# HySonLab/Protein_Redesign

Measured on AMD Instinct MI355X. Metric: denoising-steps/sec (fwd+rev) per complex, N=256 res, higher is better.
Workload: dtype f32; 1 GPU; configs[1]: synthetic 256-residue + 64-atom ligand (N=320), single_dim=512 pair_dim=64 num_blocks=4 num_steps=1000, 1 complex/GPU, sharded by sample index (no data-path collective; one all_gather of the samples at the end of the timed region); samples_per_gpu=1, hip_graph=True, outputs_finite=True, backend=single process

## Files before the change

include/prd_hip.h:

```cpp
#ifndef PRD_HIP_H
#define PRD_HIP_H

#include <stddef.h>
#include <stdint.h>

#ifdef __cplusplus
extern "C" {
#endif

#ifndef __HIP__
typedef struct ihipStream_t* hipStream_t;
#endif

#define PRD_VERSION 101
#define PRD_STEP_BOUNDARY_SYNC_INTS 2
#define PRD_ERR_ARG (-1)
#define PRD_ERR_ALIGN (-2)
#define PRD_ERR_UNSUPPORTED (-3)
#define PRD_ERR_WORKSPACE (-4)

int prd_version(void);

#define PRD_ARITH_FP32 0
#define PRD_ARITH_SPLIT16 1
// ... 163 lines not shown
int prd_tri_attn_core_v2(float* og, const float* pair, const float* mask, const float* wq, const float* wk,
                         const float* wv, const float* wg, const float* bg, int ending,
                         int b, int N, int P, int H, int c, int tune, hipStream_t stream);
int prd_tri_attn_core_v2_lse(float* og, float* lse, const float* pair, const float* mask, const float* wq, const float* wk,
                             const float* wv, const float* wg, const float* bg, int ending,
                             int b, int N, int P, int H, int c, int tune, hipStream_t stream);
int prd_tri_attn_core_fused_supported(int N, int P, int arith);
int prd_tri_attn_core_fused(float* og, float* pair_out, const float* pair, const float* og_in, const float* wo_in,
                            const float* bo_in, const float* mask, const float* wq, const float* wk, const float* wv,
                            const float* wg, const float* bg, int ending, int b, int N, int P, int H, int c,
                            hipStream_t stream);
int prd_single_attn_core(float* o, const float* qkvg, int ldq, const float* bias, const float* mask,
                         int b, int N, int H, int c, hipStream_t stream);
int prd_pair_transition(float* out, const float* pair, const float* w1, const float* b1, const float* w2,
                        const float* b2, int residual, int b, int N, int P, int* queue, int arith, hipStream_t stream);
int prd_block_tail(float* pair, const float* og, const float* wo, const float* bo, const float* w1, const float* b1,
                   const float* w2, const float* b2, const float* bias_w, const float* bias_b, float* bias_out,
                   int b, int N, int P, int H, int* queue, int arith, hipStream_t stream);
int prd_coord_head(float* eps_raw, const float* pair, const float* z, const float* mask,
                   const float* w1, const float* b1, const float* w2, int b, int N, int P, int arith, hipStream_t stream);
int prd_remove_mean(float* out, const float* x, const float* mask, int b, int N, int D, hipStream_t stream);
int prd_reverse_update(float* z, float* seq_t, int64_t* t, const float* noise_pred, const float* seq_pred,
                       const float* noise, const float* mask, const float* coef,
                       int b, int N, int n_cls, int num_steps, hipStream_t stream);

int prd_step_boundary(float* z, float* seq_t, int64_t* t, const float* eps_raw, float* seq_pred,
                      const float* noise, const float* mask, const float* coef,
                      float* single_next, const float* static_single, const float* residue_mask, const float* w_rt,
                      float* ebeta_next, const float* freqs, const float* w_beta, int* sync,
                      int b, int N, int n_cls, int num_steps, int S, int P, int time_dim,
                      const float* seq_h, int ldh, const float* w_seq, int S_h, hipStream_t stream);

int prd_spa_attn_core_supported(int N, int c, int arith);
size_t prd_spa_attn_core_workspace(int b, int N, int H, int c);
int prd_spa_attn_core(float* o, const float* qkvg, int ldq, const float* bias, const float* mask,
                      int b, int N, int H, int c, float* ws, size_t ws_bytes, int arith, hipStream_t stream);

int prd_tri_attn_heads_supported(int N, int P, int H, int c, int arith);
size_t prd_tri_attn_heads_workspace_bytes(int b, int N, int P, int H, int c);
int prd_tri_attn_core_heads(float* og, const float* pair, const float* mask, const float* wq, const float* wk,
                            const float* wv, const float* wg, const float* bg, int ending, int b, int N, int P, int H, int c,
                            float* ws, size_t ws_bytes, int arith, hipStream_t stream);
int prd_tri_attn_core_heads_lse(float* og, float* lse, const float* pair, const float* mask, const float* wq, const float* wk,
                                const float* wv, const float* wg, const float* bg, int ending, int b, int N, int P, int H, int c,
                                float* ws, size_t ws_bytes, int arith, hipStream_t stream);

int prd_tri_attn_bwd_heads_supported(int N, int P, int H, int c, int arith);
size_t prd_tri_attn_bwd_heads_workspace_bytes(int b, int N, int P, int H, int c);
int prd_tri_attn_bwd_core_heads(float* dqkvg, const float* dog, const float* og, const float* pair, const float* mask,
                                const float* wq, const float* wk, const float* wv, const float* wg, const float* bg,
                                const float* lse, float* x_out, int ending, int b, int N, int P, int H, int c,
                                float* ws, size_t ws_bytes, int arith, hipStream_t stream);

size_t prd_workspace_bytes(const char* op, int b, int N, int S, int P);

#ifdef __cplusplus
}
#endif
#endif
```

protein_redesign_amd/_lib.py:

```python
from __future__ import annotations

import ctypes as C
import os

import torch

HERE = os.path.dirname(os.path.abspath(__file__))
LIB_PATH = os.environ.get("PRD_LIB", os.path.join(HERE, "libprd_hip.so"))

vp, ci, cf, cz, cll = C.c_void_p, C.c_int, C.c_float, C.c_size_t, C.c_longlong


class PrdGemm(C.Structure):
    _fields_ = [
        ("A", vp), ("B", vp), ("C", vp),
        ("M", ci), ("N", ci), ("K", ci),
        ("lda", ci), ("ldb", ci), ("ldc", ci),
        ("G1", ci), ("G2", ci),
        ("sa1", cll), ("sa2", cll), ("sb1", cll), ("sb2", cll), ("sc1", cll), ("sc2", cll),
        ("b_kn", ci), ("alpha", cf), ("colscale", vp),
        ("bias", vp), ("act", ci), ("act_from", ci),
        ("addmat", vp), ("sad1", cll), ("sad2", cll), ("ldadd", ci),
        ("colmask", vp), ("scm1", cll), ("fill", cf),
        ("rowmask", vp), ("srm1", cll),
        ("mulmat", vp), ("smu1", cll), ("smu2", cll), ("ldmul", ci),
        ("resid", vp), ("sr1", cll), ("sr2", cll), ("ldr", ci),
        ("tile_hint", ci),
        ("a_ln", ci),
        ("ln_out", vp), ("ldlo", ci),
        ("arith", ci),
        ("C2", vp), ("ldc2", ci), ("n_split", ci),
        ("rowmask_cols", ci),
        ("rscale", vp),
        ("ws", vp), ("ws_bytes", cz),
        ("wsum", vp),
        ("out_ln", vp), ("ldol", ci),
        ("a_scale", cf),
        ("mul_pos", ci),
        ("a_amax", vp),
    ]


SIGNATURES = {
    "prd_version": [],
    "prd_tri_attn_variant": [ci, ci, ci],
    "prd_gemm": [C.POINTER(PrdGemm), vp],
    "prd_gemm_slab_workspace": [ci, ci, ci],
    "prd_gemm_slab_ok": [ci, ci, ci, ci],
    "prd_single_fc1_folded_ok": [ci] * 5,
    "prd_single_fc1_folded": [vp] * 10 + [ci] * 4 + [vp, cz, ci, vp],
    "prd_ln_rows": [vp, vp, vp, vp, ci, ci, ci, ci, vp],
    "prd_softmax_rows": [vp, ci, ci, ci, vp],
    "prd_static_pair": [vp] * 13 + [ci] * 5 + [vp],
    "prd_atom_embed": [vp] * 5 + [ci] * 4 + [vp],
    "prd_single_init": [vp] * 5 + [ci] * 3 + [vp],
    "prd_time_embed": [vp] * 4 + [ci] * 4 + [vp],
    "prd_pair_init": [vp] * 7 + [ci] * 5 + [vp],
    "prd_pair_bias": [vp] * 6 + [ci] * 4 + [vp],
    "prd_pair_bias2": [vp] * 6 + [ci] + [vp] * 5 + [ci] * 4 + [vp],
    "prd_opm_pair": [vp] * 6 + [ci] * 6 + [vp],
    "prd_pair_head_supported": [ci, ci, ci, ci],
    "prd_pair_head": [vp] * 7 + [ci] + [vp] * 3 + [ci, ci] + [vp] * 5 + [ci] + [vp] * 5 + [ci] * 5 + [vp],
    "prd_outer_linear": [vp] * 4 + [ci] + [vp] * 2 + [ci] * 5 + [vp, ci, vp],
    "prd_tri_mul": [vp] * 11 + [ci] * 5 + [vp, cz, vp, ci, vp],
    "prd_tri_mul_contract": [vp, vp, ci, ci, ci, ci, vp],
    "prd_tri_mul_contract_scaled": [vp, vp, vp, ci, ci, ci, ci, vp],
    "prd_tri_mul_chain_supported": [ci, ci, ci],
    "prd_tri_attn_core_fused_supported": [ci, ci, ci],
    "prd_tri_attn_core_fused": [vp] * 12 + [ci] * 6 + [vp],
    "prd_tri_mul_chain": [vp, vp, vp, vp, ci, ci, ci, vp, cz, ci, vp],
    "prd_tri_mul_out_bwd": [vp] * 15 + [ci] * 4 + [vp],
    "prd_tri_mul_out_bwd_amax": [vp] * 15 + [ci] * 4 + [vp, vp],
    "prd_tri_mul_bwd_operands": [vp, vp, ci, ci, ci, vp],
    "prd_tri_mul_proj_bwd": [vp] * 13 + [ci] * 5 + [vp],
    "prd_tri_attn_bwd_core": [vp] * 9 + [ci] * 6 + [vp],
    "prd_tri_attn_bwd_core_v2_supported": [ci, ci],
    "prd_tri_attn_bwd_core_v2": [vp] * 12 + [ci] * 6 + [vp],
    "prd_ln_rows_bwd": [vp, vp, vp, vp, cll, ci, vp],
    "prd_pair_bias_bwd": [vp, vp, vp, vp, vp, vp, ci, cll, ci, ci, vp],
    "prd_sym_transpose": [vp, vp, ci, ci, ci, vp],
    "prd_sym_transpose_amax": [vp, vp, ci, ci, ci, vp, vp],
    "prd_sym_rows": [vp, vp, cf, ci, ci, ci, vp],
    "prd_outer_linear_bwd_reduce": [vp, vp, ci, vp, vp, vp, cll, ci, ci, vp],
    "prd_pair_linear_supported": [ci, ci, ci],
    "prd_pair_linear": [vp, vp, vp, vp, cll, ci, ci, ci, vp, ci, vp, ci, ci, vp],
    "prd_linear_wgrad_workspace": [cll, ci, ci],
    "prd_linear_wgrad": [vp, vp, vp, vp, cll, ci, ci, ci, ci, vp, cz, ci, vp],
    "prd_embed_wgrad_workspace": [cll, ci, ci],
    "prd_embed_wgrad": [vp, vp, vp, vp, cll, ci, ci, ci, vp, cz, vp],
    "prd_rbf_rows": [vp, vp, vp, vp, ci, ci, ci, vp],
    "prd_embed_wgrad_multi": [vp, vp, vp, vp, ci, vp, cll, ci, ci, vp, cz, vp],
    "prd_tri_attn": [vp] * 10 + [ci] * 7 + [vp, cz, vp, ci, vp],
    "prd_pair_transition": [vp] * 6 + [ci] * 4 + [vp, ci, vp],
    "prd_block_tail": [vp] * 11 + [ci] * 4 + [vp, ci, vp],
    "prd_single_attn_core": [vp, vp, ci, vp, vp] + [ci] * 4 + [vp],
    "prd_coord_head": [vp] * 7 + [ci] * 4 + [vp],
    "prd_remove_mean": [vp] * 3 + [ci] * 3 + [vp],
    "prd_reverse_update": [vp] * 8 + [ci] * 4 + [vp],
    "prd_step_boundary": [vp] * 16 + [ci] * 7 + [vp, ci, vp, ci] + [vp],
    "prd_tri_attn_core": [vp] * 8 + [ci] * 7 + [vp],
    "prd_tri_attn_core_v2": [vp] * 8 + [ci] * 7 + [vp],
    "prd_tri_attn_core_v2_lse": [vp] * 9 + [ci] * 7 + [vp],
    "prd_tri_attn_v2_form": [ci, ci, ci],
    "prd_tri_attn_core_chunked": [vp] * 8 + [ci] * 6 + [vp, cz, vp],
    "prd_tri_attn_stats_bytes": [ci] * 5,
    "prd_tri_attn_v2_supported": [ci, ci, ci],
    "prd_tri_attn_out": [vp] * 5 + [ci] * 4 + [vp, ci, vp],
    "prd_spa_attn_core_supported": [ci, ci, ci],
    "prd_spa_attn_core_workspace": [ci, ci, ci, ci],
    "prd_spa_attn_core": [vp, vp, ci, vp, vp, ci, ci, ci, ci, vp, cz, ci, vp],
    "prd_workspace_bytes": [C.c_char_p, ci, ci, ci, ci],
    "prd_tri_attn_pair_supported": [ci, ci, ci],
    "prd_tri_attn_pair": [vp, vp, vp, vp, vp, ci, ci, ci, ci, ci, vp, ci, vp],
    "prd_tri_attn_heads_supported": [ci] * 5,
    "prd_tri_attn_heads_workspace_bytes": [ci] * 5,
    "prd_tri_attn_core_heads": [vp] * 8 + [ci] * 6 + [vp, cz, ci, vp],
    "prd_tri_attn_core_heads_lse": [vp] * 9 + [ci] * 6 + [vp, cz, ci, vp],
    "prd_tri_attn_bwd_heads_supported": [ci] * 5,
    "prd_tri_attn_bwd_heads_workspace_bytes": [ci] * 5,
    "prd_tri_attn_bwd_core_heads": [vp] * 12 + [ci] * 6 + [vp, cz, ci, vp],
}

GEMM_MODES = {"fp32": 0, "split16": 1, "bf16x3": 1}
DEFAULT_GEMM_MODE = "split16"

_ARITH_BEFORE_STREAM = ("prd_coord_head", "prd_pair_head", "prd_pair_init", "prd_opm_pair", "prd_outer_linear", "prd_tri_mul", "prd_tri_mul_contract", "prd_tri_mul_contract_scaled", "prd_tri_mul_proj_bwd",
                        "prd_tri_attn", "prd_tri_attn_core", "prd_tri_attn_out", "prd_pair_transition", "prd_block_tail", "prd_tri_mul_chain",
                        "prd_linear_wgrad", "prd_pair_linear", "prd_spa_attn_core", "prd_tri_attn_pair",
                        "prd_tri_attn_core_heads", "prd_tri_attn_core_heads_lse", "prd_tri_attn_bwd_core_heads", "prd_single_fc1_folded")
_ARITH_LAST = ("prd_tri_attn_variant", "prd_tri_mul_chain_supported", "prd_tri_attn_core_fused_supported", "prd_tri_attn_stats_bytes",
               "prd_gemm_slab_ok", "prd_pair_head_supported", "prd_pair_linear_supported", "prd_spa_attn_core_supported",
               "prd_tri_attn_pair_supported", "prd_tri_attn_heads_supported",
               "prd_tri_attn_bwd_heads_supported", "prd_single_fc1_folded_ok")
_TUNE_BEFORE_STREAM = ("prd_tri_attn_core_v2", "prd_tri_attn_core_v2_lse")
_TUNE_LAST = ("prd_tri_attn_v2_supported", "prd_tri_attn_v2_form")


def tune_from_env(env=None) -> int:
    env = os.environ if env is None else env

    def geti(name, default):
        v = env.get(name)
        return default if v is None or v == "" else int(v)

    t = geti("PRD_TA_VARIANT", 0) & 15
    if geti("PRD_TA2_V3", 1) == 0:
        t |= 1 << 4
    if geti("PRD_TA2_LONG", 1) == 0:
        t |= 1 << 5
    f = geti("PRD_TA2_FLAGS", -1)
    if f >= 0:
        t |= (1 << 6) | ((f & 31) << 7)
    if geti("PRD_OL_VARIANT", 0) == 1:
        t |= 1 << 12
    nw = geti("PRD_TMS_NW", 8)
    t |= (1 << 13) if nw == 12 else (2 << 13) if nw == 16 else 0
    if geti("PRD_GEMM_KG", 1) == 0:
        t |= 1 << 15
    if geti("PRD_GEMM_SLAB", 1) == 0:
        t |= 1 << 16
    if geti("PRD_GEMM_BRING", 1) == 0:
        t |= 1 << 17
    if geti("PRD_GEMM_XCDCOLS", 0) == 1:
        t |= 1 << 18
    if geti("PRD_TA2_TAIL", 1) == 0:
        t |= 1 << 19
    if geti("PRD_TA2_XCD8", 1) == 0:
        t |= 1 << 20
    if geti("PRD_TA2_GV", 1) == 0:
        t |= 1 << 21
    if geti("PRD_TMP_NW", 12) == 16:
        t |= 1 << 22
    if geti("PRD_TMS_DEPTH", 2) == 3 and nw == 8:
        t |= 3 << 13
    return t


ABI_VERSION = 101


class _Library:

    def __init__(self, cdll, mode: int, tune: int = 0):
        self._cdll = cdll
        self._mode = mode
        self._tune = tune
        self._wrapped = {}
# ... 137 lines not shown
```

protein_redesign_amd/csrc/prd_common.h:

```cpp
#pragma once
#include <hip/hip_runtime.h>
#include <stdint.h>

typedef float f32x16 __attribute__((ext_vector_type(16)));
typedef float f32x4 __attribute__((ext_vector_type(4)));
typedef float f32x2 __attribute__((ext_vector_type(2)));

#define PRD_DEV __device__ __forceinline__

PRD_DEV f32x16 mfma32(float a, float b, f32x16 c) { return __builtin_amdgcn_mfma_f32_32x32x2f32(a, b, c, 0, 0, 0); }
PRD_DEV f32x4 mfma16(float a, float b, f32x4 c) { return __builtin_amdgcn_mfma_f32_16x16x4f32(a, b, c, 0, 0, 0); }

PRD_DEV float sigmoidf_(float x) { return 1.0f / (1.0f + expf(-x)); }
PRD_DEV float relu_nan(float v) { return v < 0.f ? 0.f : v; }
PRD_DEV float sigmoid_fast(float x) { return __builtin_amdgcn_rcpf(1.0f + __builtin_amdgcn_exp2f(-1.4426950408889634f * x)); }

constexpr float NEG_LOG2E = -1.4426950408889634f;
PRD_DEV float gate_from_scaled(float y) { return __builtin_amdgcn_rcpf(1.0f + __builtin_amdgcn_exp2f(y)); }

typedef __amdgpu_buffer_rsrc_t prd_rsrc;
PRD_DEV prd_rsrc make_rsrc(const void* p) {
    const unsigned long long a = reinterpret_cast<unsigned long long>(p);
    const unsigned lo = __builtin_amdgcn_readfirstlane((unsigned)a), hi = __builtin_amdgcn_readfirstlane((unsigned)(a >> 32));
    return __builtin_amdgcn_make_buffer_rsrc(reinterpret_cast<void*>(((unsigned long long)hi << 32) | lo), 0, 0x7fffffff, 0x00020000);
}
PRD_DEV void buf_store(float v, prd_rsrc rs, unsigned lane_bytes, unsigned uniform_bytes) {
    __builtin_amdgcn_raw_buffer_store_b32(__float_as_uint(v), rs, lane_bytes, uniform_bytes, 0);
}
PRD_DEV float buf_load(prd_rsrc rs, unsigned lane_bytes, unsigned uniform_bytes) {
    return __uint_as_float(__builtin_amdgcn_raw_buffer_load_b32(rs, lane_bytes, uniform_bytes, 0));
}
constexpr unsigned BUF_OOB = 0x80000000u;

PRD_DEV int drow32(int q, int hi) { return (q & 3) + 8 * (q >> 2) + 4 * hi; }
PRD_DEV int cll_ch(int s, int hi) { return 8 * (s >> 2) + 4 * hi + (s & 3); }

PRD_DEV float xhalf_sum(float v) { return v + __shfl_xor(v, 32); }
PRD_DEV float row16_sum(float v) {
    v += __builtin_bit_cast(float, __builtin_amdgcn_update_dpp(0, __builtin_bit_cast(int, v), 0x128, 0xf, 0xf, false));
    v += __builtin_bit_cast(float, __builtin_amdgcn_update_dpp(0, __builtin_bit_cast(int, v), 0x124, 0xf, 0xf, false));
    v += __builtin_bit_cast(float, __builtin_amdgcn_update_dpp(0, __builtin_bit_cast(int, v), 0x122, 0xf, 0xf, false));
    v += __builtin_bit_cast(float, __builtin_amdgcn_update_dpp(0, __builtin_bit_cast(int, v), 0x121, 0xf, 0xf, false));
    return v;
}

template <int C>
PRD_DEV void load_row_cll(const float* __restrict__ row, int hi, bool valid, float (&x)[C / 2]) {
#pragma unroll
    for (int m = 0; m < C / 8; ++m) {
        float4 v = make_float4(0.f, 0.f, 0.f, 0.f);
        if (valid) v = *reinterpret_cast<const float4*>(row + 8 * m + 4 * hi);
        x[4 * m + 0] = v.x; x[4 * m + 1] = v.y; x[4 * m + 2] = v.z; x[4 * m + 3] = v.w;
    }
}

// ... 440 lines not shown
}

template <int NB>
PRD_DEV void zero_acc(f32x16 (&acc)[NB]) {
#pragma unroll
    for (int nb = 0; nb < NB; ++nb)
#pragma unroll
        for (int q = 0; q < 16; ++q) acc[nb][q] = 0.f;
}

PRD_DEV float max3f(float a, float b, float c) {
    float d;
    asm("v_max3_f32 %0, %1, %2, %3" : "=v"(d) : "v"(a), "v"(b), "v"(c));
    return d;
}
PRD_DEV float max2f(float a, float b) {
    float d;
    asm("v_max_f32 %0, %1, %2" : "=v"(d) : "v"(a), "v"(b));
    return d;
}

PRD_DEV float rows4_max(float v) {
    auto a = __builtin_amdgcn_permlane32_swap(__float_as_uint(v), __float_as_uint(v), false, false);
    v = max2f(__uint_as_float(a[0]), __uint_as_float(a[1]));
    auto b = __builtin_amdgcn_permlane16_swap(__float_as_uint(v), __float_as_uint(v), false, false);
    return max2f(__uint_as_float(b[0]), __uint_as_float(b[1]));
}
PRD_DEV float rows4_sum(float v) {
    auto a = __builtin_amdgcn_permlane32_swap(__float_as_uint(v), __float_as_uint(v), false, false);
    v = __uint_as_float(a[0]) + __uint_as_float(a[1]);
    auto b = __builtin_amdgcn_permlane16_swap(__float_as_uint(v), __float_as_uint(v), false, false);
    return __uint_as_float(b[0]) + __uint_as_float(b[1]);
}

PRD_DEV void wave_lds_fence() {
    __builtin_amdgcn_fence(__ATOMIC_RELEASE, "wavefront");
    __builtin_amdgcn_wave_barrier();
    __builtin_amdgcn_fence(__ATOMIC_ACQUIRE, "wavefront");
}

struct WaveTasks {
    int* q;
    long ntask, cur, stride;
    int shard, nshard, count, last;
    PRD_DEV WaveTasks(int* queue, long ntask_, int waves_per_wg) : q(queue), ntask(ntask_) {
        stride = (long)gridDim.x * waves_per_wg;
        cur = (long)(threadIdx.x >> 6) * gridDim.x + blockIdx.x;
        nshard = gridDim.x < 8 ? (int)gridDim.x : 8;
        shard = (int)(blockIdx.x % nshard);
        count = (int)((ntask - shard + nshard - 1) / nshard);
        const int wgs = (int)((gridDim.x - shard + nshard - 1) / nshard);
        last = count + wgs * waves_per_wg - 1;
    }
    PRD_DEV long next() {
        if (!q) {
            const long t = (long)__builtin_amdgcn_readfirstlane((int)cur);
            cur += stride;
            return t < ntask ? t : -1;
        }
        int t = 0;
        if ((threadIdx.x & 63) == 0) {
            t = atomicAdd(q + 32 * shard, 1);
            if (t == last) atomicExch(q + 32 * shard, 0);
        }
        t = __builtin_amdgcn_readfirstlane(t);
        return t < count ? (long)t * nshard + shard : -1;
    }
};

#define PRD_SPLIT_ARITH(a)                                                                       \
    const int arith_full = (a);                                                                  \
    const int tune = (a) >> 8;                                                                   \
    (void)tune; (void)arith_full;                                                                \
    if ((a) < 0 || ((a) & 0xff) > 1) return -1;                                                  \
    (a) &= 0xff
#define PRD_TGET_TA_VARIANT(t) ((t) & 15)
#define PRD_TGET_TA2_NO_V3(t) (((t) >> 4) & 1)
#define PRD_TGET_TA2_NO_LONG(t) (((t) >> 5) & 1)
#define PRD_TGET_TA2_FLAGS(t) ((((t) >> 6) & 1) ? (((t) >> 7) & 31) : -1)
#define PRD_TGET_TA2_NO_TAIL_SPLIT(t) (((t) >> 19) & 1)
#define PRD_TGET_TA2_NO_GV(t) (((t) >> 21) & 1)
#define PRD_TGET_TMP_NW16(t) (((t) >> 22) & 1)
#define PRD_TGET_TMS_D3(t) ((((t) >> 13) & 3) == 3)
#define PRD_TGET_OL_GEN2(t) (((t) >> 12) & 1)
#define PRD_TGET_TMS_NW(t) ((((t) >> 13) & 3) == 1 ? 12 : (((t) >> 13) & 3) == 2 ? 16 : 8)

static inline int prd_ceil_div(int a, int b) { return (a + b - 1) / b; }
static inline int prd_round_up(int a, int b) { return prd_ceil_div(a, b) * b; }
```

protein_redesign_amd/csrc/prd_pair.hip:

```cpp
#include "prd_common.h"
#include <cstdlib>
#include "../../include/prd_hip.h"
#include <mutex>

#ifdef PRD_TIMING
__device__ unsigned long long prd_dbg_pair[256 * 16 * 8];
extern "C" int prd_debug_read_pair(void* dst) { return (int)hipMemcpyFromSymbol(dst, HIP_SYMBOL(prd_dbg_pair), sizeof(prd_dbg_pair)); }
struct PairPhaseTimer {
    unsigned long long t, acc[8];
    __device__ PairPhaseTimer() { for (int k = 0; k < 8; ++k) acc[k] = 0; t = __builtin_readcyclecounter(); }
    __device__ void mark(int k) {
        __builtin_amdgcn_sched_barrier(0);
        const unsigned long long n = __builtin_readcyclecounter();
        __builtin_amdgcn_sched_barrier(0);
        acc[k] += n - t;
        t = n;
    }
    __device__ void flush() {
        if ((threadIdx.x & 63) == 0) for (int k = 0; k < 8; ++k) prd_dbg_pair[(blockIdx.x * 16 + (threadIdx.x >> 6)) * 8 + k] = acc[k];
    }
};
#else
struct PairPhaseTimer {
    __device__ void mark(int) {}
// ... 1453 lines not shown
    constexpr int NWH = 8;
    const size_t lds = (size_t)4 * P * dist_dim + (size_t)4 * P * C + ((size_t)dist_dim + P + 16 * P + 4 * P) * 4;
    const long ntask = (long)b * N * prd_ceil_div(N, 32);
    const int grid = grid_for(ntask, NWH, 256);
    if (P == 64) {
        PRD_SET_LDS((pair_head_h2_kernel<64, NWH>), lds);
        hipLaunchKernelGGL((pair_head_h2_kernel<64, NWH>), dim3(grid), dim3(NWH * 64), lds, stream, pair, static_pair, z, mask, centers, w_dist,
                           ebeta, dist_dim, ab, w_out, b_out, C, apply_mask, bias_a, gamma_a, beta_a, w_a, bvec_a, Ha, bias_b, gamma_b, beta_b,
                           w_b, bvec_b, Hb, b, N);
    } else {
        PRD_SET_LDS((pair_head_h2_kernel<32, NWH>), lds);
        hipLaunchKernelGGL((pair_head_h2_kernel<32, NWH>), dim3(grid), dim3(NWH * 64), lds, stream, pair, static_pair, z, mask, centers, w_dist,
                           ebeta, dist_dim, ab, w_out, b_out, C, apply_mask, bias_a, gamma_a, beta_a, w_a, bvec_a, Ha, bias_b, gamma_b, beta_b,
                           w_b, bvec_b, Hb, b, N);
    }
    return (int)hipGetLastError();
}

extern "C" int prd_opm_pair(float* out, const float* pair, const float* ab, const float* mask, const float* w_out,
                            const float* b_out, int flags, int b, int N, int P, int C, int arith, hipStream_t stream) {
    PRD_SPLIT_ARITH(arith);
    if (!out || !pair || !ab || !mask || !w_out || !b_out || b <= 0 || N <= 0) return PRD_ERR_ARG;
    PRD_CHECK_P(P);
    if (C <= 0 || (C & 7)) return PRD_ERR_UNSUPPORTED;
    const size_t lds = ((size_t)P * (C + 4) + P) * sizeof(float);
    if (lds > 160 * 1024) return PRD_ERR_UNSUPPORTED;
    const long ntask = (long)b * N * prd_ceil_div(N, 32);
    const int grid = grid_for(ntask, 4, 1024);
    if (arith == PRD_ARITH_SPLIT16 && (C % 128) == 0) {
        const size_t lds2 = (size_t)4 * P * C + (size_t)P * 4;
        if (P == 64) {
            PRD_SET_LDS(opm_pair_h2_kernel<64>, lds2);
            hipLaunchKernelGGL(opm_pair_h2_kernel<64>, dim3(grid), dim3(WG), lds2, stream, out, pair, ab, mask, w_out, b_out, b, N, C, flags);
        } else {
            PRD_SET_LDS(opm_pair_h2_kernel<32>, lds2);
            hipLaunchKernelGGL(opm_pair_h2_kernel<32>, dim3(grid), dim3(WG), lds2, stream, out, pair, ab, mask, w_out, b_out, b, N, C, flags);
        }
        return (int)hipGetLastError();
    }
    if (P == 64) {
        PRD_SET_LDS(opm_pair_kernel<64>, lds);
        hipLaunchKernelGGL(opm_pair_kernel<64>, dim3(grid), dim3(WG), lds, stream, out, pair, ab, mask, w_out, b_out, b, N, C, flags);
    } else {
        PRD_SET_LDS(opm_pair_kernel<32>, lds);
        hipLaunchKernelGGL(opm_pair_kernel<32>, dim3(grid), dim3(WG), lds, stream, out, pair, ab, mask, w_out, b_out, b, N, C, flags);
    }
    return (int)hipGetLastError();
}

namespace {
template <int P, int KS>
__global__ __launch_bounds__(512) void outer_linear_ks_kernel(float* out, const float* pair, const float* __restrict__ x,
                                                              const float* __restrict__ u, const float* __restrict__ w,
                                                              const float* __restrict__ bias, int b, int N, int residual, int ldu) {
    constexpr int NB = P / 32, NW = 8, S = 128 * KS, NG = NB * 4;
    constexpr int CW = 16 * KS;
    constexpr int XP = CW * 4 + 16;
    constexpr int LR = CW / 4;
    constexpr int RPI = 64 / LR;
    constexpr int NLD = 32 / RPI;
    extern __shared__ __attribute__((aligned(16))) unsigned char smem_ks[];
    float4* part = reinterpret_cast<float4*>(smem_ks);
    float4* stage = part;
    constexpr int PSZ = NW * NG * 64;
    const int lane = threadIdx.x & 63, r = lane & 31, hi = lane >> 5;
    const int wave = __builtin_amdgcn_readfirstlane(threadIdx.x >> 6);
    PairPhaseTimer pt;
    const int k0 = wave * CW;
    float4* mystage = stage + (size_t)wave * 32 * (XP / 16);
    u32x4 wh[NB][KS], wl[NB][KS];
#pragma unroll
    for (int nb = 0; nb < NB; ++nb)
#pragma unroll
        for (int st = 0; st < KS; ++st) {
            const float* wp = w + (size_t)(32 * nb + r) * (2 * S) + k0 + 16 * st + 8 * hi;
            const float4 g0 = *reinterpret_cast<const float4*>(wp), g1 = *reinterpret_cast<const float4*>(wp + 4);
            const float v[8] = {g0.x, g0.y, g0.z, g0.w, g1.x, g1.y, g1.z, g1.w};
#pragma unroll
            for (int q = 0; q < 4; ++q) {
                unsigned a_, b_;
                split2h(H2_WSCALE * v[2 * q], H2_WSCALE * v[2 * q + 1], a_, b_);
                wh[nb][st][q] = a_;
                wl[nb][st][q] = b_;
            }
        }
    const int nvb = (N + 31) / 32;
    const int npairs = nvb * (nvb + 1) / 2;
    constexpr int RG = 8;
    const int ntask = b * npairs * (32 / RG);
    struct Task { int bb, i0, jb; };
    auto decode = [&](int t) {
        Task T;
        const int grp = t % (32 / RG), t2 = t / (32 / RG);
        T.bb = t2 / npairs;
        int pidx = t2 - T.bb * npairs, ib = 0;
        while (pidx >= nvb - ib) { pidx -= nvb - ib; ++ib; }
        T.jb = ib + pidx;
        T.i0 = ib * 32 + grp * RG;
        return T;
    };
    const int lane_w = lane;
    struct Epi { float4 ui, pu, pm; };
    pt.mark(6);
    for (int t = blockIdx.x; t < ntask; t += gridDim.x) {
        const Task T = decode(t);
        int lane = lane_w;
        asm volatile("" : "+v"(lane));
// ... 52 lines not shown
        fetch_x(T.i0, xa);
        __syncthreads();
        pt.mark(4);
        auto finish = [&](int i, const float4* pb, const Epi& e) {
            if (!row_ok(i)) return;
            float4 sum = make_float4(0.f, 0.f, 0.f, 0.f);
#pragma unroll
            for (int w2 = 0; w2 < NW; ++w2) {
                const float4 v = pb[(size_t)w2 * NG * 64 + eoff];
                sum.x += v.x; sum.y += v.y; sum.z += v.z; sum.w += v.w;
            }
            const bool upper = jvalid && je >= i, mirror = jvalid && je > i;
            const float4 ui = e.ui, pu = e.pu, pm = e.pm;
            if (upper)
                *reinterpret_cast<float4*>(out + (((size_t)T.bb * N + i) * N + je) * P + ech) =
                    make_float4(pu.x + (((sum.x * H2_INV_WSCALE + ui.x) - uj.x) + bs.x), pu.y + (((sum.y * H2_INV_WSCALE + ui.y) - uj.y) + bs.y),
                                pu.z + (((sum.z * H2_INV_WSCALE + ui.z) - uj.z) + bs.z), pu.w + (((sum.w * H2_INV_WSCALE + ui.w) - uj.w) + bs.w));
            if (mirror)
                *reinterpret_cast<float4*>(out + (((size_t)T.bb * N + je) * N + i) * P + ech) =
                    make_float4(pm.x + (((sum.x * H2_INV_WSCALE + uj.x) - ui.x) + bs.x), pm.y + (((sum.y * H2_INV_WSCALE + uj.y) - ui.y) + bs.y),
                                pm.z + (((sum.z * H2_INV_WSCALE + uj.z) - ui.z) + bs.z), pm.w + (((sum.w * H2_INV_WSCALE + uj.w) - ui.w) + bs.w));
        };
        for (int ii = 0; ii < RG; ++ii) {
            const int i = T.i0 + ii;
            fetch_epi(i, enext);
            f32x16 acc[NB];
            zero_acc(acc);
            if (row_ok(i)) {
#pragma unroll
                for (int st = 0; st < KS; ++st) {
                    const float f[8] = {xa[st][0].x * xb[st][0].x, xa[st][0].y * xb[st][0].y, xa[st][0].z * xb[st][0].z, xa[st][0].w * xb[st][0].w,
                                        xa[st][1].x * xb[st][1].x, xa[st][1].y * xb[st][1].y, xa[st][1].z * xb[st][1].z, xa[st][1].w * xb[st][1].w};
                    u32x4 ph, pl;
#pragma unroll
                    for (int q = 0; q < 4; ++q) {
                        unsigned a_, b_;
                        split2h(f[2 * q], f[2 * q + 1], a_, b_);
                        ph[q] = a_;
                        pl[q] = b_;
                    }
#pragma unroll
                    for (int nb = 0; nb < NB; ++nb)
                        acc[nb] = __builtin_amdgcn_mfma_f32_32x32x16_f16(__builtin_bit_cast(f16x8_t, wh[nb][st]), __builtin_bit_cast(f16x8_t, ph), acc[nb], 0, 0, 0);
#pragma unroll
                    for (int nb = 0; nb < NB; ++nb)
                        acc[nb] = __builtin_amdgcn_mfma_f32_32x32x16_f16(__builtin_bit_cast(f16x8_t, wh[nb][st]), __builtin_bit_cast(f16x8_t, pl), acc[nb], 0, 0, 0);
#pragma unroll
                    for (int nb = 0; nb < NB; ++nb)
                        acc[nb] = __builtin_amdgcn_mfma_f32_32x32x16_f16(__builtin_bit_cast(f16x8_t, wl[nb][st]), __builtin_bit_cast(f16x8_t, ph), acc[nb], 0, 0, 0);
                }
            }
            if (ii + 1 < RG) fetch_x(i + 1, xa);
            pt.mark(0);
            if (ii > 0) finish(i - 1, part + (size_t)((ii - 1) & 1) * PSZ, ecur);
            ecur = enext;
            pt.mark(3);
            {
                float4* pw = part + (size_t)(ii & 1) * PSZ + ((size_t)wave * NG) * 64;
#pragma unroll
                for (int g = 0; g < NG; ++g)
                    pw[g * 64 + ((lane & 48) | ((lane & 15) ^ ((2 * g + hi) & 15)))] = make_float4(acc[g >> 2][4 * (g & 3)], acc[g >> 2][4 * (g & 3) + 1], acc[g >> 2][4 * (g & 3) + 2],
                                                     acc[g >> 2][4 * (g & 3) + 3]);
            }
            pt.mark(1);
            asm volatile("s_waitcnt lgkmcnt(0)\n\ts_barrier" ::: "memory");
            pt.mark(2);
        }
        finish(T.i0 + RG - 1, part + (size_t)((RG - 1) & 1) * PSZ, ecur);
        __syncthreads();
    }
    pt.mark(7);
    pt.flush();
}
}

extern "C" int prd_outer_linear(float* out, const float* pair, const float* x, const float* u, int ldu, const float* w,
                                const float* bias, int residual, int b, int N, int P, int S, int* queue, int arith, hipStream_t stream) {
    PRD_SPLIT_ARITH(arith);
    if (!out || !pair || !x || !u || !w || !bias || b <= 0 || N <= 0) return PRD_ERR_ARG;
    if (ldu < P || (ldu & 3)) return PRD_ERR_ALIGN;
    PRD_CHECK_P(P);
    if (S <= 0 || (S & 7)) return PRD_ERR_UNSUPPORTED;
    const long ntask = (long)b * N * prd_ceil_div(N, 32);
    const size_t lds = ((size_t)P * (S + 4) + P) * sizeof(float);
    const bool ol_v1 = PRD_TGET_OL_GEN2(tune);
    if (arith == PRD_ARITH_SPLIT16 && !ol_v1 && (S == 128 || S == 256 || S == 512) && (long)b * N * N < (1L << 30)) {
        const int nvb = prd_ceil_div(N, 32);
        const long ntile = (long)b * (nvb * (nvb + 1) / 2) * 4;
        const int grid = (int)(ntile < 256 ? ntile : 256);
        const size_t ldsp = (size_t)2 * 8 * (P / 32 * 4) * 64 * 16, ldss = (size_t)8 * 32 * ((S / 8) * 4 + 16);
        const size_t ldsk = ldsp > ldss ? ldsp : ldss;
#define PRD_OLKS(PP, KK)                                                                                               \
        do {                                                                                                           \
            PRD_SET_LDS((outer_linear_ks_kernel<PP, KK>), ldsk);                                                       \
            hipLaunchKernelGGL((outer_linear_ks_kernel<PP, KK>), dim3(grid), dim3(512), ldsk, stream, out, pair, x, u, w, bias, b, N, residual, ldu); \
        } while (0)
        if (P == 64) { if (S == 512) PRD_OLKS(64, 4); else if (S == 256) PRD_OLKS(64, 2); else PRD_OLKS(64, 1); }
        else { if (S == 512) PRD_OLKS(32, 4); else if (S == 256) PRD_OLKS(32, 2); else PRD_OLKS(32, 1); }
#undef PRD_OLKS
        return (int)hipGetLastError();
    }
    if (arith == PRD_ARITH_SPLIT16 && (S % 128) == 0 && (size_t)4 * P * S + 4 * P <= 160 * 1024) {
        constexpr int NWL = 8;
        const int nvb = prd_ceil_div(N, 32);
        const long nsym = (long)b * (nvb * (nvb + 1) / 2) * 32;
        const int grid = grid_for(nsym, 4, 256);
        const size_t lds2 = (size_t)4 * P * S + 4 * P;
        if (P == 64) {
            PRD_SET_LDS((outer_linear_res_h2_kernel<64, NWL>), lds2);
            hipLaunchKernelGGL((outer_linear_res_h2_kernel<64, NWL>), dim3(grid), dim3(NWL * 64), lds2, stream, out, pair, x, u, w, bias, b, N, S, residual, ldu);
        } else {
            PRD_SET_LDS((outer_linear_res_h2_kernel<32, NWL>), lds2);
            hipLaunchKernelGGL((outer_linear_res_h2_kernel<32, NWL>), dim3(grid), dim3(NWL * 64), lds2, stream, out, pair, x, u, w, bias, b, N, S, residual, ldu);
        }
        return (int)hipGetLastError();
    }
    if (lds <= 150 * 1024 && (S % 64) == 0) {
        constexpr int NWL = 8;
        const int nvb = prd_ceil_div(N, 32);
        const long nsym = (long)b * (nvb * (nvb + 1) / 2) * 32;
        const int grid = grid_for(nsym, 4, 256);
        int* oq = (nsym > (long)grid * NWL) ? queue : nullptr;
        if (P == 64) {
            PRD_SET_LDS((outer_linear_res_kernel<64, NWL>), lds);
            hipLaunchKernelGGL((outer_linear_res_kernel<64, NWL>), dim3(grid), dim3(NWL * 64), lds, stream, oq, out, pair, x, u, w, bias, b, N, S, residual, ldu);
        } else {
            PRD_SET_LDS((outer_linear_res_kernel<32, NWL>), lds);
            hipLaunchKernelGGL((outer_linear_res_kernel<32, NWL>), dim3(grid), dim3(NWL * 64), lds, stream, oq, out, pair, x, u, w, bias, b, N, S, residual, ldu);
        }
        return (int)hipGetLastError();
    }
    const int grid = grid_for(ntask, 4, 1024);
    if (P == 64) hipLaunchKernelGGL(outer_linear_kernel<64>, dim3(grid), dim3(WG), 0, stream, out, pair, x, u, w, bias, b, N, S, residual, ldu);
    else hipLaunchKernelGGL(outer_linear_kernel<32>, dim3(grid), dim3(WG), 0, stream, out, pair, x, u, w, bias, b, N, S, residual, ldu);
    return (int)hipGetLastError();
}

namespace {
template <int P>
int launch_pair_tail_h2(float* out, const float* pair, const float* og, const float* wo, const float* bo, const float* w1,
                        const float* b1, const float* w2, const float* b2, const float* bias_w, const float* bias_b,
                        float* bias_out, int H, long rows, long nn, int residual, hipStream_t stream) {
    constexpr int NWH = 12;
    const size_t lds = ((size_t)2 * 4 * P * (P / 8) + (size_t)2 * P * (4 * P / 8) + (size_t)2 * P * 8) * 16 + (size_t)(4 * P + 2 * P + 8 * P) * 4;
    if (lds > 160 * 1024) return PRD_ERR_UNSUPPORTED;
    const int grid = grid_for((rows + 31) / 32, 4, 256);
    PRD_SET_LDS((pair_tail_h2_kernel<P, NWH>), lds);
    hipLaunchKernelGGL((pair_tail_h2_kernel<P, NWH>), dim3(grid), dim3(NWH * 64), lds, stream, out, pair, og, wo, bo, w1, b1, w2, b2,
// ... 103 lines not shown
```

protein_redesign_amd/csrc/prd_tri.hip:

```cpp
#include "prd_common.h"
#include "../../include/prd_hip.h"
#include <atomic>
#include <cstdlib>
#include <mutex>

#ifdef PRD_TIMING
__device__ unsigned long long prd_dbg[256 * 16 * 8 * 4];
__device__ int prd_dbg_sel;
extern "C" int prd_debug_read(void* dst) { return (int)hipMemcpyFromSymbol(dst, HIP_SYMBOL(prd_dbg), sizeof(prd_dbg)); }
extern "C" int prd_debug_select(int id) { return (int)hipMemcpyToSymbol(HIP_SYMBOL(prd_dbg_sel), &id, sizeof(int)); }
#define PRD_STAMP(k) do { if (lane == 0 && it < 8) prd_dbg[((blockIdx.x * 12 + wave) * 8 + it) * 4 + (k)] = __builtin_readcyclecounter(); } while (0)
struct PhaseTimer {
    unsigned long long t, acc[8];
    __device__ PhaseTimer() { for (int k = 0; k < 8; ++k) acc[k] = 0; t = __builtin_readcyclecounter(); }
    __device__ void mark(int k) {
        __builtin_amdgcn_sched_barrier(0);
        const unsigned long long n = __builtin_readcyclecounter();
        __builtin_amdgcn_sched_barrier(0);
        acc[k] += n - t;
        t = n;
    }
    __device__ void flush(int id = 0) {
        if (prd_dbg_sel != 0 && prd_dbg_sel != id) return;
        if ((threadIdx.x & 63) == 0) for (int k = 0; k < 8; ++k) prd_dbg[(blockIdx.x * 16 + (threadIdx.x >> 6)) * 8 + k] = acc[k];
// ... 285 lines not shown
    *reinterpret_cast<float4*>(&As[BUF][srow * LDP + 4 * sf]) = R##a0;            \
    *reinterpret_cast<float4*>(&As[BUF][(srow + 32) * LDP + 4 * sf]) = R##a1;     \
    *reinterpret_cast<float4*>(&Bs[BUF][srow * LDP + 4 * sf]) = R##b0;            \
    *reinterpret_cast<float4*>(&Bs[BUF][(srow + 32) * LDP + 4 * sf]) = R##b1;
#define PRD_TMC_CHUNK(C, CUR, R, N)                                               \
    {                                                                             \
        const int c2 = (C) + 2 < nchunk ? (C) + 2 : nchunk - 1;                   \
        PRD_TMC_LOAD(N, c2 * KCH)                                                 \
        const float* as = &As[CUR][(wm0 + r) * LDP + hi * 16];                    \
        const float* bs = &Bs[CUR][(wn0 + r) * LDP + hi * 16];                    \
        _Pragma("unroll") for (int t = 0; t < 4; ++t) {                           \
            const float4 a = *reinterpret_cast<const float4*>(as + 4 * t);        \
            const float4 bq = *reinterpret_cast<const float4*>(bs + 4 * t);       \
            acc = mfma32(a.x, bq.x, acc);                                         \
            acc = mfma32(a.y, bq.y, acc);                                         \
            acc = mfma32(a.z, bq.z, acc);                                         \
            acc = mfma32(a.w, bq.w, acc);                                         \
        }                                                                         \
        if ((C) + 1 < nchunk) { PRD_TMC_STAGE(R, (CUR) ^ 1) }                     \
        __syncthreads();                                                          \
    }
    float4 ua0, ua1, ub0, ub1, va0, va1, vb0, vb1;
    PRD_TMC_LOAD(u, 0)
    PRD_TMC_STAGE(u, 0)
    {
        const int c1 = 1 < nchunk ? 1 : 0;
        PRD_TMC_LOAD(u, c1 * KCH)
    }
    __syncthreads();
    for (int c = 0; c < nchunk; c += 2) {
        PRD_TMC_CHUNK(c, 0, u, v)
        if (c + 1 < nchunk) PRD_TMC_CHUNK(c + 1, 1, v, u)
    }
#undef PRD_TMC_LOAD
#undef PRD_TMC_LD1
#undef PRD_TMC_STAGE
#undef PRD_TMC_CHUNK
    float* __restrict__ Oc = O + (size_t)ch * N * ldn;
    const int n = n0 + wn0 + r;
    if (n < N) {
#pragma unroll
        for (int q = 0; q < 16; ++q) {
            const int m = m0 + wm0 + drow32(q, hi);
            if (m < N) Oc[(size_t)m * ldn + n] = acc[q];
        }
    }
    }
}

constexpr int TMS_T = 160, TMS_PLANE = TMS_T * 64, TMS_OPER = 2 * TMS_PLANE;
template <int NWV, int DEPTH = 2, bool ASC = false>
__global__ __launch_bounds__(NWV * 64) void tri_mul_contract_split_kernel(float* __restrict__ O, const float* __restrict__ AB,
                                                                          int N, int ldn, int P, int nbatch, int tiles, int swap,
                                                                          const unsigned* __restrict__ a_amax) {
    constexpr int NT = NWV * 64, NPT = (2560 + NT - 1) / NT, NSUB = (25 + NWV - 1) / NWV;
    extern __shared__ __attribute__((aligned(16))) unsigned char tms[];
    PhaseTimer pt;
    const int tid = threadIdx.x, lane = tid & 63, wave = tid >> 6;
    const int r = lane & 31, hi = lane >> 5;
    const int nch = nbatch * P;
    const int t2 = tiles * tiles;
    unsigned srow[NPT], sdst[NPT], ssrc[NPT];
    bool sisb[NPT], sok[NPT];
    const int wbase = __builtin_amdgcn_readfirstlane(tid & ~63);
#pragma unroll
    for (int i = 0; i < NPT; ++i) {
        const int pw = wbase + NT * i;
        sok[i] = pw < 2560;
        const int oper = (sok[i] && pw >= 1280) ? 1 : 0;
        const int pc = sok[i] ? tid + NT * i : 0;
        const int q = pc - 1280 * oper;
        const int row = q >> 3, f = q & 7;
        sisb[i] = oper == 1;
        srow[i] = row;
        sdst[i] = oper * TMS_OPER + row * 64 + (((f >> 1) ^ ((row >> 2) & 3)) << 4) + (f & 1) * 8;
        ssrc[i] = ((unsigned)row * ldn + 4 * f) * 4u;
    }
    const unsigned swz = (unsigned)((r >> 2) & 3);
    for (int vblk = blockIdx.x; vblk < nch * t2; vblk += gridDim.x) {
        int ch, tile;
        if ((nch & 7) == 0 && (gridDim.x & 7) == 0) {
            const int xcd = vblk & 7, k = vblk >> 3;
            ch = xcd + 8 * (k / t2);
            tile = k % t2;
        } else {
            ch = vblk / t2;
            tile = vblk % t2;
        }
        const int bb = ch / P, d = ch - bb * P;
        const int m0 = (tile / tiles) * TMS_T, n0 = (tile % tiles) * TMS_T;
        float asc = 1.0f, iasc = 1.0f;
        if constexpr (ASC) {
            asc = split_scale(a_amax[bb]);
            iasc = __uint_as_float((254u << 23) - __float_as_uint(asc));
        }
        const float* __restrict__ A = AB + ((size_t)bb * 2 * P + (swap ? P : 0) + d) * N * ldn;
        const float* __restrict__ B = AB + ((size_t)bb * 2 * P + (swap ? 0 : P) + d) * N * ldn;
        const prd_rsrc ra = make_rsrc(A + (size_t)m0 * ldn), rb = make_rsrc(B + (size_t)n0 * ldn);
        unsigned off[NPT];
#pragma unroll
        for (int i = 0; i < NPT; ++i)
            off[i] = (sok[i] && (sisb[i] ? n0 : m0) + (int)srow[i] < N) ? ssrc[i] : BUF_OOB;
        int si[NSUB], sj[NSUB];
        bool sv[NSUB];
#pragma unroll
        for (int k = 0; k < NSUB; ++k) {
            const int s_ = wave + NWV * k;
// ... 61 lines not shown
        _Pragma("unroll") for (int st = 0; st < 2; ++st) {                                                          \
            const unsigned col = (((unsigned)(2 * st + hi)) ^ swz) << 4;                                            \
            _Pragma("unroll") for (int k = 0; k < NSUB; ++k) {                                                      \
                if (sv[k]) {                                                                                        \
                    const unsigned char* ap = base + (32 * si[k] + r) * 64 + col;                                   \
                    const unsigned char* bp = base + TMS_OPER + (32 * sj[k] + r) * 64 + col;                        \
                    u32x4 a[2], bq[2];                                                                              \
                    _Pragma("unroll") for (int pl = 0; pl < 2; ++pl) {                                              \
                        a[pl] = *reinterpret_cast<const u32x4*>(ap + pl * TMS_PLANE);                               \
                        bq[pl] = *reinterpret_cast<const u32x4*>(bp + pl * TMS_PLANE);                              \
                    }                                                                                               \
                    const int pa[3] = {0, 0, 1}, pb[3] = {0, 1, 0};                                                 \
                    _Pragma("unroll") for (int t = 0; t < 3; ++t)                                                   \
                        acc[k] = __builtin_amdgcn_mfma_f32_32x32x16_f16(__builtin_bit_cast(f16x8_t, a[pa[t]]),      \
                                                                        __builtin_bit_cast(f16x8_t, bq[pb[t]]), acc[k], 0, 0, 0); \
                }                                                                                                   \
            }                                                                                                       \
        }                                                                                                           \
        pt.mark(0);                                                                                                 \
        if ((C) + 1 < nchunk) { PRD_TMS_STAGE(R, cur_ ^ 1) }                                                        \
        pt.mark(1);                                                                                                 \
        __syncthreads();                                                                                            \
        pt.mark(2);                                                                                                 \
    }
            PRD_TMS_LOAD(u, 0)
            PRD_TMS_STAGE(u, 0)
            PRD_TMS_LOAD(u, (1 < nchunk ? 1 : 0))
            PRD_TMS_LOAD(v, (2 < nchunk ? 2 : nchunk - 1))
            __syncthreads();
            pt.mark(3);
            for (int c = 0; c < nchunk; c += 3) {
                PRD_TMS_CHUNK3(c, u, w)
                if (c + 1 < nchunk) PRD_TMS_CHUNK3(c + 1, v, u)
                if (c + 2 < nchunk) PRD_TMS_CHUNK3(c + 2, w, v)
            }
#undef PRD_TMS_CHUNK3
        } else {
        PRD_TMS_LOAD(u, 0)
        PRD_TMS_STAGE(u, 0)
        {
            const int c1 = 1 < nchunk ? 1 : 0;
            PRD_TMS_LOAD(u, c1)
        }
        __syncthreads();
        pt.mark(3);
        for (int c = 0; c < nchunk; c += 2) {
            PRD_TMS_CHUNK(c, 0, u, v)
            if (c + 1 < nchunk) PRD_TMS_CHUNK(c + 1, 1, v, u)
        }
        }
#undef PRD_TMS_LOAD
#undef PRD_TMS_STAGE
#undef PRD_TMS_CHUNK
        float* __restrict__ Oc = O + (size_t)ch * N * ldn;
#pragma unroll
        for (int k = 0; k < NSUB; ++k) {
            if (!sv[k]) continue;
            const int n = n0 + 32 * sj[k] + r;
            if (n < N) {
#pragma unroll
                for (int q = 0; q < 16; ++q) {
                    const int m = m0 + 32 * si[k] + drow32(q, hi);
                    if (m < N) Oc[(size_t)m * ldn + n] = ASC ? acc[k][q] * iasc : acc[k][q];
                }
            }
        }
        pt.mark(4);
    }
    pt.flush(3);
}

template <int P, int NW, bool B3>
__global__ __launch_bounds__(NW * 64) void tri_mul_out_kernel(int* queue, float* out, const float* pair, const float* __restrict__ O,
                                                              const float* __restrict__ wo, const float* __restrict__ bo,
                                                              const float* __restrict__ wog, const float* __restrict__ bog,
                                                              int b, int N, int ldn, int residual) {
    constexpr int KH = P / 2, NB = P / 32;
    constexpr int WSZ = B3 ? P * P : P * (P + 4);
    __shared__ __attribute__((aligned(16))) float Wol[WSZ];
    __shared__ __attribute__((aligned(16))) float Wgl[WSZ];
    __shared__ __attribute__((aligned(16))) float bol[P];
    __shared__ __attribute__((aligned(16))) float bgl[P];
    constexpr float ASC = B3 ? H2_INV_WSCALE : 1.0f;
    PhaseTimer pt;
    if (B3) {
        stage_weight_h2<P>(reinterpret_cast<u32x4*>(Wol), wo, P, P, threadIdx.x, NW * 64, H2_WSCALE);
        stage_weight_h2<P>(reinterpret_cast<u32x4*>(Wgl), wog, P, P, threadIdx.x, NW * 64, H2_WSCALE);
    } else {
        stage_weight_cll<P>(Wol, wo, P, P, threadIdx.x, NW * 64);
        stage_weight_cll<P>(Wgl, wog, P, P, threadIdx.x, NW * 64);
    }
    stage_vec_cll(bol, bo, P, threadIdx.x, NW * 64);
    stage_vec_cll(bgl, bog, P, threadIdx.x, NW * 64);
    __syncthreads();
    pt.mark(6);
    const int lane = threadIdx.x & 63, r = lane & 31, hi = lane >> 5, wave = threadIdx.x >> 6;
    const int nvb = (N + 31) / 32;
    const long ntask = (long)b * N * nvb;
    const long slots = (long)gridDim.x * 4;
    const long left = ntask % slots;
    const bool coop = !B3 && queue == nullptr && NB == 2 && NW >= 4 && left > 0 && left <= 2 * (long)gridDim.x;
    const long nwhole = coop ? ntask - left : ntask;
    WaveTasks tasks(queue, nwhole, NW);
    for (long task = tasks.next(); task >= 0; task = tasks.next()) {
        const int vb = (int)(task % nvb);
        const long bi = task / nvb;
        const int bb = (int)(bi / N), i = (int)(bi - (long)bb * N);
        const int j = vb * 32 + r;
        const bool valid = j < N;
        const int jj = valid ? j : 0;
        const long off = (bi * N + jj) * P;
        float x[KH], xr[KH];
        {
            const prd_rsrc ro = make_rsrc(O + (((long)bb * P) * N + i) * ldn + vb * 32);
            const unsigned cbytes = (unsigned)N * (unsigned)ldn * 4u;
            const unsigned lo = valid ? (unsigned)r * 4u + (unsigned)(4 * hi) * cbytes : BUF_OOB;
#pragma unroll
            for (int s = 0; s < KH; ++s) x[s] = buf_load(ro, lo, (unsigned)(8 * (s >> 2) + (s & 3)) * cbytes);
            const prd_rsrc rp = make_rsrc(pair + (bi * N + vb * 32) * P);
            load_row_cll_buf<P>(rp, valid ? ((unsigned)r * P + 4 * hi) * 4u : BUF_OOB, xr);
        }
        pt.mark(0);
        float gate[KH];
        {
            float xn[KH];
#pragma unroll
            for (int s = 0; s < KH; ++s) xn[s] = xr[s];
            ln_cll<KH>(xn);
            pt.mark(1);
            f32x16 ag[NB];
            zero_acc(ag);
            if (B3) {
                u32x4 xs[2][P / 16];
                split2h_cll<KH>(xn, xs);
                rowgemm_h2<P, NB>(reinterpret_cast<const u32x4*>(Wgl), P, 0, xs, ag, r, hi);
            } else {
                rowgemm<P, NB>(Wgl, xn, ag, r, hi);
            }
#pragma unroll
            for (int s = 0; s < KH; ++s) gate[s] = sigmoid_fast(ag[s >> 4][s & 15] * ASC + bgl[hi * KH + s]);
        }
        pt.mark(2);
        ln_cll<KH>(x);
        pt.mark(3);
        f32x16 ao[NB];
        zero_acc(ao);
        if (B3) {
            u32x4 xs[2][P / 16];
            split2h_cll<KH>(x, xs);
            rowgemm_h2<P, NB>(reinterpret_cast<const u32x4*>(Wol), P, 0, xs, ao, r, hi);
        } else {
            rowgemm<P, NB>(Wol, x, ao, r, hi);
        }
        pt.mark(4);
#pragma unroll
        for (int s = 0; s < KH; ++s) x[s] = (residual ? xr[s] : 0.f) + gate[s] * (ao[s >> 4][s & 15] * ASC + bol[hi * KH + s]);
        store_row_cll<P>(out + off, hi, valid, x);
        pt.mark(5);
    }
    pt.mark(7);
    pt.flush(2);
    if (coop) {
        __shared__ float part[2][64][17];
        for (long task = nwhole + blockIdx.x; task < ntask; task += gridDim.x) {
            const int vb = (int)(task % nvb);
            const long bi = task / nvb;
            const int bb = (int)(bi / N), i = (int)(bi - (long)bb * N);
            const int j = vb * 32 + r;
            const bool valid = j < N;
            const int jj = valid ? j : 0;
            const long off = (bi * N + jj) * P;
            const int nb = wave & 1;
            f32x16 acc[1];
            zero_acc(acc);
            float x[KH];
            if (wave < 2) {
                load_row_cll<P>(pair + off, hi, valid, x);
                ln_cll<KH>(x);
                if (B3) {
                    u32x4 xs[2][P / 16];
                    split2h_cll<KH>(x, xs);
                    rowgemm_h2<P, 1>(reinterpret_cast<const u32x4*>(Wgl), P, nb * 32, xs, acc, r, hi);
                } else {
                    rowgemm<P, 1>(Wgl + nb * 32 * (P + 4), x, acc, r, hi);
                }
            } else if (wave < 4) {
#pragma unroll
                for (int s = 0; s < KH; ++s)
                    x[s] = valid ? O[(((long)bb * P + cll_ch(s, hi)) * N + i) * ldn + jj] : 0.f;
                ln_cll<KH>(x);
                if (B3) {
                    u32x4 xs[2][P / 16];
                    split2h_cll<KH>(x, xs);
                    rowgemm_h2<P, 1>(reinterpret_cast<const u32x4*>(Wol), P, nb * 32, xs, acc, r, hi);
                } else {
                    rowgemm<P, 1>(Wol + nb * 32 * (P + 4), x, acc, r, hi);
                }
#pragma unroll
                for (int q = 0; q < 16; ++q) part[nb][lane][q] = acc[0][q] * ASC;
            }
            __syncthreads();
            if (wave < 2) {
                float* orow = out + off + 32 * nb + 4 * hi;
                const float* prow = pair + off + 32 * nb + 4 * hi;
#pragma unroll
                for (int gq = 0; gq < 4; ++gq) {
                    float4 pv = make_float4(0.f, 0.f, 0.f, 0.f);
                    if (valid && residual) pv = *reinterpret_cast<const float4*>(prow + 8 * gq);
                    float o4[4] = {pv.x, pv.y, pv.z, pv.w};
#pragma unroll
                    for (int e = 0; e < 4; ++e) {
                        const int q = 4 * gq + e, sidx = 16 * nb + q;
// ... 1211 lines not shown
                }
            }
            float4 qf[2], gf[2];
#pragma unroll
            for (int t = 0; t < 2; ++t) {
                const int src = 16 * t + ql + 32 * (g4 & 1);
                float lo[4], up[4], glo[4], gup[4];
#pragma unroll
                for (int e = 0; e < 4; ++e) {
                    lo[e] = __shfl(qg[e], src);
                    up[e] = __shfl(qg[4 + e], src);
                    glo[e] = __shfl(qg[8 + e], src);
                    gup[e] = __shfl(qg[12 + e], src);
                }
                const bool hiq = (g4 >> 1) != 0;
                qf[t] = make_float4(sc * (hiq ? up[0] : lo[0]), sc * (hiq ? up[1] : lo[1]), sc * (hiq ? up[2] : lo[2]), sc * (hiq ? up[3] : lo[3]));
                gf[t] = make_float4(sigmoid_fast(hiq ? gup[0] : glo[0]), sigmoid_fast(hiq ? gup[1] : glo[1]),
                                    sigmoid_fast(hiq ? gup[2] : glo[2]), sigmoid_fast(hiq ? gup[3] : glo[3]));
            }
            f32x4 o[2];
            float l_tot[2], m_ref[2];
            ta_keyloop<2, true>(Kl, Vt, kadd, qf, npad, ql, g4, o, l_tot, m_ref);
#pragma unroll
            for (int t = 0; t < 2; ++t) {
                const int v = qb * 32 + 16 * t + ql;
                if (v < N) {
                    const long pos = ending ? (((long)bb * N + v) * N + u) : (bu * N + v);
                    float4* dst = reinterpret_cast<float4*>(og + pos * HC + h * C + 4 * g4);
                    float* st = stats + (pos * H + h) * 2;
                    const float il = 1.0f / l_tot[t];
                    float4 mine = make_float4(gf[t].x * (o[t][0] * il), gf[t].y * (o[t][1] * il), gf[t].z * (o[t][2] * il), gf[t].w * (o[t][3] * il));
                    float m_new = m_ref[t], l_new = l_tot[t];
                    if (!first) {
                        const float m0 = st[0], l0 = st[1];
                        const float4 prev = *dst;
                        const float M = fmaxf(m0, m_ref[t]);
                        const float w0 = l0 * exp2f(m0 - M), w1 = l_tot[t] * exp2f(m_ref[t] - M);
                        const float iw = 1.0f / (w0 + w1);
                        const float a0 = w0 * iw, a1 = w1 * iw;
                        mine = make_float4(a0 * prev.x + a1 * mine.x, a0 * prev.y + a1 * mine.y, a0 * prev.z + a1 * mine.z, a0 * prev.w + a1 * mine.w);
                        m_new = M;
                        l_new = w0 + w1;
                    }
                    *dst = mine;
                    if (g4 == 0) { st[0] = m_new; st[1] = l_new; }
                }
            }
        }
    }
}

template <int P, int NW, bool B3>
__global__ __launch_bounds__(NW * 64) void tri_attn_out_kernel(int* queue, float* out, const float* pair, const float* __restrict__ og,
                                                               const float* __restrict__ wo, const float* __restrict__ bo, long rows, int residual) {
    constexpr int KH = P / 2, NB = P / 32, HC = 64;
    __shared__ __attribute__((aligned(16))) float Wl[B3 ? P * HC : P * (HC + 4)];
    __shared__ __attribute__((aligned(16))) float bl[P];
    if (B3) stage_weight_h2<HC>(reinterpret_cast<u32x4*>(Wl), wo, P, HC, threadIdx.x, NW * 64, H2_WSCALE);
    else stage_weight_cll<HC>(Wl, wo, P, HC, threadIdx.x, NW * 64);
    stage_vec_cll(bl, bo, P, threadIdx.x, NW * 64);
    __syncthreads();
    const int lane = threadIdx.x & 63, r = lane & 31, hi = lane >> 5;
    const long ntask = (rows + 31) / 32;
    WaveTasks tasks(queue, ntask, NW);
    for (long task = tasks.next(); task >= 0; task = tasks.next()) {
        const long pos = task * 32 + r;
        const bool valid = pos < rows;
        float x[HC / 2];
        load_row_cll<HC>(og + pos * HC, hi, valid, x);
        f32x16 acc[NB];
        zero_acc(acc);
        if (B3) {
            u32x4 xs[2][HC / 16];
            split2h_cll<HC / 2>(x, xs);
            rowgemm_h2<HC, NB>(reinterpret_cast<const u32x4*>(Wl), P, 0, xs, acc, r, hi);
        } else {
            rowgemm<HC, NB>(Wl, x, acc, r, hi);
        }
        float pr[KH];
        load_row_cll<P>(pair + pos * P, hi, valid && residual, pr);
#pragma unroll
        for (int s = 0; s < KH; ++s) pr[s] = pr[s] + (acc[s >> 4][s & 15] * (B3 ? H2_INV_WSCALE : 1.0f) + bl[hi * KH + s]);
        store_row_cll<P>(out + pos * P, hi, valid, pr);
    }
}

int grid_for(long tasks, int per_wg, int cap) {
    long g = (tasks + per_wg - 1) / per_wg;
    if (g > cap) g = cap;
    if (g < 1) g = 1;
    return (int)g;
}

}

#define PRD_SET_LDS(kernel, bytes)                                                                              \
    do {                                                                                                        \
        static std::once_flag prd_lds_once;                                                                     \
        std::call_once(prd_lds_once, [] {                                                                       \
            (void)hipFuncSetAttribute((const void*)kernel, hipFuncAttributeMaxDynamicSharedMemorySize, 160 * 1024); \
        });                                                                                                     \
        (void)(bytes);                                                                                          \
    } while (0)

static void launch_contract_split(int tune, int grid, size_t lds3, hipStream_t stream, float* O, const float* AB, int N, int ldn, int P, int nbatch,
                                  int tiles, int swap, const unsigned* a_amax = nullptr) {
    if (a_amax) {
        PRD_SET_LDS((tri_mul_contract_split_kernel<8, 2, true>), lds3);
        hipLaunchKernelGGL((tri_mul_contract_split_kernel<8, 2, true>), dim3(grid), dim3(512), lds3, stream, O, AB, N, ldn, P, nbatch, tiles, swap, a_amax);
        return;
    }
    const int nw = PRD_TGET_TMS_NW(tune);
#ifdef PRD_AB
    if (nw == 8 && PRD_TGET_TMS_D3(tune)) {
        PRD_SET_LDS((tri_mul_contract_split_kernel<8, 3>), lds3);
        hipLaunchKernelGGL((tri_mul_contract_split_kernel<8, 3>), dim3(grid), dim3(512), lds3, stream, O, AB, N, ldn, P, nbatch, tiles, swap, nullptr);
        return;
    }
    if (nw == 16) {
        PRD_SET_LDS((tri_mul_contract_split_kernel<16>), lds3);
        hipLaunchKernelGGL((tri_mul_contract_split_kernel<16>), dim3(grid), dim3(1024), lds3, stream, O, AB, N, ldn, P, nbatch, tiles, swap, nullptr);
        return;
    }
#endif
    if (nw == 12) {
        PRD_SET_LDS((tri_mul_contract_split_kernel<12>), lds3);
        hipLaunchKernelGGL((tri_mul_contract_split_kernel<12>), dim3(grid), dim3(768), lds3, stream, O, AB, N, ldn, P, nbatch, tiles, swap, nullptr);
    } else {
        PRD_SET_LDS((tri_mul_contract_split_kernel<8>), lds3);
        hipLaunchKernelGGL((tri_mul_contract_split_kernel<8>), dim3(grid), dim3(512), lds3, stream, O, AB, N, ldn, P, nbatch, tiles, swap, nullptr);
    }
}


#ifdef PRD_AB
constexpr bool PRD_FIRST_GEN = true;
#else
constexpr bool PRD_FIRST_GEN = false;
#endif
namespace {
size_t tri_attn_lds(int N, int P, bool b3, bool* long_row) {
    const int npad = prd_round_up(N, 64);
    const size_t wsz = b3 ? (size_t)3 * 64 * (2 * (P / 16) + 1) * 4 : (size_t)64 * (P + 4);
    size_t lds = (wsz + (size_t)3 * npad * KP + 16 * (npad + 4) + npad + 32) * sizeof(float);
    if (b3) lds = (size_t)64 * P * 4 + (size_t)npad * (192 + KP * 4 + 4) + (size_t)64 * (npad + 8) + 128;
    *long_row = lds > 160 * 1024;
    if (*long_row) {
        const size_t lds_sl = (size_t)64 * P * 4 + (size_t)npad * 68 + (size_t)64 * (npad + 8) + 128 + 8 * 4096;
        if (b3 && lds_sl <= 160 * 1024) return lds_sl;
        lds = ((size_t)64 * (P + 4) + (size_t)npad * KP + 16 * (npad + 4) + npad) * sizeof(float);
    }
    return lds;
}
}

extern "C" int prd_tri_attn_variant(int N, int P, int arith) {
    PRD_SPLIT_ARITH(arith);
    if (N <= 0) return PRD_ERR_ARG;
    if (P != 32 && P != 64) return PRD_ERR_UNSUPPORTED;
    bool long_row;
    const bool split = arith == PRD_ARITH_SPLIT16;
    const bool v2 = split && PRD_TGET_TA_VARIANT(tune) == 0 && prd_tri_attn_v2_supported(N, P, tune);
    const bool b3 = split && (PRD_FIRST_GEN || v2);
    const size_t lds = tri_attn_lds(N, P, b3, &long_row);
    if (lds > 160 * 1024)
        return v2 ? 2 : 3;
    if (!long_row) return 0;
    if (v2) return 2;
    const int npad = prd_round_up(N, 64);
    return (b3 && lds == (size_t)64 * P * 4 + (size_t)npad * 68 + (size_t)64 * (npad + 8) + 128 + 8 * 4096) ? 2 : 1;
}

namespace {
constexpr int TA_CHUNK_MAX = 960;
int ta_chunks(int N) { return prd_ceil_div(N, TA_CHUNK_MAX); }
}

extern "C" size_t prd_tri_attn_stats_bytes(int b, int N, int P, int H, int arith) {
    if (b <= 0 || N <= 0 || H <= 0) return 0;
    return prd_tri_attn_variant(N, P, arith) == 3 ? (size_t)b * N * N * H * 2 * sizeof(float) : 0;
}

extern "C" int prd_tri_attn_core_chunked(float* og, const float* pair, const float* mask, const float* wq, const float* wk,
// ... 44 lines not shown
extern "C" int prd_tri_mul(float* out, const float* pair, const float* mask, const float* w_proj, const float* b_proj,
                           const float* w_gate, const float* b_gate, const float* w_out, const float* b_out,
                           const float* w_ogate, const float* b_ogate, int incoming, int residual,
                           int b, int N, int P, float* ws, size_t ws_bytes, int* queue, int arith, hipStream_t stream) {
    PRD_SPLIT_ARITH(arith);
    if (!out || !pair || !mask || !w_proj || !b_proj || !w_gate || !b_gate || !w_out || !b_out || !w_ogate || !b_ogate || !ws ||
        b <= 0 || N <= 0) return PRD_ERR_ARG;
    if (P != 32 && P != 64) return PRD_ERR_UNSUPPORTED;
    if (ws_bytes < prd_workspace_bytes("tri_mul", b, N, 0, P)) return PRD_ERR_WORKSPACE;
    const int ldn = prd_round_up(N, 32);
    float* AB = ws;
    float* O = ws + (size_t)2 * b * P * N * ldn;
    const bool b3m = arith == PRD_ARITH_SPLIT16;
    {
        constexpr int NWP = 16;
        const bool b3 = b3m;
        const size_t wsz = b3 ? (size_t)2 * P * P : (size_t)2 * P * (P + 4);
        const size_t lds = (2 * wsz + 4 * P) * sizeof(float);
        const long ntask = ((long)b * N * (ldn / 32) + 7) / 8 * 8 * (2 * P / 32);
        const int grid = grid_for(ntask, 4, 256);
#define PRD_PROJ_LAUNCH(PP, BB, NWV)                                                                                 \
        do {                                                                                                         \
            PRD_SET_LDS((tri_mul_proj_kernel<PP, NWV, BB>), lds);                                                    \
            hipLaunchKernelGGL((tri_mul_proj_kernel<PP, NWV, BB>), dim3(grid), dim3(NWV * 64), lds, stream, queue, AB, pair, mask, \
                               w_proj, b_proj, w_gate, b_gate, b, N, ldn, incoming);                                 \
        } while (0)
        if (P == 64) { if (b3) { if (PRD_TGET_TMP_NW16(tune)) PRD_PROJ_LAUNCH(64, true, 16); else PRD_PROJ_LAUNCH(64, true, 12); } else PRD_PROJ_LAUNCH(64, false, NWP); }
        else { if (b3) PRD_PROJ_LAUNCH(32, true, 12); else PRD_PROJ_LAUNCH(32, false, NWP); }
#undef PRD_PROJ_LAUNCH
        int e = (int)hipGetLastError();
        if (e) return e;
    }
    {
        const int tiles = prd_ceil_div(N, 64);
        const int vblocks = b * P * tiles * tiles;
        if (b3m) {
            const int tl = prd_ceil_div(N, TMS_T);
            const int vb3 = b * P * tl * tl;
            const size_t lds3 = (size_t)4 * TMS_OPER;
        launch_contract_split(tune, vb3 < 256 ? vb3 : 256, lds3, stream, O, AB, N, ldn, P, b, tl, 0);
        }
        else
            hipLaunchKernelGGL(tri_mul_contract_kernel, dim3(vblocks < 1024 ? vblocks : 1024), dim3(256), 0, stream, O, AB, N, ldn, P, b, tiles);
        int e = (int)hipGetLastError();
        if (e) return e;
    }
    {
        constexpr int NWO = 8;
        const bool b3o = b3m;
        const long ntask = (long)b * N * prd_ceil_div(N, 32);
        const int grid = grid_for(ntask, 4, 256);
#define PRD_OUT_LAUNCH(PP, BB)                                                                                         \
        hipLaunchKernelGGL((tri_mul_out_kernel<PP, NWO, BB>), dim3(grid), dim3(NWO * 64), 0, stream, queue, out, pair, O, w_out, \
                           b_out, w_ogate, b_ogate, b, N, ldn, residual)
        if (P == 64) { if (b3o) PRD_OUT_LAUNCH(64, true); else PRD_OUT_LAUNCH(64, false); }
        else { if (b3o) PRD_OUT_LAUNCH(32, true); else PRD_OUT_LAUNCH(32, false); }
#undef PRD_OUT_LAUNCH
    }
    return (int)hipGetLastError();
}

extern "C" int prd_tri_mul_contract(float* O, const float* AB, int b, int N, int P, int arith, hipStream_t stream) {
    PRD_SPLIT_ARITH(arith);
    if (!O || !AB || b <= 0 || N <= 0) return PRD_ERR_ARG;
    if (P != 32 && P != 64 && P != 128) return PRD_ERR_UNSUPPORTED;
    const int ldn = prd_round_up(N, 32);
    if (arith == PRD_ARITH_SPLIT16) {
        const int tl = prd_ceil_div(N, TMS_T);
        const int vb3 = b * P * tl * tl;
        const size_t lds3 = (size_t)4 * TMS_OPER;
        launch_contract_split(tune, vb3 < 256 ? vb3 : 256, lds3, stream, O, AB, N, ldn, P, b, tl, 0);
    } else {
        const int tiles = prd_ceil_div(N, 64);
        const int vblocks = b * P * tiles * tiles;
        hipLaunchKernelGGL(tri_mul_contract_kernel, dim3(vblocks < 1024 ? vblocks : 1024), dim3(256), 0, stream, O, AB, N, ldn, P, b, tiles);
    }
    return (int)hipGetLastError();
}

extern "C" int prd_tri_mul_contract_scaled(float* O, const float* AB, const unsigned* a_amax, int b, int N, int P, int arith, hipStream_t stream) {
    if (!a_amax) return PRD_ERR_ARG;
    if ((arith & 0xff) != PRD_ARITH_SPLIT16) return prd_tri_mul_contract(O, AB, b, N, P, arith, stream);
    PRD_SPLIT_ARITH(arith);
    if (!O || !AB || b <= 0 || N <= 0) return PRD_ERR_ARG;
    if (P != 32 && P != 64 && P != 128) return PRD_ERR_UNSUPPORTED;
    const int ldn = prd_round_up(N, 32);
    const int tl = prd_ceil_div(N, TMS_T);
    const int vb3 = b * P * tl * tl;
    launch_contract_split(tune, vb3 < 256 ? vb3 : 256, (size_t)4 * TMS_OPER, stream, O, AB, N, ldn, P, b, tl, 0, a_amax);
    return (int)hipGetLastError();
}

extern "C" int prd_tri_mul_chain_supported(int N, int P, int arith) {
    return (N > 0 && (P == 32 || P == 64) && arith >= 0 && (arith & 0xff) == PRD_ARITH_SPLIT16) ? 1 : 0;
}

extern "C" int prd_tri_mul_chain(float* pair, const float* mask, const float* const* w_outgoing, const float* const* w_incoming,
                                 int b, int N, int P, float* ws, size_t ws_bytes, int arith, hipStream_t stream) {
    PRD_SPLIT_ARITH(arith);
    if (!pair || !mask || !w_outgoing || !w_incoming || !ws || b <= 0 || N <= 0) return PRD_ERR_ARG;
    for (int k = 0; k < 8; ++k)
        if (!w_outgoing[k] || !w_incoming[k]) return PRD_ERR_ARG;
    if (!prd_tri_mul_chain_supported(N, P, arith)) return PRD_ERR_UNSUPPORTED;
    if (ws_bytes < prd_workspace_bytes("tri_mul", b, N, 0, P)) return PRD_ERR_WORKSPACE;
    const int ldn = prd_round_up(N, 32);
    float* AB = ws;
    float* O = ws + (size_t)2 * b * P * N * ldn;
    const float* const* wa = w_outgoing;
    const float* const* wb = w_incoming;
    const size_t ldsp = ((size_t)2 * 2 * P * P + 4 * P) * sizeof(float);
    const long ptask = ((long)b * N * (ldn / 32) + 7) / 8 * 8 * (2 * P / 32);
    const int pgrid = grid_for(ptask, 4, 256);
    const int tl = prd_ceil_div(N, TMS_T);
    const int vb3 = b * P * tl * tl;
    const size_t lds3 = (size_t)4 * TMS_OPER;
    const long rtask = (long)b * N * (ldn / 32);
    const int rgrid = grid_for(rtask, 4, 256);
    const size_t ldsf = ((size_t)2 * P * P + (size_t)2 * 2 * P * P + 6 * P) * sizeof(float);
#define PRD_CHAIN_STAGE_OK() do { const hipError_t e_ = hipGetLastError(); if (e_ != hipSuccess) return (int)e_; } while (0)
    if (P == 64 && PRD_TGET_TMP_NW16(tune)) {
        PRD_SET_LDS((tri_mul_proj_kernel<64, 16, true>), ldsp);
        hipLaunchKernelGGL((tri_mul_proj_kernel<64, 16, true>), dim3(pgrid), dim3(16 * 64), ldsp, stream, (int*)nullptr, AB, pair, mask,
                           wa[0], wa[1], wa[2], wa[3], b, N, ldn, 0);
    } else if (P == 64) {
        PRD_SET_LDS((tri_mul_proj_kernel<64, 12, true>), ldsp);
        hipLaunchKernelGGL((tri_mul_proj_kernel<64, 12, true>), dim3(pgrid), dim3(12 * 64), ldsp, stream, (int*)nullptr, AB, pair, mask,
                           wa[0], wa[1], wa[2], wa[3], b, N, ldn, 0);
    } else {
        PRD_SET_LDS((tri_mul_proj_kernel<32, 12, true>), ldsp);
        hipLaunchKernelGGL((tri_mul_proj_kernel<32, 12, true>), dim3(pgrid), dim3(12 * 64), ldsp, stream, (int*)nullptr, AB, pair, mask,
                           wa[0], wa[1], wa[2], wa[3], b, N, ldn, 0);
    }
    PRD_CHAIN_STAGE_OK();
        launch_contract_split(tune, vb3 < 256 ? vb3 : 256, lds3, stream, O, AB, N, ldn, P, b, tl, 1);
    PRD_CHAIN_STAGE_OK();
    if (P == 64) {
        PRD_SET_LDS((tri_mul_out_proj_kernel<64, 12>), ldsf);
        hipLaunchKernelGGL((tri_mul_out_proj_kernel<64, 12>), dim3(rgrid), dim3(12 * 64), ldsf, stream, pair, O, mask, wa[4], wa[5], wa[6], wa[7],
                           wb[0], wb[1], wb[2], wb[3], AB, b, N, ldn);
    } else {
        PRD_SET_LDS((tri_mul_out_proj_kernel<32, 8>), ldsf);
        hipLaunchKernelGGL((tri_mul_out_proj_kernel<32, 8>), dim3(rgrid), dim3(8 * 64), ldsf, stream, pair, O, mask, wa[4], wa[5], wa[6], wa[7],
                           wb[0], wb[1], wb[2], wb[3], AB, b, N, ldn);
    }
    PRD_CHAIN_STAGE_OK();
        launch_contract_split(tune, vb3 < 256 ? vb3 : 256, lds3, stream, O, AB, N, ldn, P, b, tl, 0);
    PRD_CHAIN_STAGE_OK();
    {
        const long ntask = (long)b * N * prd_ceil_div(N, 32);
        const int grid = grid_for(ntask, 4, 256);
        if (P == 64) hipLaunchKernelGGL((tri_mul_out_kernel<64, 8, true>), dim3(grid), dim3(8 * 64), 0, stream, (int*)nullptr, pair, pair, O,
                                        wb[4], wb[5], wb[6], wb[7], b, N, ldn, 1);
        else hipLaunchKernelGGL((tri_mul_out_kernel<32, 8, true>), dim3(grid), dim3(8 * 64), 0, stream, (int*)nullptr, pair, pair, O,
                                wb[4], wb[5], wb[6], wb[7], b, N, ldn, 1);
    }
#undef PRD_CHAIN_STAGE_OK
    return (int)hipGetLastError();
}

extern "C" int prd_tri_attn_core(float* og, const float* pair, const float* mask, const float* wq, const float* wk,
                                 const float* wv, const float* wg, const float* bg, int ending,
                                 int b, int N, int P, int H, int c, int arith, hipStream_t stream) {
    PRD_SPLIT_ARITH(arith);
    if (!og || !pair || !mask || !wq || !wk || !wv || !wg || !bg || b <= 0 || N <= 0) return PRD_ERR_ARG;
    if ((P != 32 && P != 64) || c != 16 || H * c != 64) return PRD_ERR_UNSUPPORTED;
    const int npad = prd_round_up(N, 64);
    const int nqb = prd_ceil_div(N, 32);
    const bool split = arith == PRD_ARITH_SPLIT16;
    const int variant = PRD_FIRST_GEN ? PRD_TGET_TA_VARIANT(tune) : 0;
    if (split && variant == 0 && prd_tri_attn_v2_supported(N, P, tune) && (long)b * N * N <= 0x7fffffffL / 2)
        return prd_tri_attn_core_v2(og, pair, mask, wq, wk, wv, wg, bg, ending, b, N, P, H, c, tune, stream);
    const bool b3 = split && PRD_FIRST_GEN;
    bool long_row;
    const size_t lds = tri_attn_lds(N, P, b3, &long_row);
    if (lds > 160 * 1024) return PRD_ERR_UNSUPPORTED;
    const int nw = 8;
    const long rows_total = (long)b * N;
    const long cap = 256 / H;
    long per_head = cap < rows_total ? cap : rows_total;
    if (per_head < 1) per_head = 1;
    const long rounds = (rows_total + per_head - 1) / per_head;
    per_head = (rows_total + rounds - 1) / rounds;
    const int grid = (int)(per_head * H);
#define PRD_TA_LAUNCH(KERNEL, NWV, ...)                                                                                \
    do {                                                                                                               \
        PRD_SET_LDS((KERNEL<__VA_ARGS__>), lds);                                                                       \
        hipLaunchKernelGGL((KERNEL<__VA_ARGS__>), dim3(grid), dim3(NWV * 64), lds, stream, og, pair, mask, wq, wk, wv, wg, bg, b, N, npad, H, ending); \
    } while (0)
    (void)nqb; (void)nw;
    const bool split_long = long_row && b3 &&
        lds == (size_t)64 * P * 4 + (size_t)npad * 68 + (size_t)64 * (npad + 8) + 128 + 8 * 4096;
#ifdef PRD_AB
    if (split_long) { if (P == 64) PRD_TA_LAUNCH(tri_attn_core_split_long_kernel, 8, 64, 8); else PRD_TA_LAUNCH(tri_attn_core_split_long_kernel, 8, 32, 8); }
    else if (!long_row && b3) {
        if (P == 64) {
            if (variant == 1) PRD_TA_LAUNCH(tri_attn_core_split_kernel, 16, 64, 16, 1, false);
            else if (variant == 2) PRD_TA_LAUNCH(tri_attn_core_split_kernel, 12, 64, 12, 1, false);
            else if (variant == 3) PRD_TA_LAUNCH(tri_attn_core_split_kernel, 8, 64, 8, 1, true);
            else PRD_TA_LAUNCH(tri_attn_core_split_kernel, 8, 64, 8, 2, true);
        } else {
            PRD_TA_LAUNCH(tri_attn_core_split_kernel, 8, 32, 8, 2, true);
        }
    } else
#else
    (void)split_long; (void)variant;
#endif
    if (long_row) { if (P == 64) PRD_TA_LAUNCH(tri_attn_core_long_kernel, 8, 64, 8); else PRD_TA_LAUNCH(tri_attn_core_long_kernel, 8, 32, 8); }
    else { if (P == 64) PRD_TA_LAUNCH(tri_attn_core_kernel, 12, 64, 12, true, false); else PRD_TA_LAUNCH(tri_attn_core_kernel, 12, 32, 12, true, false); }
#undef PRD_TA_LAUNCH
    return (int)hipGetLastError();
}

extern "C" int prd_single_attn_core(float* o, const float* qkvg, int ldq, const float* bias, const float* mask,
                                    int b, int N, int H, int c, hipStream_t stream) {
    if (!o || !qkvg || !bias || b <= 0 || N <= 0) return PRD_ERR_ARG;
    if (c != 16 || H * c != 64) return PRD_ERR_UNSUPPORTED;
    if (ldq < 4 * H * c || (ldq & 3)) return PRD_ERR_ALIGN;
    hipLaunchKernelGGL(single_attn_core_kernel, dim3(b * H * prd_ceil_div(N, 16)), dim3(256), 0, stream, o, qkvg, bias, mask, b, N, H, ldq);
    return (int)hipGetLastError();
}

static size_t tri_attn_fused_lds(int N, int P) {
    bool long_row;
    const size_t lds = tri_attn_lds(N, P, true, &long_row);
    if (long_row) return (size_t)1 << 30;
    return lds + (size_t)P * 4 + (size_t)P * 256;
}

extern "C" int prd_tri_attn_core_fused_supported(int N, int P, int arith) {
    return (PRD_FIRST_GEN && N > 0 && (P == 32 || P == 64) && arith >= 0 && (arith & 0xff) == PRD_ARITH_SPLIT16 &&
            tri_attn_fused_lds(N, P) <= 160 * 1024) ? 1 : 0;
}

extern "C" int prd_tri_attn_core_fused(float* og, float* pair_out, const float* pair, const float* og_in, const float* wo_in,
                                       const float* bo_in, const float* mask, const float* wq, const float* wk, const float* wv,
                                       const float* wg, const float* bg, int ending, int b, int N, int P, int H, int c,
                                       hipStream_t stream) {
    if (!og || !pair_out || !pair || !og_in || !wo_in || !bo_in || !mask || !wq || !wk || !wv || !wg || !bg || b <= 0 || N <= 0 ||
        pair_out == pair) return PRD_ERR_ARG;
    if ((P != 32 && P != 64) || c != 16 || H * c != 64) return PRD_ERR_UNSUPPORTED;
    if (!prd_tri_attn_core_fused_supported(N, P, PRD_ARITH_SPLIT16)) return PRD_ERR_UNSUPPORTED;
    const int npad = prd_round_up(N, 64);
    const size_t lds = tri_attn_fused_lds(N, P);
    const long rows_total = (long)b * N;
    const long cap = 256 / H;
    long per_head = cap < rows_total ? cap : rows_total;
    if (per_head < 1) per_head = 1;
    const long rounds = (rows_total + per_head - 1) / per_head;
    per_head = (rows_total + rounds - 1) / rounds;
    const int grid = (int)(per_head * H);
#ifndef PRD_AB
    (void)grid; (void)lds; (void)npad;
    return PRD_ERR_UNSUPPORTED;
#else
    if (P == 64) {
        PRD_SET_LDS((tri_attn_core_split_kernel<64, 8, 2, true, true>), lds);
        hipLaunchKernelGGL((tri_attn_core_split_kernel<64, 8, 2, true, true>), dim3(grid), dim3(512), lds, stream, og, pair, mask, wq, wk, wv, wg,
                           bg, b, N, npad, H, ending, og_in, wo_in, bo_in, pair_out);
    } else {
        PRD_SET_LDS((tri_attn_core_split_kernel<32, 8, 2, true, true>), lds);
        hipLaunchKernelGGL((tri_attn_core_split_kernel<32, 8, 2, true, true>), dim3(grid), dim3(512), lds, stream, og, pair, mask, wq, wk, wv, wg,
                           bg, b, N, npad, H, ending, og_in, wo_in, bo_in, pair_out);
    }
    return (int)hipGetLastError();
#endif
}

extern "C" int prd_tri_attn_out(float* out, const float* pair, const float* og, const float* wo, const float* bo,
                                int residual, int b, int N, int P, int* queue, int arith, hipStream_t stream) {
    PRD_SPLIT_ARITH(arith);
    if (!out || !pair || !og || !wo || !bo || b <= 0 || N <= 0) return PRD_ERR_ARG;
    if (P != 32 && P != 64) return PRD_ERR_UNSUPPORTED;
    constexpr int NWA = 12;
    const long rows = (long)b * N * N;
    const int grid2 = grid_for((rows + 31) / 32, 4, 256);
    const bool b3 = arith == PRD_ARITH_SPLIT16;
#define PRD_TAO(PP, BB) hipLaunchKernelGGL((tri_attn_out_kernel<PP, NWA, BB>), dim3(grid2), dim3(NWA * 64), 0, stream, queue, out, pair, og, wo, bo, rows, residual)
    if (P == 64) { if (b3) PRD_TAO(64, true); else PRD_TAO(64, false); }
    else { if (b3) PRD_TAO(32, true); else PRD_TAO(32, false); }
#undef PRD_TAO
    return (int)hipGetLastError();
}

extern "C" int prd_tri_attn(float* out, const float* pair, const float* mask, const float* wq, const float* wk, const float* wv,
                            const float* wg, const float* bg, const float* wo, const float* bo, int ending, int residual,
                            int b, int N, int P, int H, int c, float* ws, size_t ws_bytes, int* queue, int arith, hipStream_t stream) {
    PRD_SPLIT_ARITH(arith);
    if (!ws) return PRD_ERR_ARG;
    if (ws_bytes < prd_workspace_bytes("tri_attn", b, N, 0, P)) return PRD_ERR_WORKSPACE;
    int e;
    if (prd_tri_attn_variant(N, P, arith_full) == 3) {
        const size_t nog = (size_t)b * N * N * 64;
        e = prd_tri_attn_core_chunked(ws, pair, mask, wq, wk, wv, wg, bg, ending, b, N, P, H, c, ws + nog, ws_bytes - nog * sizeof(float), stream);
    } else {
        e = prd_tri_attn_core(ws, pair, mask, wq, wk, wv, wg, bg, ending, b, N, P, H, c, arith_full, stream);
    }
    if (e) return e;
    return prd_tri_attn_out(out, pair, ws, wo, bo, residual, b, N, P, queue, arith_full, stream);
}
```

protein_redesign_amd/csrc/prd_tri2.hip:

```cpp
#include "prd_common.h"
#include "../../include/prd_hip.h"
#include <cstdlib>
#include <mutex>

#ifdef PRD_TIMING
__device__ unsigned long long prd_dbg2[256 * 12 * 8 * 16];
extern "C" int prd_debug_read2(void* dst) { return (int)hipMemcpyFromSymbol(dst, HIP_SYMBOL(prd_dbg2), sizeof(prd_dbg2)); }
#define PRD2_STAMP(k) do { if (lane == 0 && it < 8) prd_dbg2[((blockIdx.x * 12 + wave) * 8 + it) * 16 + (k)] = __builtin_readcyclecounter(); } while (0)
#else
#define PRD2_STAMP(k)
#endif

namespace {

constexpr float LOG2E_2 = 1.4426950408889634f;
constexpr float P_SHIFT = 4.0f;
constexpr int V2_MAXN = 384;
constexpr int PRD_V3_DEFAULT_KL = 0;

PRD_DEV f32x16 mfma_h(u32x4 a, u32x4 b, f32x16 c) {
    return __builtin_amdgcn_mfma_f32_32x32x16_f16(__builtin_bit_cast(f16x8_t, a), __builtin_bit_cast(f16x8_t, b), c, 0, 0, 0);
}

typedef _Float16 h16x2 __attribute__((ext_vector_type(2)));
// ... 507 lines not shown
#pragma unroll
                for (int k = 4; k >= 0; --k) {
                    has[k] = k == 0 ? own_t1 > 0 : (k - 1 < nhelp && qtile(m4 + k) > qtile(m4 + k - 1));
                    if (has[k]) kv = k;
                }
#pragma unroll
                for (int k = 0; k < 5; ++k) {
                    const float v_ = part[(size_t)(s0 + (has[k] ? k : kv)) * 640 + 9 * 64 + lane];
                    mm[k] = has[k] ? v_ : -INFINITY;
                }
                float M = mm[0];
#pragma unroll
                for (int k = 1; k < 5; ++k) M = max2f(M, mm[k]);
                float o[8], l = 0.f;
#pragma unroll
                for (int jj = 0; jj < 8; ++jj) o[jj] = 0.f;
#pragma unroll
                for (int k = 0; k < 5; ++k) {
                    const float* pp = part + (size_t)(s0 + (has[k] ? k : kv)) * 640 + lane;
                    const float scl = has[k] ? __builtin_amdgcn_exp2f(mm[k] - M) : 0.f;
                    l += scl * pp[8 * 64];
#pragma unroll
                    for (int jj = 0; jj < 8; ++jj) o[jj] += scl * pp[jj * 64];
                }
                finish(wave, o, l, M);
            }
        }
        PRD2_STAMP(5);
    }
}

struct V3Lds { unsigned buf0, bufsize, plane, bias, qs, gs, part; int nslot; };

PRD_DEV V3Lds v3_layout(int P, int NP) {
    V3Lds L;
    const int nqb = NP / 32, m4 = nqb & 3, nhelp = m4 ? 4 - m4 : 0;
    unsigned off = 64u * P * 4u;
    L.plane = (unsigned)NP * 16u;
    L.bufsize = 8u * L.plane + (unsigned)NP * 4u + 64u;
    L.buf0 = off; off += 2u * L.bufsize;
    L.bias = off; off += 64u;
    L.qs = off; off += 2u * (unsigned)m4 * 2048u;
    L.gs = off; off += 3u * (unsigned)m4 * 2048u;
    L.nslot = (nhelp + 1) * m4;
    L.part = off;
    return L;
}

template <int P, int NW, int KL, bool GV>
__global__ __launch_bounds__(NW * 64) void tri_attn_core_v3_kernel(
    float* __restrict__ og, const float* __restrict__ pair, const float* __restrict__ mask,
    const float* __restrict__ wq, const float* __restrict__ wk, const float* __restrict__ wv,
    const float* __restrict__ wg, const float* __restrict__ bg, int b, int N, int NP, int H, int ending, int flags,
    float* __restrict__ lse_out) {
    constexpr int C = 16, HC = 64, NT = NW * 64, KH = P / 2;
    constexpr float VSCALE = H2_WSCALE;
    extern __shared__ __attribute__((aligned(16))) unsigned char lds[];
#include "prd_tri2_v3_body.inc"
}

template <int P, int NW, int KL, bool GV>
PRD_DEV void tri_attn_core_v3_body(
    float* __restrict__ og, const float* __restrict__ pair, const float* __restrict__ mask,
    const float* __restrict__ wq, const float* __restrict__ wk, const float* __restrict__ wv,
    const float* __restrict__ wg, const float* __restrict__ bg, int b, int N, int NP, int H, int ending, int flags,
    float* __restrict__ lse_out, unsigned char* lds) {
    constexpr int C = 16, HC = 64, NT = NW * 64, KH = P / 2;
    constexpr float VSCALE = H2_WSCALE;
#include "prd_tri2_v3_body.inc"
}

constexpr unsigned PRD_SPIN_LIMIT = 1u << 22;

PRD_DEV bool spin_until_ge(unsigned* word, unsigned target, unsigned* tmo) {
    unsigned spins = 0;
    while (__hip_atomic_load(word, __ATOMIC_RELAXED, __HIP_MEMORY_SCOPE_AGENT) < target) {
        __builtin_amdgcn_s_sleep(2);
        if (++spins > PRD_SPIN_LIMIT) {
            __hip_atomic_store(tmo, 1u, __ATOMIC_RELAXED, __HIP_MEMORY_SCOPE_AGENT);
            return false;
        }
    }
    return true;
}

PRD_DEV void grid_barrier_counter(unsigned* bar, unsigned epoch) {
    asm volatile("s_waitcnt vmcnt(0)" ::: "memory");
    __syncthreads();
    if (threadIdx.x == 0) {
        __builtin_amdgcn_fence(__ATOMIC_RELEASE, "agent");
        asm volatile("s_waitcnt vmcnt(0)" ::: "memory");
        __hip_atomic_fetch_add(bar, 1u, __ATOMIC_RELAXED, __HIP_MEMORY_SCOPE_AGENT);
        spin_until_ge(bar, epoch * gridDim.x, bar + 1);
        __builtin_amdgcn_fence(__ATOMIC_ACQUIRE, "agent");
    }
    __syncthreads();
}

PRD_DEV unsigned xcc_id() {
    unsigned x;
    asm volatile("s_getreg_b32 %0, hwreg(HW_REG_XCC_ID)" : "=s"(x));
    return x & 7u;
}

PRD_DEV void grid_barrier_register(unsigned* bar, unsigned xcc) {
    if (threadIdx.x == 0) {
        __hip_atomic_fetch_add(bar + 8 + xcc, 1u, __ATOMIC_RELAXED, __HIP_MEMORY_SCOPE_AGENT);
        asm volatile("s_waitcnt vmcnt(0)" ::: "memory");
        __hip_atomic_fetch_add(bar + 2, 1u, __ATOMIC_RELAXED, __HIP_MEMORY_SCOPE_AGENT);
    }
}

PRD_DEV void grid_barrier_xcd(unsigned* bar, unsigned epoch, unsigned xcc) {
    asm volatile("s_waitcnt vmcnt(0)" ::: "memory");
    __syncthreads();
    if (threadIdx.x == 0) {
        unsigned* tmo = bar + 1;
        bool ok = spin_until_ge(bar + 2, gridDim.x, tmo);
        const unsigned mine = __hip_atomic_load(bar + 8 + xcc, __ATOMIC_RELAXED, __HIP_MEMORY_SCOPE_AGENT);
// ... 1004 lines not shown
            }
            __builtin_amdgcn_s_setprio(0);
            if (valid) {
                const float fv = __builtin_ldexpf(1.0f, -E - (int)B2_PSHIFT);
                const float fk = kover ? 0.f : fv * 0.6931471805599453f;
                float* dst = dqkvg + row_pos(v) * (4 * HC) + HC + h * C + 4 * hi;
                *reinterpret_cast<float4*>(dst) = make_float4(fk * (ok[0] + ok[8]), fk * (ok[1] + ok[9]), fk * (ok[2] + ok[10]), fk * (ok[3] + ok[11]));
                *reinterpret_cast<float4*>(dst + 8) = make_float4(fk * (ok[4] + ok[12]), fk * (ok[5] + ok[13]), fk * (ok[6] + ok[14]), fk * (ok[7] + ok[15]));
                *reinterpret_cast<float4*>(dst + HC) = make_float4(fv * (ov[0] + ov[8]), fv * (ov[1] + ov[9]), fv * (ov[2] + ov[10]), fv * (ov[3] + ov[11]));
                *reinterpret_cast<float4*>(dst + HC + 8) = make_float4(fv * (ov[4] + ov[12]), fv * (ov[5] + ov[13]), fv * (ov[6] + ov[14]), fv * (ov[7] + ov[15]));
            }
        }
    }
}

size_t v2l_lds_bytes(int N, int P, bool* share_out = nullptr) {
    const int NP = prd_round_up(N, 32), nqb = NP / 32, rem = nqb % 12, G = rem ? 12 / rem : 0;
    const size_t base = (size_t)64 * P * 4 + (size_t)NP * (2 * 32 + 64 + 4) + 128 + 64 + (size_t)V2L_TAIL_MAX * 128;
    const size_t extra = G >= 2 ? (size_t)rem * 2048 + 12 * 2560 : 0;
    const bool share = G >= 2 && base + extra <= 160 * 1024;
    if (share_out) *share_out = share;
    return base + (share ? extra : 0);
}

size_t v2_lds_bytes(int N, int P) {
    const int NP = prd_round_up(N, 32), nqb = NP / 32, m4 = nqb & 3;
    const size_t base = (size_t)64 * P * 4 + (size_t)NP * (4 * 32 + 64 + 64 + 4) + 128;
    return base + (size_t)(m4 ? m4 * (5 - m4) : 0) * 2560;
}

}

#define PRD2_SET_LDS(kernel)                                                                                    \
    do {                                                                                                        \
        static std::once_flag once;                                                                             \
        std::call_once(once, [] {                                                                               \
            (void)hipFuncSetAttribute((const void*)kernel, hipFuncAttributeMaxDynamicSharedMemorySize, 160 * 1024); \
        });                                                                                                     \
    } while (0)

extern "C" int prd_tri_attn_v2_supported(int N, int P, int tune) {
    if (N <= 0 || (P != 32 && P != 64)) return 0;
    if (N <= V2_MAXN) return v2_lds_bytes(N, P) <= 160 * 1024 ? 1 : 0;
    if (PRD_TGET_TA2_NO_LONG(tune)) return 0;
    return (prd_round_up(N, 32) <= 1024 && v2l_lds_bytes(N, P) <= 160 * 1024) ? 1 : 0;
}

extern "C" int prd_tri_attn_v2_form(int N, int P, int tune) {
    if (!prd_tri_attn_v2_supported(N, P, tune)) return 0;
    if (N > V2_MAXN) return 3;
    return (!PRD_TGET_TA2_NO_V3(tune) && v3_lds_bytes(N, P) <= 160 * 1024) ? 2 : 1;
}

extern "C" int prd_tri_attn_core_v2_lse(float* og, float* lse, const float* pair, const float* mask, const float* wq, const float* wk,
                                        const float* wv, const float* wg, const float* bg, int ending,
                                        int b, int N, int P, int H, int c, int tune, hipStream_t stream) {
    if (!og || !pair || !mask || !wq || !wk || !wv || !wg || !bg || b <= 0 || N <= 0 || tune < 0) return PRD_ERR_ARG;
    if ((P != 32 && P != 64) || c != 16 || H * c != 64) return PRD_ERR_UNSUPPORTED;
    if (!prd_tri_attn_v2_supported(N, P, tune)) return PRD_ERR_UNSUPPORTED;
    if (lse && N > V2_MAXN) return PRD_ERR_UNSUPPORTED;
    if ((long)b * N * N > 0x7fffffffL / 2) return PRD_ERR_UNSUPPORTED;
    const int NP = prd_round_up(N, 32);
    const bool long_rows = N > V2_MAXN;
    bool share = false;
    const size_t lds = long_rows ? v2l_lds_bytes(N, P, &share) : v2_lds_bytes(N, P);
    const long rows_total = (long)b * N;
    const long cap = 256 / H;
    long per_head = cap < rows_total ? cap : rows_total;
    if (per_head < 1) per_head = 1;
    const long rounds = (rows_total + per_head - 1) / per_head;
    per_head = (rows_total + rounds - 1) / rounds;
    if (per_head >= 8 && !((tune >> 20) & 1)) per_head = (per_head + 7) / 8 * 8;
    if (per_head > cap) per_head = cap;
    const int grid = (int)(per_head * H);
    constexpr int NWV = 12;
    const int flags_env = PRD_TGET_TA2_FLAGS(tune);
    const int use_v3 = !PRD_TGET_TA2_NO_V3(tune);
    const bool v3 = !long_rows && use_v3 && v3_lds_bytes(N, P) <= 160 * 1024;
    const int flags0 = flags_env >= 0 ? flags_env : (v3 ? 0 : 1);
    const int nqb_ = NP / 32, rem_ = nqb_ % 12;
    const int ntail_ = N - 32 * (nqb_ - 1);
    const bool tail1 = long_rows && nqb_ >= 2 && ntail_ >= 1 && ntail_ <= V2L_TAIL_MAX && !PRD_TGET_TA2_NO_GV(tune) && !(flags0 & 2);
    const int flags = flags0 | ((long_rows && rem_ && 12 / rem_ >= 2 && !share) ? 16 : 0) | (PRD_TGET_TA2_NO_TAIL_SPLIT(tune) ? 32 : 0)
                      | (tail1 ? 64 : 0) | ((long_rows && (flags0 & 4)) ? 128 : 0);
    if (long_rows) {
#define PRD_V2L_LAUNCH(PP, PF, GVF)                                                                                               \
        do {                                                                                                                      \
            PRD2_SET_LDS((tri_attn_core_v2l_kernel<PP, NWV, PF, GVF>));                                                           \
            hipLaunchKernelGGL((tri_attn_core_v2l_kernel<PP, NWV, PF, GVF>), dim3(grid), dim3(NWV * 64), lds, stream, og, pair, mask, wq, wk, \
                               wv, wg, bg, b, N, NP, H, ending, flags);                                                           \
        } while (0)
        const bool pf = (flags & 8) != 0;
        const bool gvl = !PRD_TGET_TA2_NO_GV(tune);
#ifdef PRD_AB
        if (P == 64) {
            if (gvl) { if (pf) PRD_V2L_LAUNCH(64, true, true); else PRD_V2L_LAUNCH(64, false, true); }
            else { if (pf) PRD_V2L_LAUNCH(64, true, false); else PRD_V2L_LAUNCH(64, false, false); }
        } else {
            if (gvl) { if (pf) PRD_V2L_LAUNCH(32, true, true); else PRD_V2L_LAUNCH(32, false, true); }
            else { if (pf) PRD_V2L_LAUNCH(32, true, false); else PRD_V2L_LAUNCH(32, false, false); }
        }
#else
        (void)pf; (void)gvl;
        if (P == 64) PRD_V2L_LAUNCH(64, false, true); else PRD_V2L_LAUNCH(32, false, true);
#endif
#undef PRD_V2L_LAUNCH
        return (int)hipGetLastError();
    }
    if (v3) {
        const size_t lds3 = v3_lds_bytes(N, P);
#define PRD_V3_LAUNCH(PP, KLF, GVF)                                                                                                 \
        do {                                                                                                                      \
            PRD2_SET_LDS((tri_attn_core_v3_kernel<PP, NWV, KLF, GVF>));                                                           \
            hipLaunchKernelGGL((tri_attn_core_v3_kernel<PP, NWV, KLF, GVF>), dim3(grid), dim3(NWV * 64), lds3, stream, og, pair, mask, wq, wk, wv, wg, \
                               bg, b, N, NP, H, ending, flags & ~6, lse);                                                         \
        } while (0)
        const int kl = flags_env >= 0 ? (flags >> 1) & 3 : PRD_V3_DEFAULT_KL;
        const bool gvf = !PRD_TGET_TA2_NO_GV(tune) && kl == 0;
#ifdef PRD_AB
        if (P == 64) {
            if (gvf) PRD_V3_LAUNCH(64, 0, true);
            else if (kl == 0) PRD_V3_LAUNCH(64, 0, false); else if (kl == 1) PRD_V3_LAUNCH(64, 1, false); else if (kl == 2) PRD_V3_LAUNCH(64, 2, false); else PRD_V3_LAUNCH(64, 3, false);
        } else {
            if (gvf) PRD_V3_LAUNCH(32, 0, true);
            else if (kl == 0) PRD_V3_LAUNCH(32, 0, false); else if (kl == 1) PRD_V3_LAUNCH(32, 1, false); else if (kl == 2) PRD_V3_LAUNCH(32, 2, false); else PRD_V3_LAUNCH(32, 3, false);
        }
#else
        (void)gvf;
        if (P == 64) PRD_V3_LAUNCH(64, 0, true); else PRD_V3_LAUNCH(32, 0, true);
#endif
#undef PRD_V3_LAUNCH
        return (int)hipGetLastError();
    }
    if (P == 64) {
        PRD2_SET_LDS((tri_attn_core_v2_kernel<64, NWV>));
        hipLaunchKernelGGL((tri_attn_core_v2_kernel<64, NWV>), dim3(grid), dim3(NWV * 64), lds, stream, og, pair, mask, wq, wk, wv, wg, bg, b, N,
                           NP, H, ending, flags, lse);
    } else {
        PRD2_SET_LDS((tri_attn_core_v2_kernel<32, NWV>));
        hipLaunchKernelGGL((tri_attn_core_v2_kernel<32, NWV>), dim3(grid), dim3(NWV * 64), lds, stream, og, pair, mask, wq, wk, wv, wg, bg, b, N,
                           NP, H, ending, flags, lse);
    }
    return (int)hipGetLastError();
}

extern "C" int prd_tri_attn_core_v2(float* og, const float* pair, const float* mask, const float* wq, const float* wk,
                                    const float* wv, const float* wg, const float* bg, int ending,
                                    int b, int N, int P, int H, int c, int tune, hipStream_t stream) {
    return prd_tri_attn_core_v2_lse(og, nullptr, pair, mask, wq, wk, wv, wg, bg, ending, b, N, P, H, c, tune, stream);
}

static int prd_cu_count() {
    static int cus = 0;
    static std::once_flag once;
    std::call_once(once, [] {
        int dev = 0, n = 0;
        if (hipGetDevice(&dev) == hipSuccess && hipDeviceGetAttribute(&n, hipDeviceAttributeMultiprocessorCount, dev) == hipSuccess) cus = n;
    });
    return cus;
}

extern "C" int prd_tri_attn_pair_supported(int N, int P, int arith) {
    PRD_SPLIT_ARITH(arith);
    if (N <= 0 || (P != 32 && P != 64) || arith != PRD_ARITH_SPLIT16) return 0;
    if (N > V2_MAXN || PRD_TGET_TA2_NO_V3(tune) || PRD_TGET_TA2_NO_GV(tune) || PRD_TGET_TA2_FLAGS(tune) >= 0) return 0;
    return v3_lds_bytes(N, P) <= 160 * 1024 ? 1 : 0;
}

extern "C" int prd_tri_attn_pair(float* og, float* pair, const float* mask, const float* const* w_start, const float* const* w_end,
                                 int b, int N, int P, int H, int c, unsigned* bar, int arith, hipStream_t stream) {
    if (!og || !pair || !mask || !w_start || !w_end || !bar || b <= 0 || N <= 0 || arith < 0) return PRD_ERR_ARG;
    const int tune = arith >> 8;
    for (int k = 0; k < 7; ++k) if (!w_start[k]) return PRD_ERR_ARG;
    for (int k = 0; k < 5; ++k) if (!w_end[k]) return PRD_ERR_ARG;
    if (c != 16 || H * c != 64) return PRD_ERR_UNSUPPORTED;
    if (!prd_tri_attn_pair_supported(N, P, arith)) return PRD_ERR_UNSUPPORTED;
    if ((long)b * N * N > 0x7fffffffL / 2) return PRD_ERR_UNSUPPORTED;
    const int NP = prd_round_up(N, 32);
    const long rows_total = (long)b * N, cap = 256 / H;
    long per_head = cap < rows_total ? cap : rows_total;
    if (per_head < 1) per_head = 1;
    const long rounds = (rows_total + per_head - 1) / per_head;
    per_head = (rows_total + rounds - 1) / rounds;
    if (per_head >= 8) per_head = (per_head + 7) / 8 * 8;
    if (per_head > cap) per_head = cap;
    const int grid = (int)(per_head * H);
    const int cus = prd_cu_count();
    if (cus <= 0 || grid > cus) return PRD_ERR_UNSUPPORTED;
    const size_t lds3 = v3_lds_bytes(N, P);
    const size_t ldso = (size_t)P * 64 * 4 + (size_t)P * 4;
    const size_t lds = lds3 > ldso ? lds3 : ldso;
    hipError_t e = hipMemsetAsync(bar, 0, 32 * sizeof(unsigned), stream);
    const int plain = PRD_TGET_TA2_NO_TAIL_SPLIT(tune) ? 1 : 0;
    if (e != hipSuccess) return (int)e;
    constexpr int NWV = 12;
    if (P == 64) {
        PRD2_SET_LDS((tri_attn_pair_kernel<64, NWV>));
        hipLaunchKernelGGL((tri_attn_pair_kernel<64, NWV>), dim3(grid), dim3(NWV * 64), lds, stream, og, pair, mask, w_start[0], w_start[1], w_start[2],
                           w_start[3], w_start[4], w_start[5], w_start[6], w_end[0], w_end[1], w_end[2], w_end[3], w_end[4], b, N, NP, H, bar, plain);
    } else {
        PRD2_SET_LDS((tri_attn_pair_kernel<32, NWV>));
        hipLaunchKernelGGL((tri_attn_pair_kernel<32, NWV>), dim3(grid), dim3(NWV * 64), lds, stream, og, pair, mask, w_start[0], w_start[1], w_start[2],
// ... 37 lines not shown
```

protein_redesign_amd/csrc/prd_tri2_v3_body.inc:

```
    const V3Lds L = v3_layout(P, NP);
    u32x4* Wb = reinterpret_cast<u32x4*>(lds);
    float* biasl = reinterpret_cast<float*>(lds + L.bias);
    const int tid = threadIdx.x, lane = tid & 63;
    const int wave = __builtin_amdgcn_readfirstlane(tid >> 6);
    const int r = lane & 31, hi = lane >> 5;
    const int nqb = NP / 32;
    const int rstride = gridDim.x / H;
    int h, slot;
    if ((rstride & 7) == 0) {
        const int xcd = blockIdx.x & 7, idx = blockIdx.x >> 3;
        h = idx % H;
        slot = (idx / H) * 8 + xcd;
    } else {
        h = blockIdx.x % H;
        slot = blockIdx.x / H;
    }
    const float sc = 0.25f * LOG2E_2;
    stage_weight_h2_rows<P>(Wb, 64, 0, wk + (long)h * C * P, C, P, tid, NT, H2_WSCALE);
    stage_weight_h2_rows<P>(Wb, 64, C, wq + (long)h * C * P, C, P, tid, NT, sc * H2_WSCALE);
    stage_weight_h2_rows<P>(Wb, 64, 2 * C, wg + (long)h * C * P, C, P, tid, NT, NEG_LOG2E * H2_WSCALE);
    stage_weight_h2_rows<P>(Wb, 64, 3 * C, wv + (long)h * C * P, C, P, tid, NT, H2_WSCALE);
    if (tid < 16) {
        const int hh = tid >> 3, e = tid & 7;
        biasl[tid] = H2_WSCALE * NEG_LOG2E * bg[h * C + 4 * hh + (e & 3) + 8 * (e >> 2)];
// ... 338 lines not shown
                    const float alpha = __builtin_amdgcn_exp2f(m_run - m_new);
                    m_run = m_new;
                    mref = m_new - P_SHIFT;
                    lsum *= alpha;
#pragma unroll
                    for (int e = 0; e < 16; ++e) { o0[e] *= alpha; s[e] -= mref; }
                    bool dummy = false;
                    PBuf p;
                    ldv(t, p);
                    exp_split(s, lsum, dummy, p);
                    pv_tile(p, o0);
                }
            }
#pragma unroll
            for (int jj = 0; jj < 8; ++jj) o8[jj] = o0[jj] + o0[jj + 8];
            work_rem -= T1 - T0;
        };
        auto put_partial = [&](int pslot, const float (&o8)[8], float lsum, float mref) {
            float* pp = reinterpret_cast<float*>(lds + L.part) + ((size_t)par * L.nslot + pslot) * 640 + lane;
#pragma unroll
            for (int jj = 0; jj < 8; ++jj) pp[jj * 64] = o8[jj];
            pp[8 * 64] = lsum;
            pp[9 * 64] = mref;
        };
        if (owner) {
            float o8[8], lsum = 0.f, mref = 0.f;
            if (remap && group_owner) {
                const unsigned qo = L.qs + (unsigned)(par * m4 + gi) * 2048u + (unsigned)hi * 512u + (unsigned)r * 16u;
                qh4 = *reinterpret_cast<const u32x4*>(lds + qo);
                ql4 = *reinterpret_cast<const u32x4*>(lds + qo + 1024u);
            }
            if (own_t1 > 0) run_piece(qh4, ql4, 0, own_t1, o8, lsum, mref);
            if (!group_owner) finish(rcur, wave, o8, lsum, gate, mref);
            else if (own_t1 > 0) put_partial((nhelp + 1) * gi, o8, lsum, mref);
        } else if (helper) {
            for (int i = 0; i < m4; ++i) {
                const int pc = (flags & 32) ? hj : (hj + i) % nhelp;
                const int T0 = qtile(m4 + pc), T1 = qtile(m4 + pc + 1);
                if (T1 <= T0) continue;
                const unsigned qo = L.qs + (unsigned)(par * m4 + i) * 2048u + (unsigned)hi * 512u + (unsigned)r * 16u;
                const u32x4 qh = *reinterpret_cast<const u32x4*>(lds + qo), ql = *reinterpret_cast<const u32x4*>(lds + qo + 1024u);
                float o8[8], lsum, mref;
                run_piece(qh, ql, T0, T1, o8, lsum, mref);
                put_partial((nhelp + 1) * i + 1 + pc, o8, lsum, mref);
            }
        }
        set_sprio();
        PRD2_STAMP(2);
        rprev = rcur;
        const int bun = bu + rstride;
        if (bun < nrows) {
            rcur = make_row(bun);
            phase1(rcur, par ^ 1, gpar == 2 ? 0 : gpar + 1);
        }
        PRD2_STAMP(4);
        gpar = gpar == 2 ? 0 : gpar + 1;
    }
    if (it > 0 && m4 > 0) {
        __syncthreads();
        if (group_owner) merge(rprev, (it - 1) & 1, gpar == 0 ? 2 : gpar - 1);
    }
```

protein_redesign_amd/ops.py:

```python
from __future__ import annotations

import math
import os
from typing import Mapping, Optional, Tuple

import torch

from ._lib import PrdGemm, arithmetic, check, dptr, lib, stream

F32 = torch.float32


_QUEUES = {}


def task_queue(device) -> int:
    import os
    if not os.environ.get("PRD_TASK_QUEUE"):
        return 0
    key = torch.device(device).index if torch.device(device).index is not None else torch.cuda.current_device()
    q = _QUEUES.get(key)
    if q is None:
        q = _QUEUES[key] = torch.zeros(256, dtype=torch.int32, device=f"cuda:{key}")
    return q.data_ptr()


class SideStream:

    def __init__(self, device):
        import os
        self.enabled = os.environ.get("PRD_SIDE_STREAM", "0") == "1"
        self.stream = torch.cuda.Stream(device=device) if self.enabled else None

    def fork(self):
        import contextlib
        if not self.enabled:
            return contextlib.nullcontext()
        self.stream.wait_stream(torch.cuda.current_stream())
        return torch.cuda.stream(self.stream)

    def join(self):
        if self.enabled:
            torch.cuda.current_stream().wait_stream(self.stream)


def _off(t, elem_offset: int = 0) -> int:
    return (t if isinstance(t, int) else dptr(t)) + 4 * elem_offset


def round_up(a: int, b: int) -> int:
    return (a + b - 1) // b * b


def gemm(A, B, Cout, M, N, K, lda, ldb, ldc, *, a_off=0, b_off=0, c_off=0, G1=1, G2=1,
         sa=(0, 0), sb=(0, 0), sc=(0, 0), b_kn=False, alpha=1.0, bias=None, act=0, act_from=0,
         addmat=None, sad=(0, 0), ldadd=0, colmask=None, scm1=0, fill=0.0, rowmask=None, srm1=0,
         mulmat=None, mul_off=0, smu=(0, 0), ldmul=0, resid=None, res_off=0, sr=(0, 0), ldr=0,
         colscale=None, tile_hint=0, a_ln=False, ln_out=None, c2=None, n_split=0, rowmask_cols=0, rscale=None,
         slab=False, wsum=None, out_ln=None, a_scale=0.0, mul_pos=False, a_amax=None, unsupported_ok=False):
    g = PrdGemm()
# ... 155 lines not shown
                              stream()), "prd_pair_bias")
    return out


def pair_bias2(pair, set_a, set_b):
    b, N, _, P = pair.shape
    (wa, ba, ga, bea), (wb, bb, gb, beb) = set_a, set_b
    Ha, Hb = wa.shape[0], wb.shape[0]
    oa = torch.empty(b, Ha, N, N, device=pair.device, dtype=F32)
    ob = torch.empty(b, Hb, N, N, device=pair.device, dtype=F32)
    check(lib().prd_pair_bias2(dptr(oa), dptr(pair), dptr(ga), dptr(bea), dptr(wa), dptr(ba), Ha,
                               dptr(ob), dptr(gb), dptr(beb), dptr(wb), dptr(bb), Hb, b, N, P, stream()), "prd_pair_bias2")
    return oa, ob


def opm_pair(pair, ab, mask, w_out, b_out, *, residual: bool, apply_mask: bool, out=None) -> torch.Tensor:
    b, N, _, P = pair.shape
    Cc = ab.shape[-1] // 2
    if out is None:
        out = torch.empty_like(pair)
    flags = (1 if residual else 0) | (2 if apply_mask else 0)
    check(lib().prd_opm_pair(dptr(out), dptr(pair), dptr(ab), dptr(mask), dptr(w_out), dptr(b_out), flags,
                             b, N, P, Cc, stream()), "prd_opm_pair")
    return out


def row_block(t: torch.Tensor):
    if t.dim() != 3 or t.stride(-1) != 1 or t.stride(0) != t.shape[1] * t.stride(1) or not t.is_cuda or t.dtype != F32:
        raise RuntimeError("expected a CUDA fp32 [b, N, C] tensor or a column block of one")
    if (t.storage_offset() | t.stride(1)) & 3:
        raise RuntimeError("column block must start on a 16-byte boundary and have a row pitch that is a multiple of 4 floats")
    return t.data_ptr(), t.stride(1)


def pair_head_supported(P: int, dist_dim: int, C: int) -> bool:
    return lib().prd_pair_head_supported(P, dist_dim, C) == 1


def pair_head(static_pair_t, z, mask, centers, w_dist, ebeta, ab, w_out, b_out, *, apply_mask: bool, set_a, set_b, out=None):
    b, N, _, P = static_pair_t.shape
    (wa, ba, ga, bea), (wb, bb_, gb, beb) = set_a, set_b
    Ha, Hb = wa.shape[0], wb.shape[0]
    if out is None:
        out = torch.empty_like(static_pair_t)
    oa = torch.empty(b, Ha, N, N, device=out.device, dtype=F32)
    ob = torch.empty(b, Hb, N, N, device=out.device, dtype=F32)
    check(lib().prd_pair_head(dptr(out), dptr(static_pair_t), dptr(z), dptr(mask), dptr(centers), dptr(w_dist), dptr(ebeta),
                              w_dist.shape[1], dptr(ab), dptr(w_out), dptr(b_out), ab.shape[-1] // 2, int(apply_mask),
                              dptr(oa), dptr(ga), dptr(bea), dptr(wa), dptr(ba), Ha, dptr(ob), dptr(gb), dptr(beb), dptr(wb), dptr(bb_), Hb,
                              b, N, P, stream()), "prd_pair_head")
    return out, oa, ob


def outer_linear_pair(pair, x, u, w, bias, *, residual: bool, out=None) -> torch.Tensor:
    b, N, _, P = pair.shape
    if out is None:
        out = torch.empty_like(pair)
    up, ldu = row_block(u)
    check(lib().prd_outer_linear(dptr(out), dptr(pair), dptr(x), up, ldu, dptr(w), dptr(bias), int(residual),
                                 b, N, P, x.shape[-1], task_queue(pair.device), stream()), "prd_outer_linear")
    return out


def workspace_bytes(op: str, b: int, N: int, S: int, P: int) -> int:
    return int(lib().prd_workspace_bytes(op.encode(), b, N, S, P))


def tri_mul(pair, mask, wts, *, incoming: bool, residual: bool, out=None, ws=None) -> torch.Tensor:
    b, N, _, P = pair.shape
    if out is None:
        out = torch.empty_like(pair)
    nbytes = workspace_bytes("tri_mul", b, N, 0, P)
    if ws is None:
        ws = torch.empty(nbytes // 4, device=pair.device, dtype=F32)
    check(lib().prd_tri_mul(dptr(out), dptr(pair), dptr(mask), *[dptr(w) for w in wts], int(incoming), int(residual),
                            b, N, P, dptr(ws), ws.numel() * 4, task_queue(pair.device), stream()), "prd_tri_mul")
    return out


def tri_mul_chain_supported(N: int, P: int) -> bool:
    return lib().prd_tri_mul_chain_supported(N, P) == 1


def tri_mul_chain_(pair, mask, wts_outgoing, wts_incoming, ws=None) -> torch.Tensor:
    import ctypes
    b, N, _, P = pair.shape
    nbytes = workspace_bytes("tri_mul", b, N, 0, P)
    if ws is None:
        ws = torch.empty(nbytes // 4, device=pair.device, dtype=F32)
    arr = ctypes.c_void_p * 8
    wa = arr(*[dptr(w) for w in wts_outgoing])
    wb = arr(*[dptr(w) for w in wts_incoming])
    check(lib().prd_tri_mul_chain(dptr(pair), dptr(mask), ctypes.cast(wa, ctypes.c_void_p), ctypes.cast(wb, ctypes.c_void_p),
                                  b, N, P, dptr(ws), ws.numel() * 4, stream()), "prd_tri_mul_chain")
    return pair


PERSISTENT_ATTN = os.environ.get("PRD_PERSISTENT_ATTN", "0") == "1"
_PAIR_BARS = {}


def tri_attn_pair_supported(N: int, P: int) -> bool:
    return lib().prd_tri_attn_pair_supported(N, P) == 1


def tri_attn_pair_bar(device) -> torch.Tensor:
    key = torch.device(device).index if torch.device(device).index is not None else torch.cuda.current_device()
    bar = _PAIR_BARS.get(key)
    if bar is None:
        bar = _PAIR_BARS[key] = torch.zeros(32, dtype=torch.int32, device=f"cuda:{key}")
    return bar


def tri_attn_pair_(pair, mask, wts_start, wts_end, H: int, c: int, og=None) -> torch.Tensor:
    import ctypes
    b, N, _, P = pair.shape
    if og is None:
        og = torch.empty(b, N, N, 64, device=pair.device, dtype=F32)
    wa = (ctypes.c_void_p * 7)(*[dptr(w) for w in wts_start])
    wb = (ctypes.c_void_p * 5)(*[dptr(w) for w in wts_end])
    bar = tri_attn_pair_bar(pair.device)
    check(lib().prd_tri_attn_pair(dptr(og), dptr(pair), dptr(mask), ctypes.cast(wa, ctypes.c_void_p), ctypes.cast(wb, ctypes.c_void_p),
                                  b, N, P, H, c, bar.data_ptr(), stream()), "prd_tri_attn_pair")
    return og


def tri_attn_pair_timed_out(device) -> bool:
    return int(tri_attn_pair_bar(device)[1].item()) != 0


def tri_mul_backward(dy, pair, mask, wts, *, incoming: bool, ws=None):
    wp, bp, wg, bg, wo, bo, wog, bog = wts
    b, N, _, P = pair.shape
    ldn = round_up(N, 32)
    dev = pair.device
    unit = b * P * N * ldn
    if ws is None:
        ws = torch.empty(3 * unit, device=dev, dtype=F32)
        scratch = torch.empty_like(pair)
        check(lib().prd_tri_mul(dptr(scratch), dptr(pair), dptr(mask), *[dptr(w) for w in wts], int(incoming), 0, b, N, P,
                                dptr(ws), ws.numel() * 4, 0, stream()), "prd_tri_mul (recompute)")
    AB = ws[:2 * unit].view(b, 2 * P, N, ldn)
    O = ws[2 * unit:].view(b, P, N, ldn)
    dy = dy.contiguous()
    dz, dgp, dx1 = torch.empty_like(pair), torch.empty_like(pair), torch.empty_like(pair)
    x, lo = torch.empty_like(pair), torch.empty_like(pair)
    ops4 = torch.empty(b, 4 * P, N, ldn, device=dev, dtype=F32)
# ... 245 lines not shown
    if bad:
        raise ValueError(f"model widths {', '.join(bad)} do not run on the GPU; supported: {MODEL_WIDTHS}")


def step_boundary_fusable(time_dim: int) -> bool:
    return 0 < time_dim <= 512 and time_dim % 2 == 0


def tri_attn_heads_supported(N: int, P: int, H: int, c: int) -> bool:
    return lib().prd_tri_attn_heads_supported(N, P, H, c) == 1


def tri_attn_heads_ws_floats(b: int, N: int, P: int, H: int, c: int) -> int:
    return int(lib().prd_tri_attn_heads_workspace_bytes(b, N, P, H, c)) // 4


def tri_attn_core_heads(pair, mask, wts, H: int, c: int, *, ending: bool, ws=None, lse=None) -> torch.Tensor:
    b, N, _, P = pair.shape
    check_head_layout(H, c, P)
    need = tri_attn_heads_ws_floats(b, N, P, H, c)
    if ws is None or ws.numel() < need:
        ws = torch.empty(need, device=pair.device, dtype=F32)
    og = ws[:b * N * N * H * c].view(b, N, N, H * c)
    if lse is not None:
        if lse.numel() != b * N * H * N * 2:
            raise ValueError("tri_attn_core_heads: lse must be [b*N, H, N, 2]")
        check(lib().prd_tri_attn_core_heads_lse(dptr(og), dptr(lse), dptr(pair), dptr(mask), *[dptr(w) for w in wts], int(ending), b, N, P,
                                                H, c, dptr(ws), ws.numel() * 4, stream()), "prd_tri_attn_core_heads_lse")
        return og
    check(lib().prd_tri_attn_core_heads(dptr(og), dptr(pair), dptr(mask), *[dptr(w) for w in wts], int(ending), b, N, P, H, c,
                                        dptr(ws), ws.numel() * 4, stream()), "prd_tri_attn_core_heads")
    return og


def tri_attn_bwd_heads_supported(N: int, P: int, H: int, c: int) -> bool:
    return lib().prd_tri_attn_bwd_heads_supported(N, P, H, c) == 1


def tri_attn_bwd_core_heads(dog, og, pair, mask, wts, H: int, c: int, *, ending: bool, lse=None, x_out=None, dqkvg=None, ws=None):
    b, N, _, P = pair.shape
    HC = H * c
    check_head_layout(H, c, P)
    if dqkvg is None:
        dqkvg = torch.empty(b, N, N, 4, HC, device=pair.device, dtype=F32)
    need = int(lib().prd_tri_attn_bwd_heads_workspace_bytes(b, N, P, H, c)) // 4
    if ws is None or ws.numel() < need:
        ws = torch.empty(need, device=pair.device, dtype=F32)
    check(lib().prd_tri_attn_bwd_core_heads(dptr(dqkvg), dptr(dog), dptr(og), dptr(pair), dptr(mask), *[dptr(w) for w in wts], dptr(lse),
                                            dptr(x_out), int(ending), b, N, P, H, c, dptr(ws), ws.numel() * 4, stream()),
          "prd_tri_attn_bwd_core_heads")
    return dqkvg


def tri_attn(pair, mask, wts, H: int, c: int, *, ending: bool, residual: bool, out=None, ws=None) -> torch.Tensor:
    b, N, _, P = pair.shape
    if not default_head_layout(H, c):
        og = tri_attn_core_heads(pair, mask, wts[:5], H, c, ending=ending, ws=ws)
        return linear(og, wts[5], wts[6], resid=pair if residual else None, out=out)
    if out is None:
        out = torch.empty_like(pair)
    nbytes = workspace_bytes("tri_attn", b, N, 0, P)
    if ws is None:
        ws = torch.empty(nbytes // 4, device=pair.device, dtype=F32)
    check(lib().prd_tri_attn(dptr(out), dptr(pair), dptr(mask), *[dptr(w) for w in wts], int(ending), int(residual),
                             b, N, P, H, c, dptr(ws), ws.numel() * 4, task_queue(pair.device), stream()), "prd_tri_attn")
    return out


def pair_transition(pair, w1, b1, w2, b2, *, residual: bool, out=None) -> torch.Tensor:
    b, N, _, P = pair.shape
    if out is None:
        out = torch.empty_like(pair)
    check(lib().prd_pair_transition(dptr(out), dptr(pair), dptr(w1), dptr(b1), dptr(w2), dptr(b2), int(residual),
                                    b, N, P, task_queue(pair.device), stream()), "prd_pair_transition")
    return out


def block_tail_(pair, og, wo, bo, w1, b1, w2, b2, bias_w=None, bias_b=None) -> Optional[torch.Tensor]:
    b, N, _, P = pair.shape
    bias_out = None
    H = 0
    if bias_w is not None:
        H = bias_w.shape[0]
        bias_out = torch.empty(b, H, N, N, device=pair.device, dtype=F32)
    check(lib().prd_block_tail(dptr(pair), dptr(og), dptr(wo), dptr(bo), dptr(w1), dptr(b1), dptr(w2), dptr(b2),
                               dptr(bias_w), dptr(bias_b), dptr(bias_out), b, N, P, H, task_queue(pair.device), stream()),
          "prd_block_tail")
    return bias_out


def coord_head(pair, z, mask, w1, b1, w2) -> torch.Tensor:
    b, N, _, P = pair.shape
    out = torch.empty(b, N, 3, device=pair.device, dtype=F32)
    check(lib().prd_coord_head(dptr(out), dptr(pair), dptr(z), dptr(mask), dptr(w1), dptr(b1), dptr(w2), b, N, P,
                               stream()), "prd_coord_head")
    return out


def remove_mean(x, mask) -> torch.Tensor:
    b, N, D = x.shape
    out = torch.empty_like(x)
    check(lib().prd_remove_mean(dptr(out), dptr(x), dptr(mask), b, N, D, stream()), "prd_remove_mean")
    return out


def reverse_update_(z, seq_t, t, noise_pred, seq_pred, noise, mask, coef, num_steps: int):
    b, N, _ = z.shape
    check(lib().prd_reverse_update(dptr(z), dptr(seq_t), dptr(t, torch.int64), dptr(noise_pred), dptr(seq_pred),
                                   dptr(noise), dptr(mask), dptr(coef), b, N, seq_pred.shape[-1], num_steps, stream()),
          "prd_reverse_update")


def step_boundary_(z, seq_t, t, eps_raw, seq_pred, noise, mask, coef, num_steps: int, single_next, static_single, residue_mask,
                   w_rt, ebeta_next, freqs, w_beta, sync, seq_h=None, w_seq=None):
    b, N, _ = z.shape
    P, TD = w_beta.shape
    hp, ldh = row_block(seq_h) if seq_h is not None else (None, 0)
    check(lib().prd_step_boundary(dptr(z), dptr(seq_t), dptr(t, torch.int64), dptr(eps_raw), dptr(seq_pred), dptr(noise), dptr(mask),
                                  dptr(coef), dptr(single_next), dptr(static_single), dptr(residue_mask), dptr(w_rt),
                                  dptr(ebeta_next), dptr(freqs), dptr(w_beta), dptr(sync, torch.int32), b, N, seq_pred.shape[-1],
                                  num_steps, static_single.shape[-1], P, TD, hp, ldh, dptr(w_seq),
                                  (seq_h.shape[-1] if seq_h is not None else 0), stream()), "prd_step_boundary")


def tri_attn_stats_floats(b: int, N: int, P: int, H: int = 4) -> int:
    return lib().prd_tri_attn_stats_bytes(b, N, P, H) // 4


def tri_attn_lse_supported(N: int, P: int) -> bool:
    return (lib().prd_get_gemm_mode() == 1 and lib().prd_tri_attn_v2_form(N, P) in (1, 2)
            and lib().prd_tri_attn_bwd_core_v2_supported(N, P) == 1 and TRI_ATTN_BWD_V2)


def tri_attn_core(pair, mask, wts, H: int, c: int, *, ending: bool, og=None, stats=None, lse=None) -> torch.Tensor:
    b, N, _, P = pair.shape
    if og is None:
        og = torch.empty(b, N, N, 64, device=pair.device, dtype=F32)
    if lse is not None:
        if not tri_attn_lse_supported(N, P) or lse.numel() != b * N * H * N * 2:
            raise ValueError("tri_attn_core: lse is kept by the split-16 short-row kernels only, as [b*N, H, N, 2]")
        check(lib().prd_tri_attn_core_v2_lse(dptr(og), dptr(lse), dptr(pair), dptr(mask), *[dptr(w) for w in wts], int(ending),
                                             b, N, P, H, c, stream()), "prd_tri_attn_core_v2_lse")
        return og
    nst = tri_attn_stats_floats(b, N, P, H)
    if nst:
        if stats is None:
            stats = torch.empty(nst, device=pair.device, dtype=F32)
        if stats.numel() < nst:
            raise ValueError("tri_attn_core: stats buffer too small")
        check(lib().prd_tri_attn_core_chunked(dptr(og), dptr(pair), dptr(mask), *[dptr(w) for w in wts], int(ending),
                                              b, N, P, H, c, dptr(stats), stats.numel() * 4, stream()), "prd_tri_attn_core_chunked")
        return og
    check(lib().prd_tri_attn_core(dptr(og), dptr(pair), dptr(mask), *[dptr(w) for w in wts], int(ending),
                                  b, N, P, H, c, stream()), "prd_tri_attn_core")
    return og


def tri_attn_v2_supported(N: int, P: int) -> bool:
    return lib().prd_tri_attn_v2_supported(N, P) == 1


def tri_attn_core_v2(pair, mask, wts, H: int, c: int, *, ending: bool, og=None) -> torch.Tensor:
    b, N, _, P = pair.shape
    if og is None:
        og = torch.empty(b, N, N, 64, device=pair.device, dtype=F32)
    check(lib().prd_tri_attn_core_v2(dptr(og), dptr(pair), dptr(mask), *[dptr(w) for w in wts], int(ending),
                                     b, N, P, H, c, stream()), "prd_tri_attn_core_v2")
    return og


def tri_attn_core_v2_lse(pair, mask, wts, H: int, c: int, *, ending: bool, lse, og=None) -> torch.Tensor:
    b, N, _, P = pair.shape
    if og is None:
        og = torch.empty(b, N, N, 64, device=pair.device, dtype=F32)
    check(lib().prd_tri_attn_core_v2_lse(dptr(og), dptr(lse), dptr(pair), dptr(mask), *[dptr(w) for w in wts], int(ending),
                                         b, N, P, H, c, stream()), "prd_tri_attn_core_v2_lse")
    return og


def tri_attn_core_fused_supported(N: int, P: int) -> bool:
    return lib().prd_tri_attn_core_fused_supported(N, P) == 1


def tri_attn_core_fused(pair, og_in, wo_in, bo_in, mask, wts, H: int, c: int, *, ending: bool, pair_out, og=None) -> torch.Tensor:
    b, N, _, P = pair.shape
    if og is None:
        og = torch.empty(b, N, N, 64, device=pair.device, dtype=F32)
    check(lib().prd_tri_attn_core_fused(dptr(og), dptr(pair_out), dptr(pair), dptr(og_in), dptr(wo_in), dptr(bo_in), dptr(mask),
                                        *[dptr(w) for w in wts], int(ending), b, N, P, H, c, stream()), "prd_tri_attn_core_fused")
    return og


def tri_attn_out(pair, og, wo, bo, *, residual: bool, out=None) -> torch.Tensor:
    b, N, _, P = pair.shape
    if out is None:
        out = torch.empty_like(pair)
    check(lib().prd_tri_attn_out(dptr(out), dptr(pair), dptr(og), dptr(wo), dptr(bo), int(residual), b, N, P,
                                 task_queue(pair.device), stream()), "prd_tri_attn_out")
    return out



def cached_pack(module, name: str, params, build):
    key = tuple((p.data_ptr(), p._version) for p in params)
    cache = module.__dict__.setdefault("_prd_pack_cache", {})
    hit = cache.get(name)
    if hit is None or hit[0] != key:
# ... 126 lines not shown
```

protein_redesign_amd/trunk.py:

```python
from __future__ import annotations

import os

import math
from argparse import Namespace
from typing import Mapping, Optional, Tuple

import torch
from torch import nn

from . import ops
from .af2_blocks import OuterProductUpdate, SPAttention

_VARIANCE_INITS = {
    "default": (1.0, "fan_in", "truncated_normal"),
    "relu": (2.0, "fan_in", "truncated_normal"),
    "glorot": (1.0, "fan_avg", "uniform"),
    "normal": (1.0, "fan_in", "normal"),
}
_TRUNC_STD_CORRECTION = 0.87962566103423978


def _variance_scaling_(weight: torch.Tensor, scale: float, mode: str, distribution: str) -> None:
    fan_out, fan_in = weight.shape
# ... 28 lines not shown

    def forward(self, x: torch.Tensor) -> torch.Tensor:
        return ops.linear(x.contiguous(), self.weight, self.bias)


def _node_mask(mask_2d: torch.Tensor) -> torch.Tensor:
    return torch.diagonal(mask_2d, dim1=-2, dim2=-1).contiguous()


class Attention(nn.Module):

    def __init__(self, embed_dim: int, head_dim: int, num_heads: int):
        super().__init__()
        self.embed_dim, self.head_dim, self.num_heads = embed_dim, head_dim, num_heads
        self.scale = 1.0 / math.sqrt(head_dim)
        self.inf = 2.0 ** 15
        self.norm = nn.LayerNorm(embed_dim, elementwise_affine=False)
        self.q_proj = Linear(embed_dim, num_heads * head_dim, bias=False, init="glorot")
        self.k_proj = Linear(embed_dim, num_heads * head_dim, bias=False, init="glorot")
        self.v_proj = Linear(embed_dim, num_heads * head_dim, bias=False, init="glorot")
        self.gate_proj = Linear(embed_dim, num_heads * head_dim, init="gating")
        self.out_proj = Linear(num_heads * head_dim, embed_dim, init="final")

    def weights(self):
        return (self.q_proj.weight, self.k_proj.weight, self.v_proj.weight, self.gate_proj.weight,
                self.gate_proj.bias, self.out_proj.weight, self.out_proj.bias)

    def packed(self):
        ws = self.weights()[:5]
        return ops.cached_pack(self, "qkvg", ws, lambda: ops.pack_attention(*ws, self.scale))

    def run_single(self, x, mask, attn_bias, resid, ln_a=False, qkvg=None):
        return ops.gated_attention_single(x, mask, attn_bias, self.packed(), self.out_proj.weight, self.out_proj.bias,
                                          self.num_heads, self.head_dim, key_mask=True, resid=resid, ln_a=ln_a, qkvg=qkvg)

    def forward(self, x: torch.Tensor, mask: torch.Tensor, attn_bias: Optional[torch.Tensor] = None) -> torch.Tensor:
        if x.dim() != 3:
            raise RuntimeError("Attention.forward expects [b, N, E]; use TriangleAttention for pair rows")
        b, N, _ = x.shape
        if attn_bias is None:
            attn_bias = torch.zeros(b, self.num_heads, N, N, device=x.device, dtype=torch.float32)
        return self.run_single(x.contiguous(), mask.contiguous(), attn_bias.contiguous(), None, ln_a=True)


class TriangleAttention(nn.Module):

    def __init__(self, pair_dim: int, head_dim: int, num_heads: int, mode: str):
        super().__init__()
        if mode not in ("starting", "ending"):
            raise ValueError(f"Invalid mode: {mode}")
        self.attn = Attention(pair_dim, head_dim, num_heads)
        self.mode = mode

    def run(self, pair, mask, *, residual: bool, out=None, ws=None):
        a = self.attn
        return ops.tri_attn(pair, mask, a.weights(), a.num_heads, a.head_dim, ending=self.mode == "ending",
                            residual=residual, out=out, ws=ws)

    def forward(self, pair: torch.Tensor, mask_2d: torch.Tensor) -> torch.Tensor:
        return self.run(pair.contiguous(), _node_mask(mask_2d), residual=False)


class TriangleMultiplication(nn.Module):

    def __init__(self, pair_dim: int, mode: str):
        super().__init__()
        if mode not in ("outgoing", "incoming"):
            raise ValueError(f"Invalid mode: {mode}")
        self.mode = mode
        self.norm = nn.LayerNorm(pair_dim, elementwise_affine=False)
        self.ab_proj = Linear(pair_dim, pair_dim * 2, init="default")
        self.ab_gate = Linear(pair_dim, pair_dim * 2, init="gating")
        self.ab_norm = nn.LayerNorm(pair_dim, elementwise_affine=False)
        self.out_proj = Linear(pair_dim, pair_dim, init="final")
        self.out_gate = Linear(pair_dim, pair_dim, init="gating")

    def weights(self):
        return (self.ab_proj.weight, self.ab_proj.bias, self.ab_gate.weight, self.ab_gate.bias,
                self.out_proj.weight, self.out_proj.bias, self.out_gate.weight, self.out_gate.bias)

    def run(self, pair, mask, *, residual: bool, out=None, ws=None):
        return ops.tri_mul(pair, mask, self.weights(), incoming=self.mode == "incoming", residual=residual, out=out, ws=ws)

    def forward(self, pair: torch.Tensor, mask_2d: torch.Tensor) -> torch.Tensor:
        return self.run(pair.contiguous(), _node_mask(mask_2d), residual=False)


_TRI_MUL_CHAIN = os.environ.get("PRD_TRI_MUL_CHAIN", "1") != "0"
_TRI_ATTN_FUSE = os.environ.get("PRD_TRI_ATTN_FUSE", "0") == "1"
_PAIR_HEAD = os.environ.get("PRD_PAIR_HEAD", "1") != "0"
_MERGE_HEAD = os.environ.get("PRD_MERGE_HEAD", "1") != "0"
_HEAD_SLAB = os.environ.get("PRD_HEAD_SLAB", "0") == "1"
_MERGE_PROJ = os.environ.get("PRD_MERGE_PROJ", "1") != "0"
_FOLD_OUT_PROJ = os.environ.get("PRD_FOLD_OUT_PROJ", "1") != "0"


class OuterLinear(nn.Module):

    def __init__(self, single_dim: int, pair_dim: int):
        super().__init__()
        self.single_dim, self.pair_dim = single_dim, pair_dim
        self.norm = nn.LayerNorm(single_dim, elementwise_affine=False)
        self.linear = Linear(single_dim * 2, pair_dim, init="final")

    def run(self, single, pair, *, residual: bool, out=None):
        b, N, S = single.shape
        w = self.linear.weight
        u = torch.empty(b, N, self.pair_dim, device=single.device, dtype=torch.float32)
        if ops.ln_fusable(S):
            x = torch.empty_like(single)
# ... 54 lines not shown
                w, pb, cs = sa.packed()
                dev = w.device
                return (torch.cat([w_ol[:, S:], w]).contiguous(), torch.cat([torch.zeros(P, device=dev), pb]).contiguous(),
                        torch.cat([torch.ones(P, device=dev), cs]).contiguous())
            return ops.cached_pack(self, "after_transition_next", ws, build), 2, P + 3 * sa.num_heads * sa.head_dim
        if tail is not None:
            tw, tb = tail
            ws = (w_ol, tw, tb)

            def build():
                dev = tw.device
                return (torch.cat([w_ol[:, S:], tw]).contiguous(), torch.cat([torch.zeros(P, device=dev), tb]).contiguous(), None)
            return ops.cached_pack(self, "after_transition_tail", ws, build), 1, P
        return None, 0, 0

    def single_track_(self, single, mask, bias, next_block=None, qkvg=None, tail=None, extra=None):
        sa = self.single_attn
        b, N, S = single.shape
        fc = self.single_fc
        HC, Hd = sa.num_heads * sa.head_dim, fc[1].weight.shape[0]
        if _FOLD_OUT_PROJ and single.is_cuda and sa.head_dim == 16 and ops.fc1_fold_ok(b * N, S, HC, Hd):
            if qkvg is None:
                qkvg = ops.project_qkvg(single, sa.packed(), HC, ln_a=True)
            og = ops.single_attn_core(qkvg, mask, bias, sa.num_heads, sa.head_dim)
            wo, bo = sa.out_proj.weight, sa.out_proj.bias
            pack = ops.cached_pack(self, "fc1_fold", (wo, bo, fc[1].weight), lambda: ops.pack_fc1_fold(wo, bo, fc[1].weight))
            single, xhat = ops.transition_single_folded(single, og, pack, bo, fc[1].bias, fc[3].weight, fc[3].bias, want_ln=True)
        else:
            single = sa.run_single(single, mask, bias, single, ln_a=True, qkvg=qkvg)
            wsum1 = ops.cached_pack(self, "fc1_rowsum", (fc[1].weight,), lambda: fc[1].weight.double().sum(1).float().contiguous())
            single, xhat = ops.transition_single(single, fc[1].weight, fc[1].bias, fc[3].weight, fc[3].bias, residual=True, wsum1=wsum1,
                                                 want_ln=True)
        packed, act, act_from = self._after_transition_pack(next_block if extra is not None else None, tail if extra is not None else None)
        if packed is None or not _MERGE_PROJ:
            return single, None, None
        P = self.outer_linear.pair_dim
        x, cat = ops.project_many(single, packed, P, act=act, act_from=act_from, xhat=xhat)
        extra["qkvg" if next_block is not None else "tail"] = cat[..., P:]
        return single, x, cat[..., :P]

    def run_(self, single: torch.Tensor, pair: torch.Tensor, mask: torch.Tensor, ws=None, bias=None, next_block=None, spare_holder=None,
             qkvg=None, tail=None, extra=None):
        sa = self.single_attn
        b, N = mask.shape
        ta = self.pair_attn_ending.attn
        general = not ops.default_head_layout(ta.num_heads, ta.head_dim)
        if general and pair.is_cuda:
            ops.check_head_layout(ta.num_heads, ta.head_dim, pair.shape[-1])
        if ws is None:
            ws = torch.empty(ws_floats(b, N, pair.shape[-1], ta.num_heads, ta.head_dim), device=pair.device, dtype=torch.float32)
        if bias is None:
            bias = ops.pair_bias(pair, self.attn_bias[1].weight, self.attn_bias[1].bias)
        single, x, u = self.single_track_(single, mask, bias, next_block=next_block, qkvg=qkvg, tail=tail, extra=extra)
        if u is not None:
            ol = self.outer_linear.linear
            ops.outer_linear_pair(pair, x, u, ol.weight, ol.bias, residual=True, out=pair)
        else:
            self.outer_linear.run(single, pair, residual=True, out=pair)
        if _TRI_MUL_CHAIN and ops.tri_mul_chain_supported(N, pair.shape[-1]):
            ops.tri_mul_chain_(pair, mask, self.pair_mul_outgoing.weights(), self.pair_mul_incoming.weights(), ws=ws)
        else:
            self.pair_mul_outgoing.run(pair, mask, residual=True, out=pair, ws=ws)
            self.pair_mul_incoming.run(pair, mask, residual=True, out=pair, ws=ws)
        pf = self.pair_fc
        nb_w = next_block.attn_bias[1].weight if next_block is not None else None
        nb_b = next_block.attn_bias[1].bias if next_block is not None else None
        if general:
            self.pair_attn_starting.run(pair, mask, residual=True, out=pair, ws=ws)
            og = ops.tri_attn_core_heads(pair, mask, ta.weights()[:5], ta.num_heads, ta.head_dim, ending=True, ws=ws)
            if og.shape[-1] == 64:
                next_bias = ops.block_tail_(pair, og, ta.out_proj.weight, ta.out_proj.bias, pf[1].weight, pf[1].bias,
                                            pf[3].weight, pf[3].bias, nb_w, nb_b)
            else:
                ops.linear(og, ta.out_proj.weight, ta.out_proj.bias, resid=pair, out=pair)
                ops.pair_transition(pair, pf[1].weight, pf[1].bias, pf[3].weight, pf[3].bias, residual=True, out=pair)
                next_bias = ops.pair_bias(pair, nb_w, nb_b) if nb_w is not None else None
            return single, pair, next_bias
        nog = b * N * N * 64
        if _TRI_ATTN_FUSE and ops.tri_attn_core_fused_supported(N, pair.shape[-1]) and ws.numel() >= 2 * nog:
            ts = self.pair_attn_starting.attn
            og_s = ops.tri_attn_core(pair, mask, ts.weights()[:5], ts.num_heads, ts.head_dim, ending=False,
                                     og=ws[:nog].view(b, N, N, 64))
            spare = spare_holder[0] if spare_holder else None
            if spare is None:
                spare = torch.empty_like(pair)
            og = ops.tri_attn_core_fused(pair, og_s, ts.out_proj.weight, ts.out_proj.bias, mask, ta.weights()[:5], ta.num_heads,
                                         ta.head_dim, ending=True, pair_out=spare, og=ws[nog: 2 * nog].view(b, N, N, 64))
            pair, spare = spare, pair
            if spare_holder is not None:
                spare_holder[0] = spare
        elif ops.PERSISTENT_ATTN and ops.tri_attn_pair_supported(N, pair.shape[-1]):
            ts = self.pair_attn_starting.attn
            og = ops.tri_attn_pair_(pair, mask, ts.weights(), ta.weights()[:5], ta.num_heads, ta.head_dim, og=ws[:nog].view(b, N, N, 64))
        else:
            self.pair_attn_starting.run(pair, mask, residual=True, out=pair, ws=ws)
            og = ops.tri_attn_core(pair, mask, ta.weights()[:5], ta.num_heads, ta.head_dim, ending=True,
                                   og=ws[:nog].view(b, N, N, 64), stats=ws[nog:] if ws.numel() > nog else None)
        next_bias = ops.block_tail_(pair, og, ta.out_proj.weight, ta.out_proj.bias, pf[1].weight, pf[1].bias,
                                    pf[3].weight, pf[3].bias, nb_w, nb_b)
        return single, pair, next_bias

    def forward(self, single: torch.Tensor, pair: torch.Tensor, mask: torch.Tensor) -> Tuple[torch.Tensor, torch.Tensor]:
        single, pair, _ = self.run_(single.contiguous(), pair.contiguous().clone(), mask.contiguous())
        return single, pair


def ws_floats(b: int, N: int, P: int, H: int, c: int) -> int:
    att = ops.workspace_bytes("tri_attn", b, N, 0, P) // 4 if ops.default_head_layout(H, c) else ops.tri_attn_heads_ws_floats(b, N, P, H, c)
    return max(ops.workspace_bytes("tri_mul", b, N, 0, P) // 4, att)


class Denoiser(nn.Module):

    def __init__(self, args):
        super().__init__()
        if isinstance(args, Mapping):
            args = Namespace(**args)
        self.single_dim, self.esm_dim, self.pair_dim = args.single_dim, args.esm_dim, args.pair_dim
        self.head_dim, self.num_heads = args.head_dim, args.num_heads
        self.transition_factor, self.num_blocks = args.transition_factor, args.num_blocks
        self.n_recycles = args.n_recycles
        self.SPAAttnBlock = SPAttention(c_in=self.single_dim, c_hidden=self.single_dim, no_heads=self.num_heads,
                                        pair_bias=True, c_z=self.pair_dim)
        self.opm = OuterProductUpdate(c_m=self.single_dim, c_z=self.pair_dim, c_hidden=self.single_dim // 4)
        self.folding_blocks = nn.ModuleList(
            [FoldingBlock(self.single_dim, self.pair_dim, self.head_dim, self.num_heads, self.transition_factor)
             for _ in range(self.num_blocks)])

    def ws_floats(self, b: int, N: int) -> int:
        return ws_floats(b, N, self.pair_dim, self.num_heads, self.head_dim)

    def project_single(self, single: torch.Tensor, mask: torch.Tensor):
        if not _MERGE_HEAD or not ops.ln_fusable(single.shape[-1]):
            ab = self.opm.project(single, mask)
            mn, qkvg = self.SPAAttnBlock.project(single)
            return ab, mn, qkvg, False
        opm, spa = self.opm, self.SPAAttnBlock
        a = spa.mha
        params = (opm.layer_norm.weight, opm.layer_norm.bias, opm.linear_1.weight, opm.linear_1.bias, opm.linear_2.weight,
                  opm.linear_2.bias, spa.layer_norm_m.weight, spa.layer_norm_m.bias, a.linear_q.weight, a.linear_k.weight,
                  a.linear_v.weight, a.linear_g.weight, a.linear_g.bias)

        def build():
            go, bo, w1, b1, w2, b2, gs, bs, wq, wk, wv, wg, bg = [p.detach().double() for p in params]
            scale = 1.0 / math.sqrt(spa.c_hidden)
            w = torch.cat([w1 * go, w2 * go, wq * gs, wk * gs, wv * gs, wg * gs])
            bias = torch.cat([b1 + w1 @ bo, b2 + w2 @ bo, (wq @ bs) * scale, wk @ bs, wv @ bs, bg + wg @ bs])
            cs = torch.cat([torch.ones(2 * opm.c_hidden, dtype=torch.float64, device=w.device),
                            torch.full((wq.shape[0],), scale, dtype=torch.float64, device=w.device),
                            torch.ones(3 * wq.shape[0], dtype=torch.float64, device=w.device)])
# ... 73 lines not shown
```

Before: 588.7 denoising-steps/s.

## Prefetch next kernel's weights into cache from tail waves of current kernel

Adds a warm-hint mechanism: several pair-track kernels (outer linear, tri-mul chain, tri-attn out, tri-attn core) take a list of the next op's weight buffers and, once a wave reaches its last task or has no work, touch those buffers one cache line at a time. The aim is to hide the cold weight fetch at the start of each following kernel behind the tail of the current one. The cost is extra loads and waits in tail waves, extra kernel arguments, and wasted traffic if the lines are evicted before the next kernel runs. It is on by default through PRD_WARM_NEXT and only applies in the non-general, no-grad path.

Measured after the change: 584.7 denoising-steps/s. About the same (-0.7%).

```diff
diff --git a/include/prd_hip.h b/include/prd_hip.h
--- a/include/prd_hip.h
+++ b/include/prd_hip.h
@@ -239,6 +239,28 @@
                                 const float* lse, float* x_out, int ending, int b, int N, int P, int H, int c,
                                 float* ws, size_t ws_bytes, int arith, hipStream_t stream);
 
+#define PRD_WARM_MAX 8
+typedef struct prd_warm {
+    int n;
+    const void* ptr[PRD_WARM_MAX];
+    size_t bytes[PRD_WARM_MAX];
+} prd_warm;
+int prd_outer_linear_warm(float* out, const float* pair, const float* x, const float* u, int ldu, const float* w,
+                          const float* bias, int residual, int b, int N, int P, int S, int* queue, const prd_warm* next,
+                          int arith, hipStream_t stream);
+int prd_tri_mul_chain_warm(float* pair, const float* mask, const float* const* w_outgoing, const float* const* w_incoming,
+                           int b, int N, int P, float* ws, size_t ws_bytes, const prd_warm* next, int arith, hipStream_t stream);
+int prd_tri_attn_warm(float* out, const float* pair, const float* mask, const float* wq, const float* wk, const float* wv,
+                      const float* wg, const float* bg, const float* wo, const float* bo, int ending, int residual,
+                      int b, int N, int P, int H, int c, float* ws, size_t ws_bytes, int* queue, const prd_warm* next,
+                      int arith, hipStream_t stream);
+int prd_tri_attn_core_warm(float* og, const float* pair, const float* mask, const float* wq, const float* wk,
+                           const float* wv, const float* wg, const float* bg, int ending,
+                           int b, int N, int P, int H, int c, const prd_warm* next, int arith, hipStream_t stream);
+int prd_tri_attn_core_v2_warm(float* og, const float* pair, const float* mask, const float* wq, const float* wk,
+                              const float* wv, const float* wg, const float* bg, int ending,
+                              int b, int N, int P, int H, int c, const prd_warm* next, int tune, hipStream_t stream);
+
 size_t prd_workspace_bytes(const char* op, int b, int N, int S, int P);
 
 #ifdef __cplusplus
diff --git a/protein_redesign_amd/_lib.py b/protein_redesign_amd/_lib.py
--- a/protein_redesign_amd/_lib.py
+++ b/protein_redesign_amd/_lib.py
@@ -39,6 +39,13 @@
         ("mul_pos", ci),
         ("a_amax", vp),
     ]
+
+
+WARM_MAX = 8
+
+
+class PrdWarm(C.Structure):
+    _fields_ = [("n", ci), ("ptr", vp * WARM_MAX), ("bytes", cz * WARM_MAX)]
 
 
 SIGNATURES = {
@@ -119,6 +126,11 @@
     "prd_tri_attn_bwd_heads_supported": [ci] * 5,
     "prd_tri_attn_bwd_heads_workspace_bytes": [ci] * 5,
     "prd_tri_attn_bwd_core_heads": [vp] * 12 + [ci] * 6 + [vp, cz, ci, vp],
+    "prd_outer_linear_warm": [vp] * 4 + [ci] + [vp] * 2 + [ci] * 5 + [vp, C.POINTER(PrdWarm), ci, vp],
+    "prd_tri_mul_chain_warm": [vp, vp, vp, vp, ci, ci, ci, vp, cz, C.POINTER(PrdWarm), ci, vp],
+    "prd_tri_attn_warm": [vp] * 10 + [ci] * 7 + [vp, cz, vp, C.POINTER(PrdWarm), ci, vp],
+    "prd_tri_attn_core_warm": [vp] * 8 + [ci] * 6 + [C.POINTER(PrdWarm), ci, vp],
+    "prd_tri_attn_core_v2_warm": [vp] * 8 + [ci] * 6 + [C.POINTER(PrdWarm), ci, vp],
 }
 
 GEMM_MODES = {"fp32": 0, "split16": 1, "bf16x3": 1}
@@ -127,12 +139,13 @@
 _ARITH_BEFORE_STREAM = ("prd_coord_head", "prd_pair_head", "prd_pair_init", "prd_opm_pair", "prd_outer_linear", "prd_tri_mul", "prd_tri_mul_contract", "prd_tri_mul_contract_scaled", "prd_tri_mul_proj_bwd",
                         "prd_tri_attn", "prd_tri_attn_core", "prd_tri_attn_out", "prd_pair_transition", "prd_block_tail", "prd_tri_mul_chain",
                         "prd_linear_wgrad", "prd_pair_linear", "prd_spa_attn_core", "prd_tri_attn_pair",
-                        "prd_tri_attn_core_heads", "prd_tri_attn_core_heads_lse", "prd_tri_attn_bwd_core_heads", "prd_single_fc1_folded")
+                        "prd_tri_attn_core_heads", "prd_tri_attn_core_heads_lse", "prd_tri_attn_bwd_core_heads", "prd_single_fc1_folded",
+                        "prd_outer_linear_warm", "prd_tri_mul_chain_warm", "prd_tri_attn_warm", "prd_tri_attn_core_warm")
 _ARITH_LAST = ("prd_tri_attn_variant", "prd_tri_mul_chain_supported", "prd_tri_attn_core_fused_supported", "prd_tri_attn_stats_bytes",
                "prd_gemm_slab_ok", "prd_pair_head_supported", "prd_pair_linear_supported", "prd_spa_attn_core_supported",
                "prd_tri_attn_pair_supported", "prd_tri_attn_heads_supported",
                "prd_tri_attn_bwd_heads_supported", "prd_single_fc1_folded_ok")
-_TUNE_BEFORE_STREAM = ("prd_tri_attn_core_v2", "prd_tri_attn_core_v2_lse")
+_TUNE_BEFORE_STREAM = ("prd_tri_attn_core_v2", "prd_tri_attn_core_v2_lse", "prd_tri_attn_core_v2_warm")
 _TUNE_LAST = ("prd_tri_attn_v2_supported", "prd_tri_attn_v2_form")
 
 
diff --git a/protein_redesign_amd/csrc/prd_common.h b/protein_redesign_amd/csrc/prd_common.h
--- a/protein_redesign_amd/csrc/prd_common.h
+++ b/protein_redesign_amd/csrc/prd_common.h
@@ -1,6 +1,7 @@
 #pragma once
 #include <hip/hip_runtime.h>
 #include <stdint.h>
+#include "../../include/prd_hip.h"
 
 typedef float f32x16 __attribute__((ext_vector_type(16)));
 typedef float f32x4 __attribute__((ext_vector_type(4)));
@@ -547,6 +548,7 @@
         const int wgs = (int)((gridDim.x - shard + nshard - 1) / nshard);
         last = count + wgs * waves_per_wg - 1;
     }
+    PRD_DEV bool is_last() const { return !q && (long)__builtin_amdgcn_readfirstlane((int)cur) >= ntask; }
     PRD_DEV long next() {
         if (!q) {
             const long t = (long)__builtin_amdgcn_readfirstlane((int)cur);
@@ -562,6 +564,40 @@
         return t < count ? (long)t * nshard + shard : -1;
     }
 };
+
+constexpr int PRD_WARM_K = 8;
+struct PrdWarmK {
+    const char* p[PRD_WARM_K];
+    unsigned bytes[PRD_WARM_K];
+    int n;
+};
+PRD_DEV void warm_touch(const PrdWarmK& w) {
+    if (w.n <= 0) return;
+    const unsigned nrank = gridDim.x >= 8 ? gridDim.x >> 3 : 1u, rank = blockIdx.x >> 3;
+    if (rank >= nrank) return;
+    const unsigned lane = threadIdx.x & 63;
+    for (unsigned base = 0;; base += 64) {
+        const unsigned idx = base + lane;
+        const char* addr = nullptr;
+        unsigned acc = 0;
+        for (int k = 0; k < w.n; ++k) {
+            const unsigned bytes = w.bytes[k], lines = (bytes + 127u) >> 7;
+            const unsigned lo = (unsigned)((unsigned long long)lines * rank / nrank);
+            const unsigned hi = (unsigned)((unsigned long long)lines * (rank + 1) / nrank);
+            const unsigned cnt = hi - lo + ((rank == nrank - 1 && bytes >= 4) ? 1u : 0u);
+            if (idx >= acc && idx < acc + cnt) {
+                const unsigned l = lo + (idx - acc);
+                addr = w.p[k] + (l < hi ? (size_t)l << 7 : (size_t)bytes - 4);
+            }
+            acc += cnt;
+        }
+        if (addr) {
+            unsigned t;
+            asm volatile("global_load_dword %0, %1, off\n\ts_waitcnt vmcnt(0)" : "=&v"(t) : "v"(addr) : "memory");
+        }
+        if (base + 64 >= acc) break;
+    }
+}
 
 #define PRD_SPLIT_ARITH(a)                                                                       \
     const int arith_full = (a);                                                                  \
@@ -580,5 +616,21 @@
 #define PRD_TGET_OL_GEN2(t) (((t) >> 12) & 1)
 #define PRD_TGET_TMS_NW(t) ((((t) >> 13) & 3) == 1 ? 12 : (((t) >> 13) & 3) == 2 ? 16 : 8)
 
+static inline int prd_warm_to_k(const prd_warm* w, PrdWarmK* k) {
+    *k = PrdWarmK{};
+    if (!w) return 0;
+    if (w->n < 0 || w->n > PRD_WARM_MAX) return PRD_ERR_ARG;
+    for (int i = 0; i < w->n; ++i) {
+        if (!w->ptr[i] || w->bytes[i] == 0 || (w->bytes[i] & 3) || w->bytes[i] >= ((size_t)1 << 32)) return PRD_ERR_ARG;
+        k->p[i] = static_cast<const char*>(w->ptr[i]);
+        k->bytes[i] = (unsigned)w->bytes[i];
+    }
+    k->n = w->n;
+    return 0;
+}
+static inline void prd_warm_add(PrdWarmK* k, const void* p, size_t bytes) {
+    if (k->n < PRD_WARM_K && p && bytes) { k->p[k->n] = static_cast<const char*>(p); k->bytes[k->n] = (unsigned)bytes; ++k->n; }
+}
+
 static inline int prd_ceil_div(int a, int b) { return (a + b - 1) / b; }
 static inline int prd_round_up(int a, int b) { return prd_ceil_div(a, b) * b; }
diff --git a/protein_redesign_amd/csrc/prd_pair.hip b/protein_redesign_amd/csrc/prd_pair.hip
--- a/protein_redesign_amd/csrc/prd_pair.hip
+++ b/protein_redesign_amd/csrc/prd_pair.hip
@@ -1529,7 +1529,8 @@
 template <int P, int KS>
 __global__ __launch_bounds__(512) void outer_linear_ks_kernel(float* out, const float* pair, const float* __restrict__ x,
                                                               const float* __restrict__ u, const float* __restrict__ w,
-                                                              const float* __restrict__ bias, int b, int N, int residual, int ldu) {
+                                                              const float* __restrict__ bias, int b, int N, int residual, int ldu,
+                                                              PrdWarmK warm) {
     constexpr int NB = P / 32, NW = 8, S = 128 * KS, NG = NB * 4;
     constexpr int CW = 16 * KS;
     constexpr int XP = CW * 4 + 16;
@@ -1688,6 +1689,7 @@
             }
             if (ii + 1 < RG) fetch_x(i + 1, xa);
             pt.mark(0);
+            if (warm.n > 0 && wave == NW - 1 && ii == RG - 1 && t + (int)gridDim.x >= ntask) warm_touch(warm);
             if (ii > 0) finish(i - 1, part + (size_t)((ii - 1) & 1) * PSZ, ecur);
             ecur = enext;
             pt.mark(3);
@@ -1705,6 +1707,7 @@
         finish(T.i0 + RG - 1, part + (size_t)((RG - 1) & 1) * PSZ, ecur);
         __syncthreads();
     }
+    if (warm.n > 0 && wave == NW - 1 && (int)blockIdx.x >= ntask) warm_touch(warm);
     pt.mark(7);
     pt.flush();
 }
@@ -1712,8 +1715,16 @@
 
 extern "C" int prd_outer_linear(float* out, const float* pair, const float* x, const float* u, int ldu, const float* w,
                                 const float* bias, int residual, int b, int N, int P, int S, int* queue, int arith, hipStream_t stream) {
+    return prd_outer_linear_warm(out, pair, x, u, ldu, w, bias, residual, b, N, P, S, queue, nullptr, arith, stream);
+}
+
+extern "C" int prd_outer_linear_warm(float* out, const float* pair, const float* x, const float* u, int ldu, const float* w,
+                                     const float* bias, int residual, int b, int N, int P, int S, int* queue, const prd_warm* next,
+                                     int arith, hipStream_t stream) {
     PRD_SPLIT_ARITH(arith);
     if (!out || !pair || !x || !u || !w || !bias || b <= 0 || N <= 0) return PRD_ERR_ARG;
+    PrdWarmK warm;
+    if (prd_warm_to_k(next, &warm)) return PRD_ERR_ARG;
     if (ldu < P || (ldu & 3)) return PRD_ERR_ALIGN;
     PRD_CHECK_P(P);
     if (S <= 0 || (S & 7)) return PRD_ERR_UNSUPPORTED;
@@ -1729,7 +1740,7 @@
 #define PRD_OLKS(PP, KK)                                                                                               \
         do {                                                                                                           \
             PRD_SET_LDS((outer_linear_ks_kernel<PP, KK>), ldsk);                                                       \
-            hipLaunchKernelGGL((outer_linear_ks_kernel<PP, KK>), dim3(grid), dim3(512), ldsk, stream, out, pair, x, u, w, bias, b, N, residual, ldu); \
+            hipLaunchKernelGGL((outer_linear_ks_kernel<PP, KK>), dim3(grid), dim3(512), ldsk, stream, out, pair, x, u, w, bias, b, N, residual, ldu, warm); \
         } while (0)
         if (P == 64) { if (S == 512) PRD_OLKS(64, 4); else if (S == 256) PRD_OLKS(64, 2); else PRD_OLKS(64, 1); }
         else { if (S == 512) PRD_OLKS(32, 4); else if (S == 256) PRD_OLKS(32, 2); else PRD_OLKS(32, 1); }
diff --git a/protein_redesign_amd/csrc/prd_tri.hip b/protein_redesign_amd/csrc/prd_tri.hip
--- a/protein_redesign_amd/csrc/prd_tri.hip
+++ b/protein_redesign_amd/csrc/prd_tri.hip
@@ -361,7 +361,7 @@
 template <int NWV, int DEPTH = 2, bool ASC = false>
 __global__ __launch_bounds__(NWV * 64) void tri_mul_contract_split_kernel(float* __restrict__ O, const float* __restrict__ AB,
                                                                           int N, int ldn, int P, int nbatch, int tiles, int swap,
-                                                                          const unsigned* __restrict__ a_amax) {
+                                                                          const unsigned* __restrict__ a_amax, PrdWarmK warm) {
     constexpr int NT = NWV * 64, NPT = (2560 + NT - 1) / NT, NSUB = (25 + NWV - 1) / NWV;
     extern __shared__ __attribute__((aligned(16))) unsigned char tms[];
     PhaseTimer pt;
@@ -529,6 +529,7 @@
 #undef PRD_TMS_LOAD
 #undef PRD_TMS_STAGE
 #undef PRD_TMS_CHUNK
+        if (warm.n > 0 && wave == NWV - 1 && vblk + (int)gridDim.x >= nch * t2) warm_touch(warm);
         float* __restrict__ Oc = O + (size_t)ch * N * ldn;
 #pragma unroll
         for (int k = 0; k < NSUB; ++k) {
@@ -544,6 +545,7 @@
         }
         pt.mark(4);
     }
+    if (warm.n > 0 && (int)blockIdx.x >= nch * t2 && wave == NWV - 1) warm_touch(warm);
     pt.flush(3);
 }
 
@@ -551,7 +553,7 @@
 __global__ __launch_bounds__(NW * 64) void tri_mul_out_kernel(int* queue, float* out, const float* pair, const float* __restrict__ O,
                                                               const float* __restrict__ wo, const float* __restrict__ bo,
                                                               const float* __restrict__ wog, const float* __restrict__ bog,
-                                                              int b, int N, int ldn, int residual) {
+                                                              int b, int N, int ldn, int residual, PrdWarmK warm) {
     constexpr int KH = P / 2, NB = P / 32;
     constexpr int WSZ = B3 ? P * P : P * (P + 4);
     __shared__ __attribute__((aligned(16))) float Wol[WSZ];
@@ -579,6 +581,7 @@
     const bool coop = !B3 && queue == nullptr && NB == 2 && NW >= 4 && left > 0 && left <= 2 * (long)gridDim.x;
     const long nwhole = coop ? ntask - left : ntask;
     WaveTasks tasks(queue, nwhole, NW);
+    bool warmed = warm.n <= 0 || wave != 0;
     for (long task = tasks.next(); task >= 0; task = tasks.next()) {
         const int vb = (int)(task % nvb);
         const long bi = task / nvb;
@@ -598,6 +601,10 @@
             load_row_cll_buf<P>(rp, valid ? ((unsigned)r * P + 4 * hi) * 4u : BUF_OOB, xr);
         }
         pt.mark(0);
+        if (!warmed && tasks.is_last()) {
+            warm_touch(warm);
+            warmed = true;
+        }
         float gate[KH];
         {
             float xn[KH];
@@ -635,6 +642,7 @@
         store_row_cll<P>(out + off, hi, valid, x);
         pt.mark(5);
     }
+    if (!warmed) warm_touch(warm);
     pt.mark(7);
     pt.flush(2);
     if (coop) {
@@ -1952,7 +1960,8 @@
 
 template <int P, int NW, bool B3>
 __global__ __launch_bounds__(NW * 64) void tri_attn_out_kernel(int* queue, float* out, const float* pair, const float* __restrict__ og,
-                                                               const float* __restrict__ wo, const float* __restrict__ bo, long rows, int residual) {
+                                                               const float* __restrict__ wo, const float* __restrict__ bo, long rows, int residual,
+                                                               PrdWarmK warm) {
     constexpr int KH = P / 2, NB = P / 32, HC = 64;
     __shared__ __attribute__((aligned(16))) float Wl[B3 ? P * HC : P * (HC + 4)];
     __shared__ __attribute__((aligned(16))) float bl[P];
@@ -1963,11 +1972,16 @@
     const int lane = threadIdx.x & 63, r = lane & 31, hi = lane >> 5;
     const long ntask = (rows + 31) / 32;
     WaveTasks tasks(queue, ntask, NW);
+    bool warmed = warm.n <= 0 || threadIdx.x >= 64;
     for (long task = tasks.next(); task >= 0; task = tasks.next()) {
         const long pos = task * 32 + r;
         const bool valid = pos < rows;
         float x[HC / 2];
         load_row_cll<HC>(og + pos * HC, hi, valid, x);
+        if (!warmed && tasks.is_last()) {
+            warm_touch(warm);
+            warmed = true;
+        }
         f32x16 acc[NB];
         zero_acc(acc);
         if (B3) {
@@ -1983,6 +1997,7 @@
         for (int s = 0; s < KH; ++s) pr[s] = pr[s] + (acc[s >> 4][s & 15] * (B3 ? H2_INV_WSCALE : 1.0f) + bl[hi * KH + s]);
         store_row_cll<P>(out + pos * P, hi, valid, pr);
     }
+    if (!warmed) warm_touch(warm);
 }
 
 int grid_for(long tasks, int per_wg, int cap) {
@@ -2004,31 +2019,31 @@
     } while (0)
 
 static void launch_contract_split(int tune, int grid, size_t lds3, hipStream_t stream, float* O, const float* AB, int N, int ldn, int P, int nbatch,
-                                  int tiles, int swap, const unsigned* a_amax = nullptr) {
+                                  int tiles, int swap, const unsigned* a_amax = nullptr, const PrdWarmK& warm = PrdWarmK{}) {
     if (a_amax) {
         PRD_SET_LDS((tri_mul_contract_split_kernel<8, 2, true>), lds3);
-        hipLaunchKernelGGL((tri_mul_contract_split_kernel<8, 2, true>), dim3(grid), dim3(512), lds3, stream, O, AB, N, ldn, P, nbatch, tiles, swap, a_amax);
+        hipLaunchKernelGGL((tri_mul_contract_split_kernel<8, 2, true>), dim3(grid), dim3(512), lds3, stream, O, AB, N, ldn, P, nbatch, tiles, swap, a_amax, warm);
         return;
     }
     const int nw = PRD_TGET_TMS_NW(tune);
 #ifdef PRD_AB
     if (nw == 8 && PRD_TGET_TMS_D3(tune)) {
         PRD_SET_LDS((tri_mul_contract_split_kernel<8, 3>), lds3);
-        hipLaunchKernelGGL((tri_mul_contract_split_kernel<8, 3>), dim3(grid), dim3(512), lds3, stream, O, AB, N, ldn, P, nbatch, tiles, swap, nullptr);
+        hipLaunchKernelGGL((tri_mul_contract_split_kernel<8, 3>), dim3(grid), dim3(512), lds3, stream, O, AB, N, ldn, P, nbatch, tiles, swap, nullptr, warm);
         return;
     }
     if (nw == 16) {
         PRD_SET_LDS((tri_mul_contract_split_kernel<16>), lds3);
-        hipLaunchKernelGGL((tri_mul_contract_split_kernel<16>), dim3(grid), dim3(1024), lds3, stream, O, AB, N, ldn, P, nbatch, tiles, swap, nullptr);
+        hipLaunchKernelGGL((tri_mul_contract_split_kernel<16>), dim3(grid), dim3(1024), lds3, stream, O, AB, N, ldn, P, nbatch, tiles, swap, nullptr, warm);
         return;
     }
 #endif
     if (nw == 12) {
         PRD_SET_LDS((tri_mul_contract_split_kernel<12>), lds3);
-        hipLaunchKernelGGL((tri_mul_contract_split_kernel<12>), dim3(grid), dim3(768), lds3, stream, O, AB, N, ldn, P, nbatch, tiles, swap, nullptr);
+        hipLaunchKernelGGL((tri_mul_contract_split_kernel<12>), dim3(grid), dim3(768), lds3, stream, O, AB, N, ldn, P, nbatch, tiles, swap, nullptr, warm);
     } else {
         PRD_SET_LDS((tri_mul_contract_split_kernel<8>), lds3);
-        hipLaunchKernelGGL((tri_mul_contract_split_kernel<8>), dim3(grid), dim3(512), lds3, stream, O, AB, N, ldn, P, nbatch, tiles, swap, nullptr);
+        hipLaunchKernelGGL((tri_mul_contract_split_kernel<8>), dim3(grid), dim3(512), lds3, stream, O, AB, N, ldn, P, nbatch, tiles, swap, nullptr, warm);
     }
 }
 
@@ -2179,7 +2194,7 @@
         const int grid = grid_for(ntask, 4, 256);
 #define PRD_OUT_LAUNCH(PP, BB)                                                                                         \
         hipLaunchKernelGGL((tri_mul_out_kernel<PP, NWO, BB>), dim3(grid), dim3(NWO * 64), 0, stream, queue, out, pair, O, w_out, \
-                           b_out, w_ogate, b_ogate, b, N, ldn, residual)
+                           b_out, w_ogate, b_ogate, b, N, ldn, residual, PrdWarmK{})
         if (P == 64) { if (b3o) PRD_OUT_LAUNCH(64, true); else PRD_OUT_LAUNCH(64, false); }
         else { if (b3o) PRD_OUT_LAUNCH(32, true); else PRD_OUT_LAUNCH(32, false); }
 #undef PRD_OUT_LAUNCH
@@ -2224,7 +2239,14 @@
 
 extern "C" int prd_tri_mul_chain(float* pair, const float* mask, const float* const* w_outgoing, const float* const* w_incoming,
                                  int b, int N, int P, float* ws, size_t ws_bytes, int arith, hipStream_t stream) {
+    return prd_tri_mul_chain_warm(pair, mask, w_outgoing, w_incoming, b, N, P, ws, ws_bytes, nullptr, arith, stream);
+}
+
+extern "C" int prd_tri_mul_chain_warm(float* pair, const float* mask, const float* const* w_outgoing, const float* const* w_incoming,
+                                      int b, int N, int P, float* ws, size_t ws_bytes, const prd_warm* next, int arith, hipStream_t stream) {
     PRD_SPLIT_ARITH(arith);
+    PrdWarmK wnext;
+    if (prd_warm_to_k(next, &wnext)) return PRD_ERR_ARG;
     if (!pair || !mask || !w_outgoing || !w_incoming || !ws || b <= 0 || N <= 0) return PRD_ERR_ARG;
     for (int k = 0; k < 8; ++k)
         if (!w_outgoing[k] || !w_incoming[k]) return PRD_ERR_ARG;
@@ -2244,6 +2266,13 @@
     const long rtask = (long)b * N * (ldn / 32);
     const int rgrid = grid_for(rtask, 4, 256);
     const size_t ldsf = ((size_t)2 * P * P + (size_t)2 * 2 * P * P + 6 * P) * sizeof(float);
+    PrdWarmK wfused = PrdWarmK{}, wout = PrdWarmK{};
+    if (next) {
+        const size_t pp = (size_t)P * P * 4, pv = (size_t)P * 4;
+        for (int k = 4; k < 8; ++k) prd_warm_add(&wfused, wa[k], (k & 1) ? pv : pp);
+        for (int k = 0; k < 4; ++k) prd_warm_add(&wfused, wb[k], 2 * ((k & 1) ? pv : pp));
+        for (int k = 4; k < 8; ++k) prd_warm_add(&wout, wb[k], (k & 1) ? pv : pp);
+    }
 #define PRD_CHAIN_STAGE_OK() do { const hipError_t e_ = hipGetLastError(); if (e_ != hipSuccess) return (int)e_; } while (0)
     if (P == 64 && PRD_TGET_TMP_NW16(tune)) {
         PRD_SET_LDS((tri_mul_proj_kernel<64, 16, true>), ldsp);
@@ -2259,7 +2288,7 @@
                            wa[0], wa[1], wa[2], wa[3], b, N, ldn, 0);
     }
     PRD_CHAIN_STAGE_OK();
-        launch_contract_split(tune, vb3 < 256 ? vb3 : 256, lds3, stream, O, AB, N, ldn, P, b, tl, 1);
+        launch_contract_split(tune, vb3 < 256 ? vb3 : 256, lds3, stream, O, AB, N, ldn, P, b, tl, 1, nullptr, wfused);
     PRD_CHAIN_STAGE_OK();
     if (P == 64) {
         PRD_SET_LDS((tri_mul_out_proj_kernel<64, 12>), ldsf);
@@ -2271,15 +2300,15 @@
                            wb[0], wb[1], wb[2], wb[3], AB, b, N, ldn);
     }
     PRD_CHAIN_STAGE_OK();
-        launch_contract_split(tune, vb3 < 256 ? vb3 : 256, lds3, stream, O, AB, N, ldn, P, b, tl, 0);
+        launch_contract_split(tune, vb3 < 256 ? vb3 : 256, lds3, stream, O, AB, N, ldn, P, b, tl, 0, nullptr, wout);
     PRD_CHAIN_STAGE_OK();
     {
         const long ntask = (long)b * N * prd_ceil_div(N, 32);
         const int grid = grid_for(ntask, 4, 256);
         if (P == 64) hipLaunchKernelGGL((tri_mul_out_kernel<64, 8, true>), dim3(grid), dim3(8 * 64), 0, stream, (int*)nullptr, pair, pair, O,
-                                        wb[4], wb[5], wb[6], wb[7], b, N, ldn, 1);
+                                        wb[4], wb[5], wb[6], wb[7], b, N, ldn, 1, wnext);
         else hipLaunchKernelGGL((tri_mul_out_kernel<32, 8, true>), dim3(grid), dim3(8 * 64), 0, stream, (int*)nullptr, pair, pair, O,
-                                wb[4], wb[5], wb[6], wb[7], b, N, ldn, 1);
+                                wb[4], wb[5], wb[6], wb[7], b, N, ldn, 1, wnext);
     }
 #undef PRD_CHAIN_STAGE_OK
     return (int)hipGetLastError();
@@ -2288,7 +2317,17 @@
 extern "C" int prd_tri_attn_core(float* og, const float* pair, const float* mask, const float* wq, const float* wk,
                                  const float* wv, const float* wg, const float* bg, int ending,
                                  int b, int N, int P, int H, int c, int arith, hipStream_t stream) {
+    return prd_tri_attn_core_warm(og, pair, mask, wq, wk, wv, wg, bg, ending, b, N, P, H, c, nullptr, arith, stream);
+}
+
+extern "C" int prd_tri_attn_core_warm(float* og, const float* pair, const float* mask, const float* wq, const float* wk,
+                                      const float* wv, const float* wg, const float* bg, int ending,
+                                      int b, int N, int P, int H, int c, const prd_warm* next, int arith, hipStream_t stream) {
     PRD_SPLIT_ARITH(arith);
+    {
+        PrdWarmK chk;
+        if (prd_warm_to_k(next, &chk)) return PRD_ERR_ARG;
+    }
     if (!og || !pair || !mask || !wq || !wk || !wv || !wg || !bg || b <= 0 || N <= 0) return PRD_ERR_ARG;
     if ((P != 32 && P != 64) || c != 16 || H * c != 64) return PRD_ERR_UNSUPPORTED;
     const int npad = prd_round_up(N, 64);
@@ -2296,7 +2335,7 @@
     const bool split = arith == PRD_ARITH_SPLIT16;
     const int variant = PRD_FIRST_GEN ? PRD_TGET_TA_VARIANT(tune) : 0;
     if (split && variant == 0 && prd_tri_attn_v2_supported(N, P, tune) && (long)b * N * N <= 0x7fffffffL / 2)
-        return prd_tri_attn_core_v2(og, pair, mask, wq, wk, wv, wg, bg, ending, b, N, P, H, c, tune, stream);
+        return prd_tri_attn_core_v2_warm(og, pair, mask, wq, wk, wv, wg, bg, ending, b, N, P, H, c, next, tune, stream);
     const bool b3 = split && PRD_FIRST_GEN;
     bool long_row;
     const size_t lds = tri_attn_lds(N, P, b3, &long_row);
@@ -2393,8 +2432,8 @@
 #endif
 }
 
-extern "C" int prd_tri_attn_out(float* out, const float* pair, const float* og, const float* wo, const float* bo,
-                                int residual, int b, int N, int P, int* queue, int arith, hipStream_t stream) {
+static int tri_attn_out_impl(float* out, const float* pair, const float* og, const float* wo, const float* bo,
+                             int residual, int b, int N, int P, int* queue, const PrdWarmK& warm, int arith, hipStream_t stream) {
     PRD_SPLIT_ARITH(arith);
     if (!out || !pair || !og || !wo || !bo || b <= 0 || N <= 0) return PRD_ERR_ARG;
     if (P != 32 && P != 64) return PRD_ERR_UNSUPPORTED;
@@ -2402,26 +2441,47 @@
     const long rows = (long)b * N * N;
     const int grid2 = grid_for((rows + 31) / 32, 4, 256);
     const bool b3 = arith == PRD_ARITH_SPLIT16;
-#define PRD_TAO(PP, BB) hipLaunchKernelGGL((tri_attn_out_kernel<PP, NWA, BB>), dim3(grid2), dim3(NWA * 64), 0, stream, queue, out, pair, og, wo, bo, rows, residual)
+#define PRD_TAO(PP, BB) hipLaunchKernelGGL((tri_attn_out_kernel<PP, NWA, BB>), dim3(grid2), dim3(NWA * 64), 0, stream, queue, out, pair, og, wo, bo, rows, residual, warm)
     if (P == 64) { if (b3) PRD_TAO(64, true); else PRD_TAO(64, false); }
     else { if (b3) PRD_TAO(32, true); else PRD_TAO(32, false); }
 #undef PRD_TAO
     return (int)hipGetLastError();
 }
 
+extern "C" int prd_tri_attn_out(float* out, const float* pair, const float* og, const float* wo, const float* bo,
+                                int residual, int b, int N, int P, int* queue, int arith, hipStream_t stream) {
+    return tri_attn_out_impl(out, pair, og, wo, bo, residual, b, N, P, queue, PrdWarmK{}, arith, stream);
+}
+
 extern "C" int prd_tri_attn(float* out, const float* pair, const float* mask, const float* wq, const float* wk, const float* wv,
                             const float* wg, const float* bg, const float* wo, const float* bo, int ending, int residual,
                             int b, int N, int P, int H, int c, float* ws, size_t ws_bytes, int* queue, int arith, hipStream_t stream) {
+    return prd_tri_attn_warm(out, pair, mask, wq, wk, wv, wg, bg, wo, bo, ending, residual, b, N, P, H, c, ws, ws_bytes, queue, nullptr, arith, stream);
+}
+
+extern "C" int prd_tri_attn_warm(float* out, const float* pair, const float* mask, const float* wq, const float* wk, const float* wv,
+                                 const float* wg, const float* bg, const float* wo, const float* bo, int ending, int residual,
+                                 int b, int N, int P, int H, int c, float* ws, size_t ws_bytes, int* queue, const prd_warm* next,
+                                 int arith, hipStream_t stream) {
     PRD_SPLIT_ARITH(arith);
     if (!ws) return PRD_ERR_ARG;
+    PrdWarmK wnext;
+    if (prd_warm_to_k(next, &wnext)) return PRD_ERR_ARG;
+    prd_warm seam = {};
+    if (next && wo && bo && (P == 32 || P == 64)) {
+        seam.n = 2;
+        seam.ptr[0] = wo; seam.bytes[0] = (size_t)P * 64 * 4;
+        seam.ptr[1] = bo; seam.bytes[1] = (size_t)P * 4;
+    }
+    const prd_warm* cnext = next ? &seam : nullptr;
     if (ws_bytes < prd_workspace_bytes("tri_attn", b, N, 0, P)) return PRD_ERR_WORKSPACE;
     int e;
     if (prd_tri_attn_variant(N, P, arith_full) == 3) {
         const size_t nog = (size_t)b * N * N * 64;
         e = prd_tri_attn_core_chunked(ws, pair, mask, wq, wk, wv, wg, bg, ending, b, N, P, H, c, ws + nog, ws_bytes - nog * sizeof(float), stream);
     } else {
-        e = prd_tri_attn_core(ws, pair, mask, wq, wk, wv, wg, bg, ending, b, N, P, H, c, arith_full, stream);
+        e = prd_tri_attn_core_warm(ws, pair, mask, wq, wk, wv, wg, bg, ending, b, N, P, H, c, cnext, arith_full, stream);
     }
     if (e) return e;
-    return prd_tri_attn_out(out, pair, ws, wo, bo, residual, b, N, P, queue, arith_full, stream);
-}
+    return tri_attn_out_impl(out, pair, ws, wo, bo, residual, b, N, P, queue, wnext, arith_full, stream);
+}
diff --git a/protein_redesign_amd/csrc/prd_tri2.hip b/protein_redesign_amd/csrc/prd_tri2.hip
--- a/protein_redesign_amd/csrc/prd_tri2.hip
+++ b/protein_redesign_amd/csrc/prd_tri2.hip
@@ -583,7 +583,7 @@
     float* __restrict__ og, const float* __restrict__ pair, const float* __restrict__ mask,
     const float* __restrict__ wq, const float* __restrict__ wk, const float* __restrict__ wv,
     const float* __restrict__ wg, const float* __restrict__ bg, int b, int N, int NP, int H, int ending, int flags,
-    float* __restrict__ lse_out) {
+    float* __restrict__ lse_out, PrdWarmK warm) {
     constexpr int C = 16, HC = 64, NT = NW * 64, KH = P / 2;
     constexpr float VSCALE = H2_WSCALE;
     extern __shared__ __attribute__((aligned(16))) unsigned char lds[];
@@ -596,6 +596,7 @@
     const float* __restrict__ wq, const float* __restrict__ wk, const float* __restrict__ wv,
     const float* __restrict__ wg, const float* __restrict__ bg, int b, int N, int NP, int H, int ending, int flags,
     float* __restrict__ lse_out, unsigned char* lds) {
+    constexpr PrdWarmK warm = {};
     constexpr int C = 16, HC = 64, NT = NW * 64, KH = P / 2;
     constexpr float VSCALE = H2_WSCALE;
 #include "prd_tri2_v3_body.inc"
@@ -1706,9 +1707,9 @@
     return (!PRD_TGET_TA2_NO_V3(tune) && v3_lds_bytes(N, P) <= 160 * 1024) ? 2 : 1;
 }
 
-extern "C" int prd_tri_attn_core_v2_lse(float* og, float* lse, const float* pair, const float* mask, const float* wq, const float* wk,
-                                        const float* wv, const float* wg, const float* bg, int ending,
-                                        int b, int N, int P, int H, int c, int tune, hipStream_t stream) {
+static int tri_attn_core_v2_impl(float* og, float* lse, const float* pair, const float* mask, const float* wq, const float* wk,
+                                 const float* wv, const float* wg, const float* bg, int ending,
+                                 int b, int N, int P, int H, int c, const PrdWarmK& warm, int tune, hipStream_t stream) {
     if (!og || !pair || !mask || !wq || !wk || !wv || !wg || !bg || b <= 0 || N <= 0 || tune < 0) return PRD_ERR_ARG;
     if ((P != 32 && P != 64) || c != 16 || H * c != 64) return PRD_ERR_UNSUPPORTED;
     if (!prd_tri_attn_v2_supported(N, P, tune)) return PRD_ERR_UNSUPPORTED;
@@ -1767,7 +1768,7 @@
         do {                                                                                                                      \
             PRD2_SET_LDS((tri_attn_core_v3_kernel<PP, NWV, KLF, GVF>));                                                           \
             hipLaunchKernelGGL((tri_attn_core_v3_kernel<PP, NWV, KLF, GVF>), dim3(grid), dim3(NWV * 64), lds3, stream, og, pair, mask, wq, wk, wv, wg, \
-                               bg, b, N, NP, H, ending, flags & ~6, lse);                                                         \
+                               bg, b, N, NP, H, ending, flags & ~6, lse, warm);                                                       \
         } while (0)
         const int kl = flags_env >= 0 ? (flags >> 1) & 3 : PRD_V3_DEFAULT_KL;
         const bool gvf = !PRD_TGET_TA2_NO_GV(tune) && kl == 0;
@@ -1798,10 +1799,24 @@
     return (int)hipGetLastError();
 }
 
+extern "C" int prd_tri_attn_core_v2_lse(float* og, float* lse, const float* pair, const float* mask, const float* wq, const float* wk,
+                                        const float* wv, const float* wg, const float* bg, int ending,
+                                        int b, int N, int P, int H, int c, int tune, hipStream_t stream) {
+    return tri_attn_core_v2_impl(og, lse, pair, mask, wq, wk, wv, wg, bg, ending, b, N, P, H, c, PrdWarmK{}, tune, stream);
+}
+
 extern "C" int prd_tri_attn_core_v2(float* og, const float* pair, const float* mask, const float* wq, const float* wk,
                                     const float* wv, const float* wg, const float* bg, int ending,
                                     int b, int N, int P, int H, int c, int tune, hipStream_t stream) {
-    return prd_tri_attn_core_v2_lse(og, nullptr, pair, mask, wq, wk, wv, wg, bg, ending, b, N, P, H, c, tune, stream);
+    return prd_tri_attn_core_v2_warm(og, pair, mask, wq, wk, wv, wg, bg, ending, b, N, P, H, c, nullptr, tune, stream);
+}
+
+extern "C" int prd_tri_attn_core_v2_warm(float* og, const float* pair, const float* mask, const float* wq, const float* wk,
+                                         const float* wv, const float* wg, const float* bg, int ending,
+                                         int b, int N, int P, int H, int c, const prd_warm* next, int tune, hipStream_t stream) {
+    PrdWarmK warm;
+    if (prd_warm_to_k(next, &warm)) return PRD_ERR_ARG;
+    return tri_attn_core_v2_impl(og, nullptr, pair, mask, wq, wk, wv, wg, bg, ending, b, N, P, H, c, warm, tune, stream);
 }
 
 static int prd_cu_count() {
diff --git a/protein_redesign_amd/csrc/prd_tri2_v3_body.inc b/protein_redesign_amd/csrc/prd_tri2_v3_body.inc
--- a/protein_redesign_amd/csrc/prd_tri2_v3_body.inc
+++ b/protein_redesign_amd/csrc/prd_tri2_v3_body.inc
@@ -414,10 +414,13 @@
         if (bun < nrows) {
             rcur = make_row(bun);
             phase1(rcur, par ^ 1, gpar == 2 ? 0 : gpar + 1);
+        } else if (warm.n > 0 && wave == 0) {
+            warm_touch(warm);
         }
         PRD2_STAMP(4);
         gpar = gpar == 2 ? 0 : gpar + 1;
     }
+    if (it == 0 && warm.n > 0 && wave == 0) warm_touch(warm);
     if (it > 0 && m4 > 0) {
         __syncthreads();
         if (group_owner) merge(rprev, (it - 1) & 1, gpar == 0 ? 2 : gpar - 1);
diff --git a/protein_redesign_amd/ops.py b/protein_redesign_amd/ops.py
--- a/protein_redesign_amd/ops.py
+++ b/protein_redesign_amd/ops.py
@@ -6,6 +6,7 @@
 
 import torch
 
+from . import _lib
 from ._lib import PrdGemm, arithmetic, check, dptr, lib, stream
 
 F32 = torch.float32
@@ -267,13 +268,30 @@
     return out, oa, ob
 
 
-def outer_linear_pair(pair, x, u, w, bias, *, residual: bool, out=None) -> torch.Tensor:
+WARM_NEXT = os.environ.get("PRD_WARM_NEXT", "1") != "0"
+
+
+def warm_hint(tensors):
+    if not WARM_NEXT or tensors is None:
+        return None
+    ts = [t for t in tensors if t is not None]
+    if len(ts) > _lib.WARM_MAX:
+        raise ValueError(f"warm_hint: at most {_lib.WARM_MAX} ranges")
+    w = _lib.PrdWarm()
+    w.n = len(ts)
+    for k, t in enumerate(ts):
+        w.ptr[k] = dptr(t)
+        w.bytes[k] = t.numel() * t.element_size()
+    return w
+
+
+def outer_linear_pair(pair, x, u, w, bias, *, residual: bool, out=None, warm=None) -> torch.Tensor:
     b, N, _, P = pair.shape
     if out is None:
         out = torch.empty_like(pair)
     up, ldu = row_block(u)
-    check(lib().prd_outer_linear(dptr(out), dptr(pair), dptr(x), up, ldu, dptr(w), dptr(bias), int(residual),
-                                 b, N, P, x.shape[-1], task_queue(pair.device), stream()), "prd_outer_linear")
+    check(lib().prd_outer_linear_warm(dptr(out), dptr(pair), dptr(x), up, ldu, dptr(w), dptr(bias), int(residual),
+                                      b, N, P, x.shape[-1], task_queue(pair.device), warm, stream()), "prd_outer_linear")
     return out
 
 
@@ -297,7 +315,7 @@
     return lib().prd_tri_mul_chain_supported(N, P) == 1
 
 
-def tri_mul_chain_(pair, mask, wts_outgoing, wts_incoming, ws=None) -> torch.Tensor:
+def tri_mul_chain_(pair, mask, wts_outgoing, wts_incoming, ws=None, warm=None) -> torch.Tensor:
     import ctypes
     b, N, _, P = pair.shape
     nbytes = workspace_bytes("tri_mul", b, N, 0, P)
@@ -306,8 +324,8 @@
     arr = ctypes.c_void_p * 8
     wa = arr(*[dptr(w) for w in wts_outgoing])
     wb = arr(*[dptr(w) for w in wts_incoming])
-    check(lib().prd_tri_mul_chain(dptr(pair), dptr(mask), ctypes.cast(wa, ctypes.c_void_p), ctypes.cast(wb, ctypes.c_void_p),
-                                  b, N, P, dptr(ws), ws.numel() * 4, stream()), "prd_tri_mul_chain")
+    check(lib().prd_tri_mul_chain_warm(dptr(pair), dptr(mask), ctypes.cast(wa, ctypes.c_void_p), ctypes.cast(wb, ctypes.c_void_p),
+                                       b, N, P, dptr(ws), ws.numel() * 4, warm, stream()), "prd_tri_mul_chain")
     return pair
 
 
@@ -659,7 +677,7 @@
     return dqkvg
 
 
-def tri_attn(pair, mask, wts, H: int, c: int, *, ending: bool, residual: bool, out=None, ws=None) -> torch.Tensor:
+def tri_attn(pair, mask, wts, H: int, c: int, *, ending: bool, residual: bool, out=None, ws=None, warm=None) -> torch.Tensor:
     b, N, _, P = pair.shape
     if not default_head_layout(H, c):
         og = tri_attn_core_heads(pair, mask, wts[:5], H, c, ending=ending, ws=ws)
@@ -669,8 +687,8 @@
     nbytes = workspace_bytes("tri_attn", b, N, 0, P)
     if ws is None:
         ws = torch.empty(nbytes // 4, device=pair.device, dtype=F32)
-    check(lib().prd_tri_attn(dptr(out), dptr(pair), dptr(mask), *[dptr(w) for w in wts], int(ending), int(residual),
-                             b, N, P, H, c, dptr(ws), ws.numel() * 4, task_queue(pair.device), stream()), "prd_tri_attn")
+    check(lib().prd_tri_attn_warm(dptr(out), dptr(pair), dptr(mask), *[dptr(w) for w in wts], int(ending), int(residual),
+                                  b, N, P, H, c, dptr(ws), ws.numel() * 4, task_queue(pair.device), warm, stream()), "prd_tri_attn")
     return out
 
 
@@ -739,7 +757,7 @@
             and lib().prd_tri_attn_bwd_core_v2_supported(N, P) == 1 and TRI_ATTN_BWD_V2)
 
 
-def tri_attn_core(pair, mask, wts, H: int, c: int, *, ending: bool, og=None, stats=None, lse=None) -> torch.Tensor:
+def tri_attn_core(pair, mask, wts, H: int, c: int, *, ending: bool, og=None, stats=None, lse=None, warm=None) -> torch.Tensor:
     b, N, _, P = pair.shape
     if og is None:
         og = torch.empty(b, N, N, 64, device=pair.device, dtype=F32)
@@ -758,8 +776,8 @@
         check(lib().prd_tri_attn_core_chunked(dptr(og), dptr(pair), dptr(mask), *[dptr(w) for w in wts], int(ending),
                                               b, N, P, H, c, dptr(stats), stats.numel() * 4, stream()), "prd_tri_attn_core_chunked")
         return og
-    check(lib().prd_tri_attn_core(dptr(og), dptr(pair), dptr(mask), *[dptr(w) for w in wts], int(ending),
-                                  b, N, P, H, c, stream()), "prd_tri_attn_core")
+    check(lib().prd_tri_attn_core_warm(dptr(og), dptr(pair), dptr(mask), *[dptr(w) for w in wts], int(ending),
+                                       b, N, P, H, c, warm, stream()), "prd_tri_attn_core")
     return og
 
 
diff --git a/protein_redesign_amd/trunk.py b/protein_redesign_amd/trunk.py
--- a/protein_redesign_amd/trunk.py
+++ b/protein_redesign_amd/trunk.py
@@ -104,10 +104,10 @@
         self.attn = Attention(pair_dim, head_dim, num_heads)
         self.mode = mode
 
-    def run(self, pair, mask, *, residual: bool, out=None, ws=None):
+    def run(self, pair, mask, *, residual: bool, out=None, ws=None, warm=None):
         a = self.attn
         return ops.tri_attn(pair, mask, a.weights(), a.num_heads, a.head_dim, ending=self.mode == "ending",
-                            residual=residual, out=out, ws=ws)
+                            residual=residual, out=out, ws=ws, warm=warm)
 
     def forward(self, pair: torch.Tensor, mask_2d: torch.Tensor) -> torch.Tensor:
         return self.run(pair.contiguous(), _node_mask(mask_2d), residual=False)
@@ -268,19 +268,23 @@
         if bias is None:
             bias = ops.pair_bias(pair, self.attn_bias[1].weight, self.attn_bias[1].bias)
         single, x, u = self.single_track_(single, mask, bias, next_block=next_block, qkvg=qkvg, tail=tail, extra=extra)
+        pf = self.pair_fc
+        nb_w = next_block.attn_bias[1].weight if next_block is not None else None
+        nb_b = next_block.attn_bias[1].bias if next_block is not None else None
+        chain = _TRI_MUL_CHAIN and ops.tri_mul_chain_supported(N, pair.shape[-1])
+        hint = (ops.warm_hint if pair.is_cuda and not general and not torch.is_grad_enabled() else (lambda ts: None))
         if u is not None:
             ol = self.outer_linear.linear
-            ops.outer_linear_pair(pair, x, u, ol.weight, ol.bias, residual=True, out=pair)
+            ops.outer_linear_pair(pair, x, u, ol.weight, ol.bias, residual=True, out=pair,
+                                  warm=hint(self.pair_mul_outgoing.weights()[:4]) if chain else None)
         else:
             self.outer_linear.run(single, pair, residual=True, out=pair)
-        if _TRI_MUL_CHAIN and ops.tri_mul_chain_supported(N, pair.shape[-1]):
-            ops.tri_mul_chain_(pair, mask, self.pair_mul_outgoing.weights(), self.pair_mul_incoming.weights(), ws=ws)
+        if chain:
+            ops.tri_mul_chain_(pair, mask, self.pair_mul_outgoing.weights(), self.pair_mul_incoming.weights(), ws=ws,
+                               warm=hint(self.pair_attn_starting.attn.weights()[:5]))
         else:
             self.pair_mul_outgoing.run(pair, mask, residual=True, out=pair, ws=ws)
             self.pair_mul_incoming.run(pair, mask, residual=True, out=pair, ws=ws)
-        pf = self.pair_fc
-        nb_w = next_block.attn_bias[1].weight if next_block is not None else None
-        nb_b = next_block.attn_bias[1].bias if next_block is not None else None
         if general:
             self.pair_attn_starting.run(pair, mask, residual=True, out=pair, ws=ws)
             og = ops.tri_attn_core_heads(pair, mask, ta.weights()[:5], ta.num_heads, ta.head_dim, ending=True, ws=ws)
@@ -309,9 +313,11 @@
             ts = self.pair_attn_starting.attn
             og = ops.tri_attn_pair_(pair, mask, ts.weights(), ta.weights()[:5], ta.num_heads, ta.head_dim, og=ws[:nog].view(b, N, N, 64))
         else:
-            self.pair_attn_starting.run(pair, mask, residual=True, out=pair, ws=ws)
+            self.pair_attn_starting.run(pair, mask, residual=True, out=pair, ws=ws, warm=hint(ta.weights()[:5]))
             og = ops.tri_attn_core(pair, mask, ta.weights()[:5], ta.num_heads, ta.head_dim, ending=True,
-                                   og=ws[:nog].view(b, N, N, 64), stats=ws[nog:] if ws.numel() > nog else None)
+                                   og=ws[:nog].view(b, N, N, 64), stats=ws[nog:] if ws.numel() > nog else None,
+                                   warm=hint((ta.out_proj.weight, ta.out_proj.bias, pf[1].weight, pf[1].bias, pf[3].weight, pf[3].bias,
+                                              nb_w, nb_b)))
         next_bias = ops.block_tail_(pair, og, ta.out_proj.weight, ta.out_proj.bias, pf[1].weight, pf[1].bias,
                                     pf[3].weight, pf[3].bias, nb_w, nb_b)
         return single, pair, next_bias
```
